# MadNLP/MadNLP.jl

Hardware: NVIDIA H100
Metric: ipm_iters_per_sec (higher is better)
Workload: dtype f64

## Files before the change

### include/b200kkt.h

```cpp
#ifndef B200KKT_H
#define B200KKT_H

#include <stdint.h>

#ifdef __cplusplus
extern "C" {
#endif

#define B2_OK                 0
#define B2_ERR_INVALID        1
#define B2_ERR_CUDA           2
#define B2_ERR_SYMBOLIC       3
#define B2_ERR_FACTORIZATION  4
#define B2_ERR_SOLVE          5
#define B2_ERR_NO_DEVICE      6
#define B2_ERR_UNSUPPORTED    7

#define B2_ORDER_METIS_ND 0
#define B2_ORDER_MINDEG   1
#define B2_ORDER_NATURAL  2
#define B2_ORDER_USER     3

const char* b2_last_error(void);
int b2_version(void);
int b2_device_count(int* count);

typedef struct b2_options {
    int32_t ordering;
    int32_t nemin;
    double  relax_zeros;
    double  pivot_eps;
    int32_t use_cuda_graph;
    int32_t small_front_max;
    int32_t n_parts;
    int32_t part_rank;
    int32_t kkt_n_primal;
    int32_t fuse_max_fronts;
    int32_t dep_schedule;
    int32_t chain_merge_f;
    int32_t kkt_n_dual;
    int32_t dense_pivoting;
    int32_t sparse_pivoting;
    int32_t reserved[1];
} b2_options;

#define B2_DENSE_PIVOT_STATIC        0
#define B2_DENSE_PIVOT_BUNCH_KAUFMAN 1
#define B2_SPARSE_PIVOT_STATIC       0
#define B2_SPARSE_PIVOT_PAIRS        1

#define B2_PIVOT_1X1            0
#define B2_PIVOT_1X1_PERTURBED  1
#define B2_PIVOT_2X2_FIRST      2
#define B2_PIVOT_2X2_SECOND     3

int b2_options_default(b2_options* opt);

typedef struct b2_solver b2_solver;

typedef struct b2_stats {
    int64_t n, nnz_a, nnz_l, flops;
    int64_t n_supernodes, n_levels;
    int64_t max_front, n_small_fronts, n_big_fronts;
    int64_t factor_bytes, workspace_bytes;
    int64_t sep_rows;
    int64_t n_factor_launches, n_solve_launches;
    int64_t n_perturbed;
} b2_stats;

int b2_create(int32_t n, int64_t nnz, const int32_t* colptr_h, const int32_t* rowval_h,
              const double* nzval_d, const b2_options* opt, const int32_t* user_perm_h,
              b2_solver** out);
int b2_create_symbolic_only(int32_t n, int64_t nnz, const int32_t* colptr_h, const int32_t* rowval_h,
                            const b2_options* opt, const int32_t* user_perm_h, b2_solver** out);
int b2_destroy(b2_solver* s);
int b2_set_values_ptr(b2_solver* s, const double* nzval_d);
int b2_factorize(b2_solver* s, void* stream);
int b2_inertia(b2_solver* s, int64_t* num_pos, int64_t* num_zero, int64_t* num_neg, void* stream);
int b2_inertia_enqueue(b2_solver* s, void* stream);
int b2_inertia_fetch(b2_solver* s, int64_t* num_pos, int64_t* num_zero, int64_t* num_neg);
int b2_solve(b2_solver* s, double* x_d, int32_t nrhs, void* stream);
int b2_improve(b2_solver* s, int32_t* changed);
int b2_get_stats(b2_solver* s, b2_stats* st);
int b2_get_perm(b2_solver* s, int32_t* perm_h);

int b2_exchange_buffer(b2_solver* s, double** buf_d, int64_t* n_factor_doubles, int64_t* n_solve_doubles);
int b2_exchange_vector(b2_solver* s, double** buf_d, int64_t* n_doubles);
int b2_inertia_parts(b2_solver* s, int64_t* local_neg, int64_t* local_zero, int64_t* top_neg, int64_t* top_zero, void* stream);
int b2_factorize_local(b2_solver* s, void* stream);
int b2_factorize_top(b2_solver* s, void* stream);
int b2_solve_fwd_local(b2_solver* s, double* x_d, void* stream);
int b2_solve_top(b2_solver* s, double* x_d, void* stream);
int b2_solve_bwd_local(b2_solver* s, double* x_d, void* stream);
int b2_owned_mask(b2_solver* s, uint8_t* owned_h);

typedef struct b2_symbolic_sizes {
    int64_t n, n_supernodes, n_rows, n_children, n_rel, n_amap, n_levels, lval_size, cb_size;
} b2_symbolic_sizes;
int b2_symbolic_query(b2_solver* s, b2_symbolic_sizes* sz);
int b2_symbolic_export(b2_solver* s, int32_t* perm, int32_t* sn_first, int32_t* sn_parent, int32_t* sn_level,
                       int64_t* rows_ptr, int32_t* rows, int64_t* lp_off, int64_t* cb_off,
                       int64_t* rel_ptr, int32_t* rel, int64_t* amap_ptr, int64_t* amap_src, int64_t* amap_dst);
int b2_symbolic_owner(b2_solver* s, int32_t* owner);
int b2_symbolic_exchange(b2_solver* s, int64_t* cbv_off, int64_t* exch_cb, int64_t* exch_cbv);
int b2_debug_get_factor(b2_solver* s, double* lval_h, double* dvec_h);
int b2_symbolic_pairs(b2_solver* s, uint8_t* pair_start_h);
int b2_get_pivot_blocks(b2_solver* s, int8_t* kind_h, double* d_h, double* d_off_h);
int b2_debug_profile_front(b2_solver* s, int32_t sn, int32_t reps, int64_t* stamps_h);
int b2_debug_trace(b2_solver* s, uint64_t* stamps_h, int32_t* parent_h, int32_t* w_h, int32_t* f_h, int64_t capacity, int64_t* count);
int b2_debug_trace_solve(b2_solver* s, uint64_t* stamps_h, int64_t capacity, int64_t* count);
int b2_debug_dep_order(b2_solver* s, int32_t* order_h, int64_t capacity, int64_t* count);

typedef struct b2d_solver b2d_solver;
int b2d_create(int32_t N, int32_t lda, const double* A_d, const b2_options* opt, b2d_solver** out);
int b2d_destroy(b2d_solver* s);
int b2d_debug_trace(b2d_solver* s, uint64_t* stamps_h, int64_t capacity, int64_t* count);
int b2d_factorize(b2d_solver* s, void* stream);
int b2d_inertia(b2d_solver* s, int64_t* num_pos, int64_t* num_zero, int64_t* num_neg, void* stream);
int b2d_inertia_enqueue(b2d_solver* s, void* stream);
int b2d_inertia_fetch(b2d_solver* s, int64_t* num_pos, int64_t* num_zero, int64_t* num_neg);
int b2d_solve(b2d_solver* s, double* x_d, int32_t nrhs, void* stream);
int b2d_get_pivots(b2d_solver* s, int32_t* ipiv_h, double* d_h, double* e_h);

int b2_coo_to_csc(int32_t m, int32_t n, int64_t nnz_coo, const int32_t* I_h, const int32_t* J_h,
                  int32_t* colptr_h, int32_t* rowval_h, int64_t* map_h, int64_t* nnz_csc);

int b2_coo_to_csc_device(int32_t m, int32_t n, int64_t nnz_coo, const int32_t* I_d, const int32_t* J_d,
                         int32_t* colptr_d, int32_t* rowval_d, int64_t* map_d, int64_t* nnz_csc, void* stream);

typedef struct b2_transfer_plan b2_transfer_plan;
int b2_transfer_plan_create(int64_t nnz_coo, int64_t nnz_csc, const int64_t* map_h, b2_transfer_plan** out);
int b2_transfer_plan_destroy(b2_transfer_plan* p);
int b2_transfer(b2_transfer_plan* p, double* dst_nz_d, const double* V_d, void* stream);

typedef struct b2_condensed_plan b2_condensed_plan;
int b2_condensed_symbolic(int32_t n, int32_t m,
                          const int32_t* H_colptr_h, const int32_t* H_rowval_h,
                          const int32_t* Jt_colptr_h, const int32_t* Jt_rowval_h,
                          b2_condensed_plan** out, int64_t* nnz_aug);
int b2_condensed_symbolic_device(int32_t n, int32_t m,
                                 const int32_t* H_colptr_d, const int32_t* H_rowval_d,
                                 const int32_t* Jt_colptr_d, const int32_t* Jt_rowval_d,
                                 b2_condensed_plan** out, int64_t* nnz_aug, void* stream);
int b2_condensed_pattern(b2_condensed_plan* p, int32_t* colptr_h, int32_t* rowval_h);
int b2_condensed_plan_sizes(b2_condensed_plan* p, int64_t* n_dptr, int64_t* n_hptr, int64_t* n_jptr);
int b2_condensed_plan_destroy(b2_condensed_plan* p);
int b2_condensed_assemble(b2_condensed_plan* p, double* aug_nz_d, const double* pr_diag_d,
                          const double* du_diag_d, const double* H_nz_d, const double* Jt_nz_d,
                          double* diag_buffer_d, void* stream);

int b2d_condensed_assemble(int32_t n, int32_t m, int32_t ns, int32_t n_eq,
                           const int64_t* ind_ineq_d, const int64_t* ind_eq_d,
                           const double* hess_d, const double* jac_d,
                           const double* pr_diag_d, const double* du_diag_d,
                           double* diag_buffer_d, double* aug_d, void* stream);

int b2d_aug_assemble(int32_t n, int32_t m, int32_t ns, const int64_t* ind_ineq_d,
                     const double* hess_d, const double* jac_d, const double* pr_diag_d,
                     const double* du_diag_d, const double* diag_hess_d, double* aug_d, void* stream);
int b2d_copy_diag(int32_t n, int32_t lda, const double* A_d, double* d_d, void* stream);

typedef struct b2d_ozaki_plan b2d_ozaki_plan;
int b2d_ozaki_plan_create(int32_t n, int32_t ns, b2d_ozaki_plan** out);
int b2d_ozaki_plan_destroy(b2d_ozaki_plan* p);
int b2d_condensed_assemble_ozaki(b2d_ozaki_plan* p, int32_t n, int32_t m, int32_t ns, int32_t n_eq,
                                 const int64_t* ind_ineq_d, const int64_t* ind_eq_d,
                                 const double* hess_d, const double* jac_d,
                                 const double* pr_diag_d, const double* du_diag_d,
                                 double* diag_buffer_d, double* aug_d, void* stream);
int b2d_ozaki_plan_status(b2d_ozaki_plan* p, int32_t* timed_out, void* stream);

int b2d_gemv_n(int32_t rows, int32_t cols, int32_t lda, const double* A_d, const double* x_d, double* y_d, double alpha, double beta, void* stream);
int b2d_gemv_t(int32_t rows, int32_t cols, int32_t lda, const double* A_d, const double* x_d, double* y_d, double alpha, double beta, void* stream);
int b2d_symv_lower(int32_t n, int32_t lda, const double* A_d, const double* x_d, double* y_d, double alpha, double beta, void* stream);

typedef struct b2_bounds b2_bounds;
typedef struct b2d_kkt b2d_kkt;
int b2d_kkt_create(int32_t n, int32_t m, int32_t ns, const int64_t* ind_ineq_h, b2d_kkt** out);
int b2d_kkt_destroy(b2d_kkt* k);
int b2d_kkt_solve_pre(b2d_kkt* k, b2_bounds* b, const double* jac_d, const double* pr_diag_d, const double* diag_buffer_d,
                      const double* l_diag_d, const double* u_diag_d, double* buffer_d, double* pd_buffer_d, double* w_d, void* stream);
int b2d_kkt_solve_post(b2d_kkt* k, b2_bounds* b, const double* jac_d, const double* pr_diag_d, const double* diag_buffer_d,
                       const double* l_lower_d, const double* u_lower_d, const double* l_diag_d, const double* u_diag_d,
                       const double* buffer_d, const double* pd_buffer_d, double* w_d, void* stream);
int b2d_kkt_mul(b2d_kkt* k, b2_bounds* b, const double* hess_d, const double* jac_d, const double* reg_d, const double* du_diag_d,
                const double* l_lower_d, const double* u_lower_d, const double* l_diag_d, const double* u_diag_d,
                double alpha, double beta, const double* x_d, double* w_d, void* stream);

typedef struct b2_bounds b2_bounds;
int b2_bounds_create(int64_t n_tot, int64_t nlb, int64_t nub, const int64_t* ind_lb_h, const int64_t* ind_ub_h,
                     b2_bounds** out);
int b2_bounds_destroy(b2_bounds* b);

int b2_set_aug_diagonal(b2_bounds* b, const double* reg_d, const double* l_lower_d, const double* l_diag_d,
                        const double* u_lower_d, const double* u_diag_d, double* pr_diag_d, void* stream);
int b2_set_aug_diagonal_unreduced(int64_t n_tot, int64_t nlb, int64_t nub, const double* reg_d, const double* l_lower_d,
                                  const double* u_lower_d, double* pr_diag_d, double* l_lower_aug_d, double* u_lower_aug_d,
                                  void* stream);
int b2_unreduced_solve_pre(int64_t n_tot, int64_t m, int64_t nlb, int64_t nub, const double* l_lower_aug_d,
                           const double* u_lower_aug_d, double* w_d, void* stream);
int b2_unreduced_solve_post(int64_t n_tot, int64_t m, int64_t nlb, int64_t nub, const double* l_lower_aug_d,
                            const double* u_lower_aug_d, double* w_d, void* stream);
int b2_scaled_set_aug_diagonal(b2_bounds* b, const double* reg_d, const double* l_lower_d, const double* l_diag_d,
                               const double* u_lower_d, const double* u_diag_d, double* pr_diag_d, double* scaling_d, void* stream);
int b2_scaled_transfer(b2_transfer_plan* p, int64_t n, int64_t n_tot, const int32_t* colptr_d, const int32_t* rowval_d,
                       const double* scaling_d, double* dst_nz_d, const double* V_d, void* stream);
int b2_scaled_solve_pre(b2_bounds* b, int64_t m, const double* l_diag_d, const double* u_diag_d, const double* scaling_d, double* w_d,
                        void* stream);
int b2_scaled_solve_post(b2_bounds* b, int64_t m, const double* l_lower_d, const double* u_lower_d, const double* l_diag_d,
                         const double* u_diag_d, const double* scaling_d, double* w_d, void* stream);
int b2_scaled_kktmul(b2_bounds* b, int64_t m, const double* reg_d, const double* du_diag_d, const double* l_lower_d,
                     const double* u_lower_d, const double* l_diag_d, const double* u_diag_d, double alpha, double beta,
                     const double* x_d, double* w_d, void* stream);
int b2_scaled_regularize_diagonal(int64_t n_tot, int64_t m, double dw, double dc, const double* scaling_d, double* reg_d,
                                  double* pr_diag_d, double* du_diag_d, void* stream);
int b2_regularize_diagonal(int64_t n_tot, int64_t m, double dw, double dc, double* reg_d, double* pr_diag_d,
                           double* du_diag_d, void* stream);
int b2_reduce_rhs(b2_bounds* b, int64_t m, const double* l_diag_d, const double* u_diag_d, double* w_d, void* stream);
int b2_finish_aug_solve(b2_bounds* b, int64_t m, const double* l_lower_d, const double* u_lower_d,
                        const double* l_diag_d, const double* u_diag_d, double* w_d, void* stream);

typedef struct b2_spmv_plan b2_spmv_plan;
int b2_spmv_plan_create(int32_t nrow, int32_t ncol, const int32_t* colptr_h, const int32_t* rowval_h, b2_spmv_plan** out);
int b2_spmv_plan_destroy(b2_spmv_plan* p);
int b2_spmv_n(b2_spmv_plan* p, const double* nz_d, const double* x_d, double* y_d, double alpha, double beta, void* stream);
int b2_spmv_t(b2_spmv_plan* p, const double* nz_d, const double* x_d, double* y_d, double alpha, double beta, void* stream);
int b2_spmv_symlower(b2_spmv_plan* p, const double* nz_d, const double* x_d, double* y_d, double alpha, double beta, void* stream);

int b2_kktmul(b2_bounds* b, int64_t m, const double* reg_d, const double* du_diag_d,
              const double* l_lower_d, const double* u_lower_d, const double* l_diag_d, const double* u_diag_d,
              double alpha, double beta, const double* x_d, double* w_d, void* stream);

int b2_condensed_solve_pre(b2_bounds* b, b2_spmv_plan* jt, int64_t n, int64_t m,
                           const double* jt_nz_d, const double* pr_diag_d, const double* diag_buffer_d,
                           const double* l_diag_d, const double* u_diag_d, double* buffer_d, double* w_d, void* stream);
int b2_condensed_solve_post(b2_bounds* b, b2_spmv_plan* jt, int64_t n, int64_t m,
                            const double* jt_nz_d, const double* pr_diag_d, const double* diag_buffer_d,
                            const double* l_lower_d, const double* u_lower_d, const double* l_diag_d, const double* u_diag_d,
                            const double* buffer_d, double* w_d, void* stream);
int b2_condensed_refine_pre(b2_bounds* b, b2_spmv_plan* jt, int64_t n, int64_t m,
                            const double* jt_nz_d, const double* pr_diag_d, const double* diag_buffer_d,
                            const double* l_diag_d, const double* u_diag_d, double* buffer_d, double* w_d, double* norms_d, void* stream);
int b2_condensed_solve_post_update(b2_bounds* b, b2_spmv_plan* jt, int64_t n, int64_t m,
                                   const double* jt_nz_d, const double* pr_diag_d, const double* diag_buffer_d,
                                   const double* l_lower_d, const double* u_lower_d, const double* l_diag_d, const double* u_diag_d,
                                   const double* buffer_d, double* w_d, double* x_d, double* norms_d, void* stream);
int b2_condensed_kkt_mul(b2_bounds* b, b2_spmv_plan* hess, b2_spmv_plan* jt, int64_t n, int64_t m,
                         const double* hess_nz_d, const double* jt_nz_d,
                         const double* reg_d, const double* du_diag_d, const double* l_lower_d, const double* u_lower_d,
                         const double* l_diag_d, const double* u_diag_d, double alpha, double beta,
                         const double* x_d, double* w_d, void* stream);
int b2_condensed_kkt_mul_norm(b2_bounds* b, b2_spmv_plan* hess, b2_spmv_plan* jt, int64_t n, int64_t m,
                         const double* hess_nz_d, const double* jt_nz_d,
                         const double* reg_d, const double* du_diag_d, const double* l_lower_d, const double* u_lower_d,
                         const double* l_diag_d, const double* u_diag_d, double alpha, double beta,
                         const double* x_d, double* w_d, double* norm_inf_d, void* stream);
int b2_condensed_kkt_mul_norm_y(b2_bounds* b, b2_spmv_plan* hess, b2_spmv_plan* jt, int64_t n, int64_t m,
                           const double* hess_nz_d, const double* jt_nz_d,
                           const double* reg_d, const double* du_diag_d, const double* l_lower_d, const double* u_lower_d,
                           const double* l_diag_d, const double* u_diag_d, double alpha, double beta,
                           const double* x_d, const double* y_d, double* w_d, double* norm_inf_d, void* stream);

int b2_richardson_begin(int64_t n, const double* b_d, double* w_d, double* x_d, double* norm_b_d, void* stream);
int b2_richardson_update(int64_t n, const double* b_d, double* w_d, double* x_d, double* norms_d, void* stream);
int b2_norm_inf(int64_t n, const double* x_d, double* out_d, void* stream);
int b2_axpy(int64_t n, double a, const double* x_d, double* y_d, void* stream);
int b2_copy(int64_t n, const double* x_d, double* y_d, void* stream);
int b2_copy_many(int32_t count, const double* const* src_d, double* const* dst_d, const int64_t* n, void* stream);
int b2_fill(int64_t n, double v, double* x_d, void* stream);

int b2_get_alpha_max(b2_bounds* b, const double* x_d, const double* xl_d, const double* xu_d, const double* dx_d, double tau,
                     double* out_d, void* stream);
int b2_get_alpha_z(b2_bounds* b, const double* zl_d, const double* zu_d, const double* dzl_d, const double* dzu_d, double tau,
                   double* out_d, void* stream);
int b2_get_varphi(b2_bounds* b, double obj_val, const double* x_d, const double* xl_d, const double* xu_d, double mu, double* out_d,
                  void* stream);
int b2_get_varphi_d(b2_bounds* b, const double* f_d, const double* x_d, const double* xl_d, const double* xu_d, const double* dx_d,
                    double mu, double* out_d, void* stream);
int b2_get_inf_du(b2_bounds* b, const double* f_d, const double* zl_d, const double* zu_d, const double* jacl_d, double sd,
                  double* out_d, void* stream);
int b2_get_inf_compl(b2_bounds* b, const double* x_d, const double* xl_d, const double* xu_d, const double* zl_d, const double* zu_d,
                     double mu, double sc, double* out_d, void* stream);
int b2_get_average_complementarity(b2_bounds* b, const double* x_d, const double* xl_d, const double* xu_d, const double* zl_d,
                                   const double* zu_d, double* out_d, void* stream);
int b2_get_min_complementarity(b2_bounds* b, const double* x_d, const double* xl_d, const double* xu_d, const double* zl_d,
                               const double* zu_d, double* out_d, void* stream);
int b2_get_rel_search_norm(b2_bounds* b, int64_t n, const double* x_d, const double* dx_d, double* out_d, void* stream);
int b2_get_sd(b2_bounds* b, int64_t m, const double* l_d, const double* zl_d, const double* zu_d, double s_max, double* out_d,
              void* stream);
int b2_get_sc(b2_bounds* b, const double* zl_d, const double* zu_d, double s_max, double* out_d, void* stream);
int b2_set_aug_rhs(b2_bounds* b, int64_t m, const double* x_d, const double* xl_d, const double* xu_d, const double* f_d,
                   const double* zl_d, const double* zu_d, const double* jacl_d, const double* c_d, double mu, double* p_d, void* stream);

int b2_set_g_ifr(int64_t n, const double* f_d, const double* x_d, const double* xl_d, const double* xu_d, const double* jacl_d, double mu,
                 double* g_d, void* stream);
int b2_set_aug_rhs_ifr(int64_t n_tot, int64_t m, int64_t nlb, int64_t nub, const double* c_d, double* p0_d, void* stream);
#define B2_CURV_WXT  0
#define B2_CURV_WXN  1
#define B2_CURV_GN   2
#define B2_CURV_TT   3
#define B2_CURV_LHS  4
#define B2_CURV_PASS 5
#define B2_CURV_RESULT_LEN 6
int b2_mul_hess_blk_tail(b2_bounds* b, int64_t n_h, int32_t unreduced, const double* pr_diag_d, const double* l_lower_d,
                         const double* l_diag_d, const double* u_lower_d, const double* u_diag_d, const double* t_d, double* wx_d,
                         const double* n_d, const double* g_d, double tol, double* result_d, void* stream);

int b2_rr_init(b2_bounds* b, int64_t m, const double* x_d, const double* c_d, double mu_R, double rho, double* x_ref_d, double* D_R_d,
               double* f_R_d, double* pp_d, double* nn_d, double* zp_d, double* zn_d, double* y_d, double* zl_d, double* zu_d, void* stream);
int b2_set_aug_rr(b2_bounds* b, int64_t m, double del_w, double del_c, double zeta, const double* D_R_d, const double* pp_d,
                  const double* nn_d, const double* zp_d, const double* zn_d, const double* x_d, const double* xl_d, const double* xu_d,
                  const double* zl_d, const double* zu_d, double* reg_d, double* du_diag_d, double* l_lower_d, double* u_lower_d,
                  double* l_diag_d, double* u_diag_d, void* stream);
int b2_set_aug_rr_scaled(b2_bounds* b, int64_t m, double del_w, double del_c, double zeta, const double* D_R_d, const double* pp_d,
                         const double* nn_d, const double* zp_d, const double* zn_d, const double* x_d, const double* xl_d, const double* xu_d,
                         const double* zl_d, const double* zu_d, double* reg_d, double* du_diag_d, double* l_lower_d, double* u_lower_d,
                         double* l_diag_d, double* u_diag_d, void* stream);
int b2_set_aug_rhs_rr(b2_bounds* b, int64_t m, const double* x_d, const double* xl_d, const double* xu_d, const double* zl_d,
                      const double* zu_d, const double* jacl_d, const double* f_R_d, const double* c_d, const double* y_d, const double* pp_d,
                      const double* nn_d, const double* zp_d, const double* zn_d, double mu_R, double rho, double* p_d, void* stream);
int b2_finish_aug_solve_rr(int64_t m, const double* l_d, const double* dl_d, const double* pp_d, const double* nn_d, const double* zp_d,
                           const double* zn_d, double mu_R, double rho, double* dpp_d, double* dnn_d, double* dzp_d, double* dzn_d,
                           void* stream);
int b2_set_f_rr(int64_t n, double zeta, const double* D_R_d, const double* x_d, const double* x_ref_d, double* f_R_d, void* stream);
int b2_reset_bound_dual(int64_t n, double* z_d, const double* x_d, double mu, double kappa_sigma, void* stream);
int b2_reset_bound_dual_lu(b2_bounds* b, double* zl_d, double* zu_d, const double* x_d, const double* xl_d, const double* xu_d, double mu,
                           double kappa_sigma, void* stream);
int b2_adjust_boundary(b2_bounds* b, const double* x_d, double* xl_d, double* xu_d, double mu, void* stream);
int b2_get_theta(b2_bounds* b, int64_t m, const double* c_d, double* out_d, void* stream);
int b2_get_theta_r(b2_bounds* b, int64_t m, const double* c_d, const double* pp_d, const double* nn_d, double* out_d, void* stream);
int b2_get_inf_pr_r(b2_bounds* b, int64_t m, const double* c_d, const double* pp_d, const double* nn_d, double* out_d, void* stream);
int b2_get_obj_val_r(b2_bounds* b, int64_t m, const double* pp_d, const double* nn_d, const double* D_R_d, const double* x_d,
                     const double* x_ref_d, double rho, double zeta, double* out_d, void* stream);
int b2_get_inf_du_r(b2_bounds* b, int64_t m, const double* f_R_d, const double* l_d, const double* zl_d, const double* zu_d,
                    const double* jacl_d, const double* zp_d, const double* zn_d, double rho, double sd, double* out_d, void* stream);
int b2_get_inf_compl_r(b2_bounds* b, int64_t m, const double* x_d, const double* xl_d, const double* xu_d, const double* zl_d,
                       const double* zu_d, const double* pp_d, const double* zp_d, const double* nn_d, const double* zn_d, double mu_R,
                       double sc, double* out_d, void* stream);
int b2_get_alpha_max_r(b2_bounds* b, int64_t m, const double* x_d, const double* xl_d, const double* xu_d, const double* dx_d,
                       const double* pp_d, const double* dpp_d, const double* nn_d, const double* dnn_d, double tau_R, double* out_d,
                       void* stream);
int b2_get_alpha_z_r(b2_bounds* b, int64_t m, const double* zl_d, const double* zu_d, const double* dzl_d, const double* dzu_d,
                     const double* zp_d, const double* dzp_d, const double* zn_d, const double* dzn_d, double tau_R, double* out_d,
                     void* stream);
int b2_get_varphi_r(b2_bounds* b, int64_t m, double obj_val, const double* x_d, const double* xl_d, const double* xu_d, const double* pp_d,
                    const double* nn_d, double mu_R, double* out_d, void* stream);
int b2_get_varphi_d_r(b2_bounds* b, int64_t m, const double* f_R_d, const double* x_d, const double* xl_d, const double* xu_d,
                      const double* dx_d, const double* pp_d, const double* nn_d, const double* dpp_d, const double* dnn_d, double mu_R,
                      double rho, double* out_d, void* stream);

int b2_set_aug_diagonal_iterate(b2_bounds* b, int64_t m, double del_w, double del_c, const double* x_d, const double* xl_d, const double* xu_d,
                                const double* zl_d, const double* zu_d, double* reg_d, double* du_diag_d, double* l_lower_d,
                                double* u_lower_d, double* l_diag_d, double* u_diag_d, void* stream);
int b2_set_aug_diagonal_iterate_scaled(b2_bounds* b, int64_t m, double del_w, double del_c, const double* x_d, const double* xl_d,
                                       const double* xu_d, const double* zl_d, const double* zu_d, double* reg_d, double* du_diag_d,
                                       double* l_lower_d, double* u_lower_d, double* l_diag_d, double* u_diag_d, void* stream);
int b2_set_aug_rhs_perturbed(b2_bounds* b, int64_t m, const double* x_d, const double* xl_d, const double* xu_d, const double* f_d,
                             const double* zl_d, const double* zu_d, const double* jacl_d, const double* c_d, const double* c_trial_d,
                             double alpha, double mu, double kappa_d, int64_t nllb, const int64_t* ind_llb_d, int64_t nuub,
                             const int64_t* ind_uub_d, double* p_d, void* stream);
int b2_set_initial_rhs(b2_bounds* b, int64_t m, const double* f_d, const double* zl_d, const double* zu_d, double* p_d, void* stream);
#define B2_DUAL_INIT_NORM       0
#define B2_DUAL_INIT_COPY       1
#define B2_DUAL_INIT_RESULT_LEN 2
int b2_dual_init_select(b2_bounds* b, int64_t m, const double* dy_d, int32_t solved, double constr_mult_init_max, double* y_d,
                        double* result_d, void* stream);
int b2_get_pd_error(b2_bounds* b, int64_t m, const double* c_d, const double* f_d, const double* zl_d, const double* zu_d,
                    const double* jacl_d, const double* x_d, const double* xl_d, const double* xu_d, double mu, double* out_d, void* stream);
int b2_restore_update(b2_bounds* b, int64_t m, const double* alpha_max_d, const double* alpha_z_d, double* alpha_d, const double* dx_d,
                      const double* dy_d, const double* dzl_d, const double* dzu_d, double* x_d, double* y_d, double* zl_d, double* zu_d,
                      void* stream);
int b2_soc_trial(int64_t n, const double* alpha_d, const double* x_d, const double* wx_d, double* x_trial_d, void* stream);

#define B2_QF_TAU         0
#define B2_QF_NRM_PRIMAL  1
#define B2_QF_NRM_DUAL    2
#define B2_QF_MU_AVG      3
#define B2_QF_SCAL_LEN    4
#define B2_QF_SIGMA       0
#define B2_QF_MU          1
#define B2_QF_N_EVAL      2
#define B2_QF_N_GS_ITER   3
#define B2_QF_TOL_EXIT    4
#define B2_QF_TRACE       8
#define B2_QF_MAX_GS_ITER 64
#define B2_QF_RESULT_LEN(max_gs_iter) (B2_QF_TRACE + 4 * (6 + (max_gs_iter)))
int b2_primal_dual_norm2(b2_bounds* b, int64_t m, const double* p_d, double* out_d, void* stream);
int b2_set_centering_aug_rhs(b2_bounds* b, int64_t m, int64_t nllb, const int64_t* ind_llb_d, int64_t nuub, const int64_t* ind_uub_d,
                             const double* mu_d, double kappa_d, double* p_d, void* stream);
int b2_qf_search(b2_bounds* b, int64_t m, const double* x_d, const double* xl_d, const double* xu_d, const double* zl_d, const double* zu_d,
                 const double* aff_d, const double* cen_d, const double* scal_d, double sigma_min, double sigma_max, double mu_min,
                 double mu_max, double sigma_tol, int32_t max_gs_iter, double* result_d, void* stream);

typedef struct b2_lbfgs b2_lbfgs;
int b2_lbfgs_create(int64_t n, int32_t max_history, int32_t init_strategy, double init_value, double sigma_min, double sigma_max,
                    b2_lbfgs** out);
int b2_lbfgs_destroy(b2_lbfgs* h);
int b2_lbfgs_state(b2_lbfgs* h, int64_t* p, int64_t* skipped, double* sigma, void* stream);
int b2_lbfgs_init(b2_lbfgs* h, double* Bk_d, const double* g0_d, double f0, void* stream);
int b2_lbfgs_update(b2_lbfgs* h, double* Bk_d, const double* sk_d, const double* yk_d, void* stream);
int b2_lbfgs_smw_prepare(b2_lbfgs* h, b2_solver* s, int64_t n_tot_plus_m, double* H_d, void* stream);
int b2_lbfgs_smw_apply(b2_lbfgs* h, int64_t n_tot_plus_m, const double* H_d, double* w_d, void* stream);
int b2_lbfgs_kkt_mul_lowrank(b2_lbfgs* h, double alpha, const double* x_d, double* w_d, void* stream);
#define B2_LBFGS_BUF_S  0
#define B2_LBFGS_BUF_Y  1
#define B2_LBFGS_BUF_U  2
#define B2_LBFGS_BUF_V  3
#define B2_LBFGS_BUF_SS 4
#define B2_LBFGS_BUF_L  5
#define B2_LBFGS_BUF_D  6
#define B2_LBFGS_BUF_J  7
#define B2_LBFGS_BUF_DL 8
#define B2_LBFGS_BUF_T  9
#define B2_LBFGS_BUF_TF 10
int b2_lbfgs_debug_get(b2_lbfgs* h, int32_t what, double* dst_h, int64_t* first, void* stream);
int b2_lbfgs_debug_ipiv(b2_lbfgs* h, int32_t* ipiv_h, void* stream);
int b2_debug_bk_factor(int32_t N, double* A_d, int32_t* ipiv_d, void* stream);
int b2_debug_bk_solve(int32_t N, const double* F_d, const int32_t* ipiv_d, double* b_d, void* stream);

#define B2_QN_BFGS        1
#define B2_QN_DAMPED_BFGS 2
typedef struct b2d_qn b2d_qn;
int b2d_qn_create(int64_t n, int32_t kind, b2d_qn** out);
int b2d_qn_destroy(b2d_qn* h);
int b2d_qn_init(b2d_qn* h, double* Bk_d, const double* g0_d, double f0, void* stream);
int b2d_qn_update(b2d_qn* h, double* Bk_d, const double* sk_d, const double* yk_d, void* stream);
int b2d_qn_rank2(b2d_qn* h, double* Bk_d, const double* yk_d, void* stream);
int b2d_qn_state(b2d_qn* h, int32_t* instantiated, int32_t* accepted, double* scalars, void* stream);
int b2d_qn_debug_vectors(b2d_qn* h, double* bsk_h, double* rk_h, void* stream);

#define B2_KRYLOV_MAX_RESTART 16
#define B2_KRYLOV_H           0
#define B2_KRYLOV_CS          272
#define B2_KRYLOV_SN          288
#define B2_KRYLOV_G           304
#define B2_KRYLOV_Y           321
#define B2_KRYLOV_SCALE       337
#define B2_KRYLOV_REC         344
#define B2_KRYLOV_REC_EST     0
#define B2_KRYLOV_REC_H       1
#define B2_KRYLOV_REC_NORM_W  2
#define B2_KRYLOV_REC_NORM_X  3
#define B2_KRYLOV_REC_NORM_B  4
#define B2_KRYLOV_REC_NORM_B2 5
#define B2_KRYLOV_REC_LEN     8
#define B2_KRYLOV_STATE_LEN   352
typedef struct b2_krylov b2_krylov;
int b2_krylov_create(int64_t n, int32_t restart, b2_krylov** out);
int b2_krylov_destroy(b2_krylov* h);
int b2_krylov_buffers(b2_krylov* h, double** V_d, double** Z_d, double** state_d);
int b2_krylov_begin(b2_krylov* h, int32_t first, const double* b_d, double* x_d, double* w_d, void* stream);
int b2_krylov_scale(b2_krylov* h, int32_t k, const double* w_d, void* stream);
int b2_krylov_orthogonalize(b2_krylov* h, int32_t k, double* w_d, void* stream);
int b2_krylov_close(b2_krylov* h, int32_t m, const double* b_d, double* x_d, double* w_d, void* stream);

typedef struct b2_inertia_source {
    const int32_t* counters_d;
    int64_t n;
    int32_t neg[2], zero[2];
    int32_t fail;
    int32_t reserved;
} b2_inertia_source;
int b2_inertia_source_get(b2_solver* s, b2_inertia_source* out);
typedef struct b2_refine_record {
    double ratio;
    double norm_w, norm_x, norm_b;
    int64_t ir;
    int64_t steps;
    int64_t num_pos, num_zero, num_neg;
    int32_t inertia_ok;
    int32_t fail;
    int64_t seq;
} b2_refine_record;
typedef struct b2_refine_loop b2_refine_loop;
int b2_refine_loop_create(b2_refine_loop** out);
int b2_refine_loop_destroy(b2_refine_loop* h);
int b2_refine_loop_begin(b2_refine_loop* h, int64_t n, const double* b_d, double* w_d, double* x_d, double* norms_d, void* stream);
int b2_refine_loop_end(b2_refine_loop* h, const b2_inertia_source* src, int64_t expect_pos, int64_t expect_neg, int32_t max_iter,
                       double tol, void* stream);
int b2_refine_loop_launch(b2_refine_loop* h, void* stream);
int b2_refine_loop_wait(b2_refine_loop* h);
int b2_refine_loop_record(b2_refine_loop* h, b2_refine_record* out);

typedef struct b2_inertia_options {
    double first_hessian_perturbation, min_hessian_perturbation, max_hessian_perturbation;
    double perturb_inc_fact_first, perturb_inc_fact, perturb_dec_fact;
} b2_inertia_options;
#define B2_TRIALS_ACCEPTED 1
#define B2_TRIALS_FAILED   2
#define B2_TRIALS_HANDOVER 3
#define B2_TRIALS_FAULT    4
typedef struct b2_inertia_record {
    int32_t status;
    int32_t inertia_ok;
    int64_t trials;
    double del_w, del_w_prev, del_c_prev;
    int64_t num_pos, num_zero, num_neg;
    int64_t ir;
    double ratio;
    int64_t ir_total;
    int64_t seq;
} b2_inertia_record;
int b2_inertia_trial_bound(const b2_inertia_options* opt, int64_t* out);
typedef struct b2_inertia_loop b2_inertia_loop;
int b2_inertia_loop_create(const b2_inertia_options* opt, b2_inertia_loop** out);
int b2_inertia_loop_destroy(b2_inertia_loop* h);
int b2_inertia_loop_begin(b2_inertia_loop* h, int64_t n_tot, int64_t m, double* reg_d, double* pr_diag_d, double* du_diag_d,
                          int32_t dual_always, void* stream);
int b2_inertia_loop_begin_scaled(b2_inertia_loop* h, int64_t n_tot, int64_t m, double* reg_d, double* pr_diag_d, double* du_diag_d,
                                 const double* scaling_d, int32_t dual_always, void* stream);
int b2_inertia_loop_refine(b2_inertia_loop* h, const b2_inertia_source* src, int64_t expect_pos, int64_t expect_neg, int64_t n,
                           const double* b_d, double* w_d, double* x_d, double* norms_d, void* stream);
int b2_inertia_loop_end(b2_inertia_loop* h, int32_t max_iter, double tol, double acceptable_tol, void* stream);
int b2_inertia_loop_launch(b2_inertia_loop* h, double del_w_last, double del_c, int64_t num_zero, void* stream);
int b2_inertia_loop_wait(b2_inertia_loop* h);
int b2_inertia_loop_record(b2_inertia_loop* h, b2_inertia_record* out, double* del_w_out, int64_t cap);


#ifdef __cplusplus
}
#endif
#endif
```

### madnlp.jl_b200/capi.py

```python
from __future__ import annotations

import ctypes as C
import os

_HERE = os.path.dirname(os.path.abspath(__file__))
LIB_PATH = os.path.join(_HERE, "csrc", "libb200kkt.so")

B2_OK = 0
B2_ERR_INVALID, B2_ERR_CUDA, B2_ERR_SYMBOLIC, B2_ERR_FACTORIZATION, B2_ERR_SOLVE, B2_ERR_NO_DEVICE, B2_ERR_UNSUPPORTED = 1, 2, 3, 4, 5, 6, 7
ORDER_METIS_ND, ORDER_MINDEG, ORDER_NATURAL, ORDER_USER = 0, 1, 2, 3
QN_BFGS, QN_DAMPED_BFGS = 1, 2
B2_DENSE_PIVOT_STATIC, B2_DENSE_PIVOT_BUNCH_KAUFMAN = 0, 1
B2_SPARSE_PIVOT_STATIC, B2_SPARSE_PIVOT_PAIRS = 0, 1
B2_PIVOT_1X1, B2_PIVOT_1X1_PERTURBED, B2_PIVOT_2X2_FIRST, B2_PIVOT_2X2_SECOND = 0, 1, 2, 3
CURV_WXT, CURV_WXN, CURV_GN, CURV_TT, CURV_LHS, CURV_PASS, CURV_RESULT_LEN = 0, 1, 2, 3, 4, 5, 6
DUAL_INIT_NORM, DUAL_INIT_COPY, DUAL_INIT_RESULT_LEN = 0, 1, 2
QF_TAU, QF_NRM_PRIMAL, QF_NRM_DUAL, QF_MU_AVG, QF_SCAL_LEN = 0, 1, 2, 3, 4
QF_SIGMA, QF_MU, QF_N_EVAL, QF_N_GS_ITER, QF_TOL_EXIT, QF_TRACE, QF_MAX_GS_ITER = 0, 1, 2, 3, 4, 8, 64
KRYLOV_MAX_RESTART, KRYLOV_Y, KRYLOV_REC, KRYLOV_REC_LEN, KRYLOV_STATE_LEN = 16, 321, 344, 8, 352
KREC_EST, KREC_H, KREC_NORM_W, KREC_NORM_X, KREC_NORM_B, KREC_NORM_B2 = 0, 1, 2, 3, 4, 5


def qf_result_len(max_gs_iter):
    return QF_TRACE + 4 * (6 + max_gs_iter)


class B2Error(RuntimeError):
    def __init__(self, code, msg):
        super().__init__(f"b200kkt error {code}: {msg}")
        self.code = code


class SymbolicException(B2Error):
    pass


class FactorizationException(B2Error):
    pass


class SolveException(B2Error):
    pass


class InertiaException(RuntimeError):
    pass


class _Pivoting(C.Structure):
    _fields_ = [("dense_pivoting", C.c_int32), ("sparse_pivoting", C.c_int32)]


class _OptionsTail(C.Union):
    _anonymous_ = ("_pivoting",)
    _fields_ = [("_pivoting", _Pivoting), ("reserved", C.c_int32 * 3)]


class Options(C.Structure):
    _anonymous_ = ("_tail",)
    _fields_ = [
        ("ordering", C.c_int32), ("nemin", C.c_int32), ("relax_zeros", C.c_double), ("pivot_eps", C.c_double),
        ("use_cuda_graph", C.c_int32), ("small_front_max", C.c_int32), ("n_parts", C.c_int32), ("part_rank", C.c_int32),
        ("kkt_n_primal", C.c_int32), ("fuse_max_fronts", C.c_int32), ("dep_schedule", C.c_int32), ("chain_merge_f", C.c_int32), ("kkt_n_dual", C.c_int32),
        ("_tail", _OptionsTail),
    ]


class Stats(C.Structure):
    _fields_ = [(k, C.c_int64) for k in (
        "n", "nnz_a", "nnz_l", "flops", "n_supernodes", "n_levels", "max_front", "n_small_fronts", "n_big_fronts",
        "factor_bytes", "workspace_bytes", "sep_rows", "n_factor_launches", "n_solve_launches", "n_perturbed")]

    def as_dict(self):
        return {k: int(getattr(self, k)) for k, _ in self._fields_}


class InertiaSource(C.Structure):
    _fields_ = [("counters_d", C.c_void_p), ("n", C.c_int64), ("neg", C.c_int32 * 2), ("zero", C.c_int32 * 2), ("fail", C.c_int32),
                ("reserved", C.c_int32)]


class RefineRecord(C.Structure):
    _fields_ = [("ratio", C.c_double), ("norm_w", C.c_double), ("norm_x", C.c_double), ("norm_b", C.c_double), ("ir", C.c_int64),
                ("steps", C.c_int64), ("num_pos", C.c_int64), ("num_zero", C.c_int64), ("num_neg", C.c_int64), ("inertia_ok", C.c_int32),
                ("fail", C.c_int32), ("seq", C.c_int64)]


class InertiaSchedule(C.Structure):
    _fields_ = [(k, C.c_double) for k in ("first_hessian_perturbation", "min_hessian_perturbation", "max_hessian_perturbation",
                                          "perturb_inc_fact_first", "perturb_inc_fact", "perturb_dec_fact")]


TRIALS_ACCEPTED, TRIALS_FAILED, TRIALS_HANDOVER, TRIALS_FAULT = 1, 2, 3, 4


class InertiaRecord(C.Structure):
    _fields_ = [("status", C.c_int32), ("inertia_ok", C.c_int32), ("trials", C.c_int64), ("del_w", C.c_double),
                ("del_w_prev", C.c_double), ("del_c_prev", C.c_double), ("num_pos", C.c_int64), ("num_zero", C.c_int64),
                ("num_neg", C.c_int64), ("ir", C.c_int64), ("ratio", C.c_double), ("ir_total", C.c_int64), ("seq", C.c_int64)]


class SymbolicSizes(C.Structure):
    _fields_ = [(k, C.c_int64) for k in (
        "n", "n_supernodes", "n_rows", "n_children", "n_rel", "n_amap", "n_levels", "lval_size", "cb_size")]


def _load():
    if not os.path.exists(LIB_PATH):
        raise ImportError(
            f"{LIB_PATH} not found: build it with `python -c 'import __graft_entry__ as g; g.build()'` "
            f"(or `make -C madnlp.jl_b200/csrc`). The GPU KKT path has no CPU fallback.")
    return C.CDLL(LIB_PATH)


lib = _load()

_p = C.c_void_p
_i32, _i64, _f64 = C.c_int32, C.c_int64, C.c_double
_PP = C.POINTER(C.c_void_p)

PROTOTYPES = {
    "b2_last_error": (C.c_char_p, []),
    "b2_version": (C.c_int, []),
    "b2_device_count": (C.c_int, [C.POINTER(C.c_int)]),
    "b2_options_default": (C.c_int, [C.POINTER(Options)]),
    "b2_create": (C.c_int, [_i32, _i64, _p, _p, _p, C.POINTER(Options), _p, _PP]),
    "b2_create_symbolic_only": (C.c_int, [_i32, _i64, _p, _p, C.POINTER(Options), _p, _PP]),
    "b2_destroy": (C.c_int, [_p]),
    "b2_set_values_ptr": (C.c_int, [_p, _p]),
    "b2_factorize": (C.c_int, [_p, _p]),
    "b2_inertia": (C.c_int, [_p, C.POINTER(_i64), C.POINTER(_i64), C.POINTER(_i64), _p]),
    "b2_inertia_enqueue": (C.c_int, [_p, _p]),
    "b2_inertia_fetch": (C.c_int, [_p, C.POINTER(_i64), C.POINTER(_i64), C.POINTER(_i64)]),
    "b2_solve": (C.c_int, [_p, _p, _i32, _p]),
    "b2_improve": (C.c_int, [_p, C.POINTER(_i32)]),
    "b2_get_stats": (C.c_int, [_p, C.POINTER(Stats)]),
    "b2_get_perm": (C.c_int, [_p, _p]),
    "b2_exchange_buffer": (C.c_int, [_p, _PP, C.POINTER(_i64), C.POINTER(_i64)]),
    "b2_exchange_vector": (C.c_int, [_p, _PP, C.POINTER(_i64)]),
    "b2_inertia_parts": (C.c_int, [_p, C.POINTER(_i64), C.POINTER(_i64), C.POINTER(_i64), C.POINTER(_i64), _p]),
    "b2_factorize_local": (C.c_int, [_p, _p]),
    "b2_factorize_top": (C.c_int, [_p, _p]),
    "b2_solve_fwd_local": (C.c_int, [_p, _p, _p]),
    "b2_solve_top": (C.c_int, [_p, _p, _p]),
    "b2_solve_bwd_local": (C.c_int, [_p, _p, _p]),
    "b2_owned_mask": (C.c_int, [_p, _p]),
    "b2_symbolic_query": (C.c_int, [_p, C.POINTER(SymbolicSizes)]),
    "b2_symbolic_export": (C.c_int, [_p] + [_p] * 13),
    "b2_symbolic_owner": (C.c_int, [_p, _p]),
    "b2_symbolic_exchange": (C.c_int, [_p, _p, C.POINTER(_i64), C.POINTER(_i64)]),
    "b2_debug_get_factor": (C.c_int, [_p, _p, _p]),
    "b2_symbolic_pairs": (C.c_int, [_p, _p]),
    "b2_get_pivot_blocks": (C.c_int, [_p, _p, _p, _p]),
    "b2_debug_profile_front": (C.c_int, [_p, _i32, _i32, _p]),
    "b2d_debug_trace": (C.c_int, [_p, _p, _i64, C.POINTER(_i64)]),
    "b2_debug_trace": (C.c_int, [_p, _p, _p, _p, _p, _i64, C.POINTER(_i64)]),
    "b2_debug_trace_solve": (C.c_int, [_p, _p, _i64, C.POINTER(_i64)]),
    "b2_debug_dep_order": (C.c_int, [_p, _p, _i64, C.POINTER(_i64)]),
    "b2d_create": (C.c_int, [_i32, _i32, _p, C.POINTER(Options), _PP]),
    "b2d_destroy": (C.c_int, [_p]),
    "b2d_factorize": (C.c_int, [_p, _p]),
    "b2d_inertia": (C.c_int, [_p, C.POINTER(_i64), C.POINTER(_i64), C.POINTER(_i64), _p]),
    "b2d_inertia_enqueue": (C.c_int, [_p, _p]),
    "b2d_inertia_fetch": (C.c_int, [_p, C.POINTER(_i64), C.POINTER(_i64), C.POINTER(_i64)]),
    "b2d_solve": (C.c_int, [_p, _p, _i32, _p]),
    "b2d_get_pivots": (C.c_int, [_p, _p, _p, _p]),
    "b2_condensed_symbolic_device": (C.c_int, [_i32, _i32, _p, _p, _p, _p, _PP, C.POINTER(_i64), _p]),
    "b2_coo_to_csc_device": (C.c_int, [_i32, _i32, _i64, _p, _p, _p, _p, _p, C.POINTER(_i64), _p]),
    "b2d_ozaki_plan_create": (C.c_int, [_i32, _i32, _PP]),
    "b2d_ozaki_plan_destroy": (C.c_int, [_p]),
    "b2d_condensed_assemble_ozaki": (C.c_int, [_p, _i32, _i32, _i32, _i32] + [_p] * 9),
    "b2d_ozaki_plan_status": (C.c_int, [_p, C.POINTER(_i32), _p]),
    "b2d_kkt_create": (C.c_int, [_i32, _i32, _i32, _p, _PP]),
    "b2d_kkt_destroy": (C.c_int, [_p]),
    "b2d_kkt_solve_pre": (C.c_int, [_p] * 10 + [_p]),
    "b2d_kkt_solve_post": (C.c_int, [_p] * 12 + [_p]),
    "b2d_kkt_mul": (C.c_int, [_p] * 10 + [_f64, _f64, _p, _p, _p]),
    "b2d_gemv_n": (C.c_int, [_i32, _i32, _i32, _p, _p, _p, _f64, _f64, _p]),
    "b2d_gemv_t": (C.c_int, [_i32, _i32, _i32, _p, _p, _p, _f64, _f64, _p]),
    "b2d_symv_lower": (C.c_int, [_i32, _i32, _p, _p, _p, _f64, _f64, _p]),
    "b2_coo_to_csc": (C.c_int, [_i32, _i32, _i64, _p, _p, _p, _p, _p, C.POINTER(_i64)]),
    "b2_transfer_plan_create": (C.c_int, [_i64, _i64, _p, _PP]),
    "b2_transfer_plan_destroy": (C.c_int, [_p]),
    "b2_transfer": (C.c_int, [_p, _p, _p, _p]),
    "b2_condensed_symbolic": (C.c_int, [_i32, _i32, _p, _p, _p, _p, _PP, C.POINTER(_i64)]),
    "b2_condensed_pattern": (C.c_int, [_p, _p, _p]),
    "b2_condensed_plan_sizes": (C.c_int, [_p, C.POINTER(_i64), C.POINTER(_i64), C.POINTER(_i64)]),
    "b2_condensed_plan_destroy": (C.c_int, [_p]),
    "b2_condensed_assemble": (C.c_int, [_p, _p, _p, _p, _p, _p, _p, _p]),
    "b2d_condensed_assemble": (C.c_int, [_i32, _i32, _i32, _i32, _p, _p, _p, _p, _p, _p, _p, _p, _p]),
    "b2d_aug_assemble": (C.c_int, [_i32, _i32, _i32] + [_p] * 8),
    "b2d_copy_diag": (C.c_int, [_i32, _i32, _p, _p, _p]),
    "b2_bounds_create": (C.c_int, [_i64, _i64, _i64, _p, _p, _PP]),
    "b2_bounds_destroy": (C.c_int, [_p]),
    "b2_set_aug_diagonal": (C.c_int, [_p, _p, _p, _p, _p, _p, _p, _p]),
    "b2_set_aug_diagonal_unreduced": (C.c_int, [_i64, _i64, _i64] + [_p] * 7),
    "b2_unreduced_solve_pre": (C.c_int, [_i64, _i64, _i64, _i64, _p, _p, _p, _p]),
    "b2_unreduced_solve_post": (C.c_int, [_i64, _i64, _i64, _i64, _p, _p, _p, _p]),
    "b2_regularize_diagonal": (C.c_int, [_i64, _i64, _f64, _f64, _p, _p, _p, _p]),
    "b2_scaled_set_aug_diagonal": (C.c_int, [_p] + [_p] * 7 + [_p]),
    "b2_scaled_transfer": (C.c_int, [_p, _i64, _i64, _p, _p, _p, _p, _p, _p]),
    "b2_scaled_solve_pre": (C.c_int, [_p, _i64, _p, _p, _p, _p, _p]),
    "b2_scaled_solve_post": (C.c_int, [_p, _i64, _p, _p, _p, _p, _p, _p, _p]),
    "b2_scaled_kktmul": (C.c_int, [_p, _i64, _p, _p, _p, _p, _p, _p, _f64, _f64, _p, _p, _p]),
    "b2_scaled_regularize_diagonal": (C.c_int, [_i64, _i64, _f64, _f64, _p, _p, _p, _p, _p]),
    "b2_reduce_rhs": (C.c_int, [_p, _i64, _p, _p, _p, _p]),
    "b2_finish_aug_solve": (C.c_int, [_p, _i64, _p, _p, _p, _p, _p, _p]),
    "b2_spmv_plan_create": (C.c_int, [_i32, _i32, _p, _p, _PP]),
    "b2_spmv_plan_destroy": (C.c_int, [_p]),
    "b2_spmv_n": (C.c_int, [_p, _p, _p, _p, _f64, _f64, _p]),
    "b2_spmv_t": (C.c_int, [_p, _p, _p, _p, _f64, _f64, _p]),
    "b2_spmv_symlower": (C.c_int, [_p, _p, _p, _p, _f64, _f64, _p]),
    "b2_kktmul": (C.c_int, [_p, _i64, _p, _p, _p, _p, _p, _p, _f64, _f64, _p, _p, _p]),
    "b2_condensed_solve_pre": (C.c_int, [_p, _p, _i64, _i64, _p, _p, _p, _p, _p, _p, _p, _p]),
    "b2_condensed_solve_post": (C.c_int, [_p, _p, _i64, _i64, _p, _p, _p, _p, _p, _p, _p, _p, _p, _p]),
    "b2_condensed_kkt_mul": (C.c_int, [_p, _p, _p, _i64, _i64, _p, _p, _p, _p, _p, _p, _p, _p, _f64, _f64, _p, _p, _p]),
    "b2_condensed_kkt_mul_norm": (C.c_int, [_p, _p, _p, _i64, _i64, _p, _p, _p, _p, _p, _p, _p, _p, _f64, _f64, _p, _p, _p, _p]),
    "b2_condensed_refine_pre": (C.c_int, [_p, _p, _i64, _i64, _p, _p, _p, _p, _p, _p, _p, _p, _p]),
    "b2_condensed_solve_post_update": (C.c_int, [_p, _p, _i64, _i64, _p, _p, _p, _p, _p, _p, _p, _p, _p, _p, _p, _p]),
    "b2_condensed_kkt_mul_norm_y": (C.c_int, [_p, _p, _p, _i64, _i64, _p, _p, _p, _p, _p, _p, _p, _p, _f64, _f64, _p, _p, _p, _p, _p]),
    "b2_get_alpha_max": (C.c_int, [_p, _p, _p, _p, _p, _f64, _p, _p]),
    "b2_get_alpha_z": (C.c_int, [_p, _p, _p, _p, _p, _f64, _p, _p]),
    "b2_get_varphi": (C.c_int, [_p, _f64, _p, _p, _p, _f64, _p, _p]),
    "b2_get_varphi_d": (C.c_int, [_p, _p, _p, _p, _p, _p, _f64, _p, _p]),
    "b2_get_inf_du": (C.c_int, [_p, _p, _p, _p, _p, _f64, _p, _p]),
    "b2_get_inf_compl": (C.c_int, [_p, _p, _p, _p, _p, _p, _f64, _f64, _p, _p]),
    "b2_get_average_complementarity": (C.c_int, [_p, _p, _p, _p, _p, _p, _p, _p]),
    "b2_get_min_complementarity": (C.c_int, [_p, _p, _p, _p, _p, _p, _p, _p]),
    "b2_get_rel_search_norm": (C.c_int, [_p, _i64, _p, _p, _p, _p]),
    "b2_get_sd": (C.c_int, [_p, _i64, _p, _p, _p, _f64, _p, _p]),
    "b2_get_sc": (C.c_int, [_p, _p, _p, _f64, _p, _p]),
    "b2_set_aug_rhs": (C.c_int, [_p, _i64, _p, _p, _p, _p, _p, _p, _p, _p, _f64, _p, _p]),
    "b2_set_g_ifr": (C.c_int, [_i64, _p, _p, _p, _p, _p, _f64, _p, _p]),
    "b2_set_aug_rhs_ifr": (C.c_int, [_i64, _i64, _i64, _i64, _p, _p, _p]),
    "b2_mul_hess_blk_tail": (C.c_int, [_p, _i64, _i32] + [_p] * 9 + [_f64, _p, _p]),
    "b2_rr_init": (C.c_int, [_p, _i64, _p, _p, _f64, _f64] + [_p] * 10 + [_p]),
    "b2_set_aug_rr": (C.c_int, [_p, _i64, _f64, _f64, _f64] + [_p] * 16 + [_p]),
    "b2_set_aug_rr_scaled": (C.c_int, [_p, _i64, _f64, _f64, _f64] + [_p] * 16 + [_p]),
    "b2_set_aug_rhs_rr": (C.c_int, [_p, _i64] + [_p] * 13 + [_f64, _f64, _p, _p]),
    "b2_finish_aug_solve_rr": (C.c_int, [_i64] + [_p] * 6 + [_f64, _f64] + [_p] * 4 + [_p]),
    "b2_set_f_rr": (C.c_int, [_i64, _f64, _p, _p, _p, _p, _p]),
    "b2_reset_bound_dual": (C.c_int, [_i64, _p, _p, _f64, _f64, _p]),
    "b2_reset_bound_dual_lu": (C.c_int, [_p] + [_p] * 5 + [_f64, _f64, _p]),
    "b2_adjust_boundary": (C.c_int, [_p, _p, _p, _p, _f64, _p]),
    "b2_get_theta": (C.c_int, [_p, _i64, _p, _p, _p]),
    "b2_get_theta_r": (C.c_int, [_p, _i64, _p, _p, _p, _p, _p]),
    "b2_get_inf_pr_r": (C.c_int, [_p, _i64, _p, _p, _p, _p, _p]),
    "b2_get_obj_val_r": (C.c_int, [_p, _i64] + [_p] * 5 + [_f64, _f64, _p, _p]),
    "b2_get_inf_du_r": (C.c_int, [_p, _i64] + [_p] * 7 + [_f64, _f64, _p, _p]),
    "b2_get_inf_compl_r": (C.c_int, [_p, _i64] + [_p] * 9 + [_f64, _f64, _p, _p]),
    "b2_get_alpha_max_r": (C.c_int, [_p, _i64] + [_p] * 8 + [_f64, _p, _p]),
    "b2_get_alpha_z_r": (C.c_int, [_p, _i64] + [_p] * 8 + [_f64, _p, _p]),
    "b2_get_varphi_r": (C.c_int, [_p, _i64, _f64] + [_p] * 5 + [_f64, _p, _p]),
    "b2_get_varphi_d_r": (C.c_int, [_p, _i64] + [_p] * 9 + [_f64, _f64, _p, _p]),
    "b2_set_aug_diagonal_iterate": (C.c_int, [_p, _i64, _f64, _f64] + [_p] * 11 + [_p]),
    "b2_set_aug_diagonal_iterate_scaled": (C.c_int, [_p, _i64, _f64, _f64] + [_p] * 11 + [_p]),
    "b2_set_aug_rhs_perturbed": (C.c_int, [_p, _i64] + [_p] * 9 + [_f64, _f64, _f64, _i64, _p, _i64, _p, _p, _p]),
    "b2_set_initial_rhs": (C.c_int, [_p, _i64, _p, _p, _p, _p, _p]),
    "b2_dual_init_select": (C.c_int, [_p, _i64, _p, _i32, _f64, _p, _p, _p]),
    "b2_get_pd_error": (C.c_int, [_p, _i64] + [_p] * 8 + [_f64, _p, _p]),
    "b2_restore_update": (C.c_int, [_p, _i64] + [_p] * 11 + [_p]),
    "b2_soc_trial": (C.c_int, [_i64, _p, _p, _p, _p, _p]),
    "b2_primal_dual_norm2": (C.c_int, [_p, _i64, _p, _p, _p]),
    "b2_set_centering_aug_rhs": (C.c_int, [_p, _i64, _i64, _p, _i64, _p, _p, _f64, _p, _p]),
    "b2_qf_search": (C.c_int, [_p, _i64] + [_p] * 8 + [_f64] * 5 + [_i32, _p, _p]),
    "b2_richardson_begin": (C.c_int, [_i64, _p, _p, _p, _p, _p]),
    "b2_richardson_update": (C.c_int, [_i64, _p, _p, _p, _p, _p]),
    "b2_copy_many": (C.c_int, [_i32, C.POINTER(C.c_void_p), C.POINTER(C.c_void_p), C.POINTER(_i64), _p]),
    "b2_norm_inf": (C.c_int, [_i64, _p, _p, _p]),
    "b2_axpy": (C.c_int, [_i64, _f64, _p, _p, _p]),
    "b2_copy": (C.c_int, [_i64, _p, _p, _p]),
    "b2_fill": (C.c_int, [_i64, _f64, _p, _p]),
    "b2_lbfgs_create": (C.c_int, [_i64, _i32, _i32, _f64, _f64, _f64, _PP]),
    "b2_lbfgs_destroy": (C.c_int, [_p]),
    "b2_lbfgs_state": (C.c_int, [_p, C.POINTER(_i64), C.POINTER(_i64), C.POINTER(_f64), _p]),
    "b2_lbfgs_init": (C.c_int, [_p, _p, _p, _f64, _p]),
    "b2_lbfgs_update": (C.c_int, [_p, _p, _p, _p, _p]),
    "b2_lbfgs_smw_prepare": (C.c_int, [_p, _p, _i64, _p, _p]),
    "b2_lbfgs_smw_apply": (C.c_int, [_p, _i64, _p, _p, _p]),
    "b2_lbfgs_kkt_mul_lowrank": (C.c_int, [_p, _f64, _p, _p, _p]),
    "b2_lbfgs_debug_get": (C.c_int, [_p, _i32, _p, C.POINTER(_i64), _p]),
    "b2_lbfgs_debug_ipiv": (C.c_int, [_p, _p, _p]),
    "b2_debug_bk_factor": (C.c_int, [_i32, _p, _p, _p]),
    "b2_debug_bk_solve": (C.c_int, [_i32, _p, _p, _p, _p]),
    "b2d_qn_create": (C.c_int, [_i64, _i32, _PP]),
    "b2d_qn_destroy": (C.c_int, [_p]),
    "b2d_qn_init": (C.c_int, [_p, _p, _p, _f64, _p]),
    "b2d_qn_update": (C.c_int, [_p, _p, _p, _p, _p]),
    "b2d_qn_rank2": (C.c_int, [_p, _p, _p, _p]),
    "b2d_qn_state": (C.c_int, [_p, C.POINTER(_i32), C.POINTER(_i32), _p, _p]),
    "b2d_qn_debug_vectors": (C.c_int, [_p, _p, _p, _p]),
    "b2_krylov_create": (C.c_int, [_i64, _i32, _PP]),
    "b2_krylov_destroy": (C.c_int, [_p]),
    "b2_krylov_buffers": (C.c_int, [_p, _PP, _PP, _PP]),
    "b2_krylov_begin": (C.c_int, [_p, _i32, _p, _p, _p, _p]),
    "b2_krylov_scale": (C.c_int, [_p, _i32, _p, _p]),
    "b2_krylov_orthogonalize": (C.c_int, [_p, _i32, _p, _p]),
    "b2_krylov_close": (C.c_int, [_p, _i32, _p, _p, _p, _p]),
    "b2_inertia_source_get": (C.c_int, [_p, C.POINTER(InertiaSource)]),
    "b2_refine_loop_create": (C.c_int, [_PP]),
    "b2_refine_loop_destroy": (C.c_int, [_p]),
    "b2_refine_loop_begin": (C.c_int, [_p, _i64, _p, _p, _p, _p, _p]),
    "b2_refine_loop_end": (C.c_int, [_p, C.POINTER(InertiaSource), _i64, _i64, _i32, _f64, _p]),
    "b2_refine_loop_launch": (C.c_int, [_p, _p]),
    "b2_refine_loop_wait": (C.c_int, [_p]),
    "b2_refine_loop_record": (C.c_int, [_p, C.POINTER(RefineRecord)]),
    "b2_inertia_trial_bound": (C.c_int, [C.POINTER(InertiaSchedule), C.POINTER(_i64)]),
    "b2_inertia_loop_create": (C.c_int, [C.POINTER(InertiaSchedule), _PP]),
    "b2_inertia_loop_destroy": (C.c_int, [_p]),
    "b2_inertia_loop_begin": (C.c_int, [_p, _i64, _i64, _p, _p, _p, _i32, _p]),
    "b2_inertia_loop_begin_scaled": (C.c_int, [_p, _i64, _i64, _p, _p, _p, _p, _i32, _p]),
    "b2_inertia_loop_refine": (C.c_int, [_p, C.POINTER(InertiaSource), _i64, _i64, _i64, _p, _p, _p, _p, _p]),
    "b2_inertia_loop_end": (C.c_int, [_p, _i32, _f64, _f64, _p]),
    "b2_inertia_loop_launch": (C.c_int, [_p, _f64, _f64, _i64, _p]),
    "b2_inertia_loop_wait": (C.c_int, [_p]),
    "b2_inertia_loop_record": (C.c_int, [_p, C.POINTER(InertiaRecord), _p, _i64]),
}

for _name, (_res, _args) in PROTOTYPES.items():
    _fn = getattr(lib, _name)
    _fn.restype = _res
    _fn.argtypes = _args


def last_error() -> str:
    return (lib.b2_last_error() or b"").decode()


_EXC = {B2_ERR_SYMBOLIC: SymbolicException, B2_ERR_FACTORIZATION: FactorizationException, B2_ERR_SOLVE: SolveException}


def check(rc: int):
    if rc != B2_OK:
        raise _EXC.get(rc, B2Error)(rc, last_error())


def device_count() -> int:
    n = C.c_int(0)
    rc = lib.b2_device_count(C.byref(n))
    return n.value if rc == B2_OK else 0


def require_device():
    if device_count() == 0:
        raise B2Error(B2_ERR_NO_DEVICE, "no CUDA device visible; the GPU KKT path has no CPU fallback")


def default_options(**kw) -> Options:
    o = Options()
    check(lib.b2_options_default(C.byref(o)))
    for k, v in kw.items():
        if not hasattr(o, k):
            raise TypeError(f"unknown b2 option {k!r}")
        setattr(o, k, v)
    return o


def ptr(t):
    if t is None:
        return None
    if hasattr(t, "data_ptr"):
        return t.data_ptr()
    return t.ctypes.data


def copy_many(pairs, stream=None):
    n = len(pairs)
    src = (C.c_void_p * n)(*[s.data_ptr() for s, _ in pairs])
    dst = (C.c_void_p * n)(*[d.data_ptr() for _, d in pairs])
    ns = (C.c_int64 * n)(*[d.numel() for _, d in pairs])
    check(lib.b2_copy_many(n, src, dst, ns, stream_ptr(stream)))


def stream_ptr(stream=None):
    if stream is None:
        import torch
        return torch.cuda.current_stream().cuda_stream
    return getattr(stream, "cuda_stream", stream)
```

### madnlp.jl_b200/csrc/assembly.cu

```cuda
#include <algorithm>
#include <cstring>
#include <numeric>
#include <stdexcept>
#include <vector>

#include "common.cuh"
#include "condensed_plan.cuh"

using namespace b2;

extern "C" int b2_coo_to_csc(int32_t m, int32_t n, int64_t nnz_coo, const int32_t* I_h, const int32_t* J_h,
                             int32_t* colptr_h, int32_t* rowval_h, int64_t* map_h, int64_t* nnz_csc) {
    if (m < 0 || n < 0 || nnz_coo < 0 || (nnz_coo && (!I_h || !J_h)) || !colptr_h || !rowval_h || !map_h) {
        set_error("b2_coo_to_csc: invalid argument");
        return B2_ERR_INVALID;
    }
    std::vector<int64_t> order(nnz_coo);
    std::iota(order.begin(), order.end(), (int64_t)0);
    for (int64_t k = 0; k < nnz_coo; ++k)
        if (I_h[k] < 0 || I_h[k] >= m || J_h[k] < 0 || J_h[k] >= n) { set_error("b2_coo_to_csc: index out of range"); return B2_ERR_INVALID; }
    std::stable_sort(order.begin(), order.end(), [&](int64_t a, int64_t b) {
        if (J_h[a] != J_h[b]) return J_h[a] < J_h[b];
        return I_h[a] < I_h[b];
    });
    std::fill(colptr_h, colptr_h + n + 1, 0);
    int64_t slot = -1;
    int32_t li = -1, lj = -1;
    for (int64_t q = 0; q < nnz_coo; ++q) {
        const int64_t k = order[q];
        if (I_h[k] != li || J_h[k] != lj) {
            ++slot;
            li = I_h[k]; lj = J_h[k];
            rowval_h[slot] = li;
            colptr_h[lj + 1]++;
        }
        map_h[k] = slot;
    }
    for (int32_t j = 0; j < n; ++j) colptr_h[j + 1] += colptr_h[j];
    if (nnz_csc) *nnz_csc = slot + 1;
    return B2_OK;
}

struct b2_transfer_plan {
    int64_t nnz_coo = 0, nnz_csc = 0;
    DevBuf<int32_t> ptr;
    DevBuf<int32_t> src;
};

__global__ void k_transfer(int64_t nslot, const int32_t* __restrict__ ptr, const int32_t* __restrict__ src,
                           const double* __restrict__ V, double* __restrict__ dst) {
    pdl_sync();
    for (int64_t i = (int64_t)blockIdx.x * blockDim.x + threadIdx.x; i < nslot; i += (int64_t)gridDim.x * blockDim.x) {
        const int a = ptr[i], b = ptr[i + 1];
        double acc = 0.0;
        for (int q = a; q < b; ++q) acc = __dadd_rn(acc, V[src[q]]);
        dst[i] = acc;
    }
}

extern "C" int b2_transfer_plan_create(int64_t nnz_coo, int64_t nnz_csc, const int64_t* map_h, b2_transfer_plan** out) {
    if (!out || nnz_coo < 0 || nnz_csc < 0 || (nnz_coo && !map_h) || nnz_coo >= (int64_t)1 << 31) {
        set_error("b2_transfer_plan_create: invalid argument");
        return B2_ERR_INVALID;
    }
    std::vector<int32_t> ptr(nnz_csc + 1, 0), src(nnz_coo);
    for (int64_t k = 0; k < nnz_coo; ++k) {
        if (map_h[k] < 0 || map_h[k] >= nnz_csc) { set_error("b2_transfer_plan_create: map out of range"); return B2_ERR_INVALID; }
        ptr[map_h[k] + 1]++;
    }
    for (int64_t i = 0; i < nnz_csc; ++i) ptr[i + 1] += ptr[i];
    std::vector<int32_t> pos(ptr.begin(), ptr.end() - 1);
    for (int64_t k = 0; k < nnz_coo; ++k) src[pos[map_h[k]]++] = (int32_t)k;
    auto* p = new b2_transfer_plan();
    p->nnz_coo = nnz_coo; p->nnz_csc = nnz_csc;
    if (p->ptr.upload(ptr.data(), ptr.size()) != cudaSuccess || p->src.upload(src.data(), src.size()) != cudaSuccess) {
        delete p;
        return cuda_fail(cudaGetLastError(), "transfer plan upload", __FILE__, __LINE__);
    }
    *out = p;
    return B2_OK;
}

extern "C" int b2_transfer_plan_destroy(b2_transfer_plan* p) { delete p; return B2_OK; }

extern "C" int b2_transfer(b2_transfer_plan* p, double* dst_nz_d, const double* V_d, void* stream) {
    if (!p || !dst_nz_d || !V_d) { set_error("b2_transfer: invalid argument"); return B2_ERR_INVALID; }
    if (p->nnz_csc == 0) return B2_OK;
    const int grid = (int)std::min<int64_t>((p->nnz_csc + 255) / 256, 8 * sm_count());
    launch_pdl(k_transfer, dim3(grid), dim3(256), 0, as_stream(stream), p->nnz_csc, p->ptr.p, p->src.p, V_d, dst_nz_d);
    B2_CUDA(cudaGetLastError());
    return B2_OK;
}

__device__ __forceinline__ int64_t slot_column(const int32_t* __restrict__ colptr, int64_t lo, int64_t hi, int64_t slot) {
    while (lo < hi) {
        const int64_t mid = (lo + hi + 1) >> 1;
        if (colptr[mid] <= slot) lo = mid; else hi = mid - 1;
    }
    return lo;
}
__global__ void k_scaled_transfer(int64_t nslot, int64_t ncol, int64_t n_tot, const int32_t* __restrict__ ptr, const int32_t* __restrict__ src,
                                  const int32_t* __restrict__ colptr, const int32_t* __restrict__ rowval, const double* __restrict__ sf,
                                  const double* __restrict__ V, double* __restrict__ dst) {
    __shared__ int64_t cspan[2];
    pdl_sync();
    const int64_t s0 = (int64_t)blockIdx.x * blockDim.x;
    if (threadIdx.x < 2) cspan[threadIdx.x] = slot_column(colptr, 0, ncol - 1, threadIdx.x ? std::min<int64_t>(s0 + blockDim.x, nslot) - 1 : s0);
    __syncthreads();
    const int64_t i = s0 + threadIdx.x;
    if (i >= nslot) return;
    const int64_t c = slot_column(colptr, cspan[0], cspan[1], i);
    const int64_t r = rowval[i];
    const int a = ptr[i], b = ptr[i + 1];
    double acc = 0.0;
    if (c >= n_tot) {
        for (int q = a; q < b; ++q) acc = __dadd_rn(acc, V[src[q]]);
    } else if (r >= n_tot) {
        const double sc = sf[c];
        for (int q = a; q < b; ++q) acc = __dadd_rn(acc, __dmul_rn(V[src[q]], sc));
    } else {
        const double sr = sf[r], sc = sf[c];
        for (int q = a; q < b; ++q) {
            const int k = src[q];
            const double v = V[k];
            acc = __dadd_rn(acc, k < n_tot ? v : __dmul_rn(__dmul_rn(v, sr), sc));
        }
    }
    dst[i] = acc;
}

extern "C" int b2_scaled_transfer(b2_transfer_plan* p, int64_t n, int64_t n_tot, const int32_t* colptr_d, const int32_t* rowval_d,
                                  const double* scaling_d, double* dst_nz_d, const double* V_d, void* stream) {
    B2_NEED(p && n >= 0 && n_tot >= 0 && n_tot <= n && (p->nnz_csc == 0 || (n > 0 && colptr_d && rowval_d && dst_nz_d && V_d)),
            "b2_scaled_transfer");
    B2_NEED(n_tot == 0 || p->nnz_csc == 0 || scaling_d, "b2_scaled_transfer");
    if (p->nnz_csc == 0) return B2_OK;
    launch_pdl(k_scaled_transfer, dim3((unsigned)((p->nnz_csc + 255) / 256)), dim3(256), 0, as_stream(stream), p->nnz_csc, n, n_tot,
               p->ptr.p, p->src.p, colptr_d, rowval_d, scaling_d, V_d, dst_nz_d);
    B2_CUDA(cudaGetLastError());
    return B2_OK;
}

__global__ void k_diag_buffer(int64_t m, const double* __restrict__ Ss, const double* __restrict__ Sd, double* __restrict__ D) {
    pdl_sync();
    for (int64_t i = (int64_t)blockIdx.x * blockDim.x + threadIdx.x; i < m; i += (int64_t)gridDim.x * blockDim.x)
        D[i] = __ddiv_rn(Ss[i], __dsub_rn(1.0, __dmul_rn(Sd[i], Ss[i])));
}

__global__ void k_condensed(int64_t nslot, const int32_t* __restrict__ hsrc, const int32_t* __restrict__ dsrc,
                            const int32_t* __restrict__ tptr, const int4* __restrict__ trip,
                            const double* __restrict__ Hnz, const double* __restrict__ pr, const double* __restrict__ D,
                            const double* __restrict__ Jt, double* __restrict__ nz) {
    pdl_sync();
    for (int64_t i = (int64_t)blockIdx.x * blockDim.x + threadIdx.x; i < nslot; i += (int64_t)gridDim.x * blockDim.x) {
        double acc = 0.0;
        const int h = hsrc[i], dd = dsrc[i];
        if (h >= 0) acc = __dadd_rn(acc, Hnz[h]);
        if (dd >= 0) acc = __dadd_rn(acc, pr[dd]);
        const int a = tptr[i], b = tptr[i + 1];
        for (int q0 = a; q0 < b; q0 += 4) {
            int4 t[4]; double dv[4], j1[4], j2[4];
#pragma unroll
            for (int u = 0; u < 4; ++u) t[u] = (q0 + u < b) ? trip[q0 + u] : make_int4(-1, 0, 0, 0);
#pragma unroll
            for (int u = 0; u < 4; ++u) { const bool ok = t[u].x >= 0; dv[u] = ok ? D[t[u].x] : 0.0; j1[u] = ok ? Jt[t[u].y] : 0.0; j2[u] = ok ? Jt[t[u].z] : 0.0; }
#pragma unroll
            for (int u = 0; u < 4; ++u) if (t[u].x >= 0) acc = __dadd_rn(acc, __dmul_rn(__dmul_rn(dv[u], j1[u]), j2[u]));
        }
        nz[i] = acc;
    }
}

extern "C" int b2_condensed_symbolic(int32_t n, int32_t m, const int32_t* Hc, const int32_t* Hr,
                                     const int32_t* Jc, const int32_t* Jr, b2_condensed_plan** out, int64_t* nnz_aug) {
    if (!out || n <= 0 || m < 0 || !Hc || !Jc) { set_error("b2_condensed_symbolic: invalid argument"); return B2_ERR_INVALID; }
    struct Ent { int32_t col, row, kind, s1, s2; };
    const int64_t nnzH = Hc[n];
    int64_t nj = 0;
    for (int32_t i = 0; i < m; ++i) { const int64_t c = Jc[i + 1] - Jc[i]; nj += c * (c + 1) / 2; }
    std::vector<Ent> e;
    e.reserve((size_t)(n + nnzH + nj));
    for (int32_t i = 0; i < n; ++i) e.push_back({i, i, -1, i, 0});
    for (int32_t j = 0; j < n; ++j)
        for (int32_t p = Hc[j]; p < Hc[j + 1]; ++p) e.push_back({j, Hr[p], 0, p, 0});
    for (int32_t i = 0; i < m; ++i)
        for (int32_t j = Jc[i]; j < Jc[i + 1]; ++j)
            for (int32_t k = j; k < Jc[i + 1]; ++k) e.push_back({Jr[j], Jr[k], i + 1, j, k});
    std::stable_sort(e.begin(), e.end(), [](const Ent& a, const Ent& b) {
        if (a.col != b.col) return a.col < b.col;
        return a.row < b.row;
    });
    auto* p = new b2_condensed_plan();
    p->n = n; p->m = m;
    p->colptr.assign(n + 1, 0);
    std::vector<int32_t> hsrc, dsrc, tptr;
    std::vector<int4> trip;
    trip.reserve(nj);
    int32_t lc = -1, lr = -1;
    for (const Ent& x : e) {
        if (x.row < x.col) { delete p; set_error("b2_condensed_symbolic: entry above the diagonal (H must be lower, Jt rows sorted)"); return B2_ERR_INVALID; }
        if (x.col != lc || x.row != lr) {
            lc = x.col; lr = x.row;
            p->rowval.push_back(x.row);
            p->colptr[x.col + 1]++;
            hsrc.push_back(-1); dsrc.push_back(-1);
            tptr.push_back((int32_t)trip.size());
        }
        if (x.kind == -1) { dsrc.back() = x.s1; p->n_dptr++; }
        else if (x.kind == 0) {
            if (hsrc.back() >= 0) { delete p; set_error("b2_condensed_symbolic: duplicate entry in H"); return B2_ERR_INVALID; }
            hsrc.back() = x.s1; p->n_hptr++;
        } else { trip.push_back(make_int4(x.kind - 1, x.s1, x.s2, 0)); p->n_jptr++; }
    }
    tptr.push_back((int32_t)trip.size());
    for (int32_t j = 0; j < n; ++j) p->colptr[j + 1] += p->colptr[j];
    p->nnz_aug = (int64_t)p->rowval.size();
    if (trip.empty()) trip.push_back(make_int4(0, 0, 0, 0));
    int ndev = 0;
    if (cudaGetDeviceCount(&ndev) == cudaSuccess && ndev > 0) {
        if (p->hsrc.upload(hsrc.data(), hsrc.size()) != cudaSuccess || p->dsrc.upload(dsrc.data(), dsrc.size()) != cudaSuccess ||
            p->tptr.upload(tptr.data(), tptr.size()) != cudaSuccess || p->trip.upload(trip.data(), trip.size()) != cudaSuccess) {
            delete p;
            return cuda_fail(cudaGetLastError(), "condensed plan upload", __FILE__, __LINE__);
        }
    } else {
        cudaGetLastError();
    }
    *out = p;
    if (nnz_aug) *nnz_aug = p->nnz_aug;
    return B2_OK;
}

extern "C" int b2_condensed_pattern(b2_condensed_plan* p, int32_t* colptr_h, int32_t* rowval_h) {
    if (!p || !colptr_h || !rowval_h) return B2_ERR_INVALID;
    std::memcpy(colptr_h, p->colptr.data(), p->colptr.size() * sizeof(int32_t));
    std::memcpy(rowval_h, p->rowval.data(), p->rowval.size() * sizeof(int32_t));
    return B2_OK;
}

extern "C" int b2_condensed_plan_sizes(b2_condensed_plan* p, int64_t* n_dptr, int64_t* n_hptr, int64_t* n_jptr) {
    if (!p) return B2_ERR_INVALID;
    if (n_dptr) *n_dptr = p->n_dptr;
    if (n_hptr) *n_hptr = p->n_hptr;
    if (n_jptr) *n_jptr = p->n_jptr;
    return B2_OK;
}

extern "C" int b2_condensed_plan_destroy(b2_condensed_plan* p) { delete p; return B2_OK; }

extern "C" int b2_condensed_assemble(b2_condensed_plan* p, double* aug_nz_d, const double* pr_diag_d, const double* du_diag_d,
                                     const double* H_nz_d, const double* Jt_nz_d, double* diag_buffer_d, void* stream) {
    if (!p || !aug_nz_d || !pr_diag_d || !du_diag_d || !diag_buffer_d) { set_error("b2_condensed_assemble: invalid argument"); return B2_ERR_INVALID; }
    if (!p->hsrc.p) { set_error("b2_condensed_assemble: plan has no device state (no CUDA device at creation)"); return B2_ERR_NO_DEVICE; }
    cudaStream_t st = as_stream(stream);
    if (p->m > 0) {
        const int g = (int)std::min<int64_t>((p->m + 255) / 256, 8 * sm_count());
        launch_pdl(k_diag_buffer, dim3(g), dim3(256), 0, st, p->m, pr_diag_d + p->n, du_diag_d, diag_buffer_d);
    }
    const int grid = (int)std::min<int64_t>((p->nnz_aug + 255) / 256, 8 * sm_count());
    launch_pdl(k_condensed, dim3(grid), dim3(256), 0, st, p->nnz_aug, p->hsrc.p, p->dsrc.p, p->tptr.p, p->trip.p, H_nz_d, pr_diag_d, diag_buffer_d,
                                      Jt_nz_d, aug_nz_d);
    B2_CUDA(cudaGetLastError());
    return B2_OK;
}

constexpr int DT_M = 128, DT_N = 64, DT_K = 16;

__global__ void k_dense_diag_buffer(int64_t ns, const int64_t* __restrict__ ind_ineq, const double* __restrict__ Ss,
                                    const double* __restrict__ du, double* __restrict__ D) {
    for (int64_t i = (int64_t)blockIdx.x * blockDim.x + threadIdx.x; i < ns; i += (int64_t)gridDim.x * blockDim.x)
        D[i] = Ss[i] / (1.0 - du[ind_ineq[i]] * Ss[i]);
}

__global__ void __launch_bounds__(256) k_dense_syrk(int n, int m, int ns, int N, const int64_t* __restrict__ ind_ineq,
                                                    const double* __restrict__ hess, const double* __restrict__ jac,
                                                    const double* __restrict__ pr, const double* __restrict__ D,
                                                    double* __restrict__ aug) {
    const int ti = blockIdx.x, tj = blockIdx.y;
    const int i0 = ti * DT_M, j0 = tj * DT_N;
    if (j0 > i0 + DT_M - 1) return;
    extern __shared__ double dsm[];
    typedef double (*ATile)[DT_K][DT_M + 4];
    typedef double (*BTile)[DT_K][DT_N + 4];
    ATile As = (ATile)dsm;
    BTile Bs = (BTile)(dsm + 2 * DT_K * (DT_M + 4));
    const int tid = threadIdx.x, warp = tid >> 5, lane = tid & 31;
    const int g = lane >> 2, q = lane & 3;
    const int wi = (warp & 3) * 32, wj = (warp >> 2) * 32;
    double c[4][4][2];
#pragma unroll
    for (int x = 0; x < 4; ++x)
#pragma unroll
        for (int y = 0; y < 4; ++y) c[x][y][0] = c[x][y][1] = 0.0;
    const int nchunk = (ns + DT_K - 1) / DT_K;
    const int lk = tid % DT_K, lc = tid / DT_K;
    double ra[DT_M / 16], rb[DT_N / 16];
    auto gload = [&](int ch) {
        const int k = ch * DT_K + lk;
        const bool kv = k < ns;
        const int64_t row = kv ? ind_ineq[k] : 0;
        const double dk = kv ? D[k] : 0.0;
#pragma unroll
        for (int cc = 0; cc < DT_M / 16; ++cc) {
            const int col = i0 + lc + 16 * cc;
            ra[cc] = (kv && col < n) ? jac[(size_t)col * m + row] : 0.0;
        }
#pragma unroll
        for (int cc = 0; cc < DT_N / 16; ++cc) {
            const int col = j0 + lc + 16 * cc;
            rb[cc] = (kv && col < n) ? dk * jac[(size_t)col * m + row] : 0.0;
        }
    };
    auto sstore = [&](int buf) {
#pragma unroll
        for (int cc = 0; cc < DT_M / 16; ++cc) As[buf][lk][lc + 16 * cc] = ra[cc];
#pragma unroll
        for (int cc = 0; cc < DT_N / 16; ++cc) Bs[buf][lk][lc + 16 * cc] = rb[cc];
    };
    if (nchunk > 0) { gload(0); sstore(0); }
    __syncthreads();
    for (int ch = 0; ch < nchunk; ++ch) {
        const int buf = ch & 1;
        if (ch + 1 < nchunk) gload(ch + 1);
#pragma unroll
        for (int k0 = 0; k0 < DT_K; k0 += 4) {
            double af[4], bf[4];
#pragma unroll
            for (int x = 0; x < 4; ++x) af[x] = As[buf][k0 + q][wi + 8 * x + g];
#pragma unroll
            for (int y = 0; y < 4; ++y) bf[y] = Bs[buf][k0 + q][wj + 8 * y + g];
#pragma unroll
            for (int x = 0; x < 4; x += 2)
#pragma unroll
                for (int y = 0; y < 4; ++y)
                    asm volatile("mma.sync.aligned.m16n8k4.row.col.f64.f64.f64.f64 {%0,%1,%2,%3}, {%4,%5}, {%6}, {%0,%1,%2,%3};\n"
                                 : "+d"(c[x][y][0]), "+d"(c[x][y][1]), "+d"(c[x + 1][y][0]), "+d"(c[x + 1][y][1])
                                 : "d"(af[x]), "d"(af[x + 1]), "d"(bf[y]));
        }
        if (ch + 1 < nchunk) sstore(buf ^ 1);
        __syncthreads();
    }
#pragma unroll
    for (int x = 0; x < 4; ++x)
#pragma unroll
        for (int y = 0; y < 4; ++y)
#pragma unroll
            for (int e = 0; e < 2; ++e) {
                const int i = i0 + wi + 8 * x + g;
                const int j = j0 + wj + 8 * y + 2 * q + e;
                if (i < n && j < n && i >= j) {
                    double v = c[x][y][e] + hess[(size_t)j * n + i];
                    if (i == j) v += pr[i];
                    aug[(size_t)j * N + i] = v;
                }
            }
}

__global__ void k_dense_eq_rows(int n, int m, int n_eq, int N, const int64_t* __restrict__ ind_eq,
                                const double* __restrict__ jac, const double* __restrict__ du, double* __restrict__ aug) {
    const int64_t total = (int64_t)n_eq * N;
    for (int64_t t = (int64_t)blockIdx.x * blockDim.x + threadIdx.x; t < total; t += (int64_t)gridDim.x * blockDim.x) {
        const int i = (int)(t % n_eq), j = (int)(t / n_eq);
        double v;
        if (j < n) v = jac[(size_t)j * m + ind_eq[i]];
        else {
            const int jj = j - n;
            if (jj > i) continue;
            v = (jj == i) ? du[ind_eq[i]] : 0.0;
        }
        aug[(size_t)j * N + n + i] = v;
    }
}

int b2d_assemble_parts(int32_t n, int32_t m, int32_t ns, int32_t n_eq, const int64_t* ind_ineq_d, const int64_t* ind_eq_d,
                       const double* jac_d, const double* pr_diag_d, const double* du_diag_d, double* diag_buffer_d, double* aug_d,
                       bool before_syrk, cudaStream_t st) {
    const int N = n + n_eq;
    if (before_syrk) {
        if (ns > 0) {
            const int g = std::min((ns + 255) / 256, 8 * sm_count());
            k_dense_diag_buffer<<<g, 256, 0, st>>>(ns, ind_ineq_d, pr_diag_d + n, du_diag_d, diag_buffer_d);
        }
    } else if (n_eq > 0) {
        const int64_t total = (int64_t)n_eq * N;
        const int g = (int)std::min<int64_t>((total + 255) / 256, 8 * sm_count());
        k_dense_eq_rows<<<g, 256, 0, st>>>(n, m, n_eq, N, ind_eq_d, jac_d, du_diag_d, aug_d);
    }
    B2_CUDA(cudaGetLastError());
    return B2_OK;
}

extern "C" int b2d_condensed_assemble(int32_t n, int32_t m, int32_t ns, int32_t n_eq, const int64_t* ind_ineq_d,
// ... 73 lines not shown
```

### madnlp.jl_b200/csrc/kktvec.cu

```cuda
#include <algorithm>
#include <cstring>
#include <vector>

#include "bounds.cuh"
#include "common.cuh"

using namespace b2;

extern "C" int b2_bounds_create(int64_t n_tot, int64_t nlb, int64_t nub, const int64_t* ind_lb_h, const int64_t* ind_ub_h,
                                b2_bounds** out) {
    if (!out || n_tot < 0 || nlb < 0 || nub < 0 || (nlb && !ind_lb_h) || (nub && !ind_ub_h)) {
        set_error("b2_bounds_create: invalid argument");
        return B2_ERR_INVALID;
    }
    std::vector<int32_t> lp(n_tot, -1), up(n_tot, -1);
    for (int64_t k = 0; k < nlb; ++k) {
        if (ind_lb_h[k] < 0 || ind_lb_h[k] >= n_tot || lp[ind_lb_h[k]] != -1) { set_error("b2_bounds_create: bad ind_lb"); return B2_ERR_INVALID; }
        lp[ind_lb_h[k]] = (int32_t)k;
    }
    for (int64_t k = 0; k < nub; ++k) {
        if (ind_ub_h[k] < 0 || ind_ub_h[k] >= n_tot || up[ind_ub_h[k]] != -1) { set_error("b2_bounds_create: bad ind_ub"); return B2_ERR_INVALID; }
        up[ind_ub_h[k]] = (int32_t)k;
    }
    auto* b = new b2_bounds();
    b->n_tot = n_tot; b->nlb = nlb; b->nub = nub;
    if (b->ind_lb.upload(ind_lb_h, nlb) != cudaSuccess || b->ind_ub.upload(ind_ub_h, nub) != cudaSuccess ||
        b->lbpos.upload(lp.data(), lp.size()) != cudaSuccess || b->ubpos.upload(up.data(), up.size()) != cudaSuccess ||
        b->red_part.alloc(8 * B2_RED_BLOCKS) != cudaSuccess || b->red_ticket.alloc(1) != cudaSuccess ||
        cudaMemset(b->red_ticket.p, 0, sizeof(unsigned)) != cudaSuccess || b->qf_state.alloc(B2_QF_STATE_DOUBLES) != cudaSuccess ||
        cudaMemset(b->qf_state.p, 0, B2_QF_STATE_DOUBLES * sizeof(double)) != cudaSuccess) {
        delete b;
        return cuda_fail(cudaGetLastError(), "bounds upload", __FILE__, __LINE__);
    }
    *out = b;
    return B2_OK;
}
extern "C" int b2_bounds_destroy(b2_bounds* b) { delete b; return B2_OK; }

__global__ void k_set_aug_diagonal(int64_t n_tot, const int32_t* __restrict__ lbpos, const int32_t* __restrict__ ubpos,
                                   const double* __restrict__ reg, const double* __restrict__ ll, const double* __restrict__ ld,
                                   const double* __restrict__ ul, const double* __restrict__ ud, double* __restrict__ pr) {
    pdl_sync();
    GRID_STRIDE(i, n_tot) {
        double v = reg[i];
        const int p = lbpos[i], q = ubpos[i];
        if (p >= 0) v = __dsub_rn(v, __ddiv_rn(ll[p], ld[p]));
        if (q >= 0) v = __dsub_rn(v, __ddiv_rn(ul[q], ud[q]));
        pr[i] = v;
    }
}
extern "C" int b2_set_aug_diagonal(b2_bounds* b, const double* reg_d, const double* l_lower_d, const double* l_diag_d,
                                   const double* u_lower_d, const double* u_diag_d, double* pr_diag_d, void* stream) {
    if (!b || !reg_d || !pr_diag_d) { set_error("b2_set_aug_diagonal: invalid argument"); return B2_ERR_INVALID; }
    if (b->n_tot == 0) return B2_OK;
    launch_pdl(k_set_aug_diagonal, dim3(grid_elem(b->n_tot)), dim3(256), 0, as_stream(stream), b->n_tot, b->lbpos.p, b->ubpos.p, reg_d, l_lower_d, l_diag_d,
                                                                         u_lower_d, u_diag_d, pr_diag_d);
    B2_CUDA(cudaGetLastError());
    return B2_OK;
}

__global__ void k_set_aug_diagonal_unreduced(int64_t n_tot, int64_t nlb, int64_t nub, const double* __restrict__ reg,
                                             const double* __restrict__ ll, const double* __restrict__ ul, double* __restrict__ pr,
                                             double* __restrict__ lla, double* __restrict__ ula) {
    GRID_STRIDE(t, n_tot + nlb + nub) {
        if (t < n_tot) pr[t] = reg[t];
        else if (t < n_tot + nlb) lla[t - n_tot] = __dsqrt_rn(ll[t - n_tot]);
        else ula[t - n_tot - nlb] = __dsqrt_rn(ul[t - n_tot - nlb]);
    }
}
extern "C" int b2_set_aug_diagonal_unreduced(int64_t n_tot, int64_t nlb, int64_t nub, const double* reg_d, const double* l_lower_d,
                                             const double* u_lower_d, double* pr_diag_d, double* l_lower_aug_d, double* u_lower_aug_d,
                                             void* stream) {
    if (n_tot < 0 || nlb < 0 || nub < 0 || (n_tot && (!reg_d || !pr_diag_d)) || (nlb && (!l_lower_d || !l_lower_aug_d)) ||
        (nub && (!u_lower_d || !u_lower_aug_d))) {
        set_error("b2_set_aug_diagonal_unreduced: invalid argument");
        return B2_ERR_INVALID;
    }
    const int64_t tot = n_tot + nlb + nub;
    if (tot == 0) return B2_OK;
    k_set_aug_diagonal_unreduced<<<grid_elem(tot), 256, 0, as_stream(stream)>>>(n_tot, nlb, nub, reg_d, l_lower_d, u_lower_d, pr_diag_d,
                                                                               l_lower_aug_d, u_lower_aug_d);
    B2_CUDA(cudaGetLastError());
    return B2_OK;
}

template <bool POST>
__global__ void k_unreduced_scale(int64_t nlb, int64_t nub, const double* __restrict__ sl, const double* __restrict__ su,
                                  double* __restrict__ wz) {
    GRID_STRIDE(t, nlb + nub) {
        const bool lower = t < nlb;
        const double s = lower ? sl[t] : su[t - nlb];
        const double v = wz[t];
        if (POST) wz[t] = __dmul_rn(v, lower ? -s : s);
        else if (s != 0.0) wz[t] = __ddiv_rn(v, s);
    }
}
template <bool POST>
static int unreduced_scale(const char* name, int64_t n_tot, int64_t m, int64_t nlb, int64_t nub, const double* sl, const double* su,
                           double* w, void* stream) {
    if (n_tot < 0 || m < 0 || nlb < 0 || nub < 0 || !w || (nlb && !sl) || (nub && !su)) {
        set_error(std::string(name) + ": invalid argument");
        return B2_ERR_INVALID;
    }
    if (nlb + nub == 0) return B2_OK;
    k_unreduced_scale<POST><<<grid_elem(nlb + nub), 256, 0, as_stream(stream)>>>(nlb, nub, sl, su, w + n_tot + m);
    B2_CUDA(cudaGetLastError());
    return B2_OK;
}
extern "C" int b2_unreduced_solve_pre(int64_t n_tot, int64_t m, int64_t nlb, int64_t nub, const double* l_lower_aug_d,
                                      const double* u_lower_aug_d, double* w_d, void* stream) {
    return unreduced_scale<false>("b2_unreduced_solve_pre", n_tot, m, nlb, nub, l_lower_aug_d, u_lower_aug_d, w_d, stream);
}
extern "C" int b2_unreduced_solve_post(int64_t n_tot, int64_t m, int64_t nlb, int64_t nub, const double* l_lower_aug_d,
                                       const double* u_lower_aug_d, double* w_d, void* stream) {
    return unreduced_scale<true>("b2_unreduced_solve_post", n_tot, m, nlb, nub, l_lower_aug_d, u_lower_aug_d, w_d, stream);
}

__global__ void k_regularize(int64_t n_tot, int64_t m, double dw, double dc, double* __restrict__ reg, double* __restrict__ pr,
                             double* __restrict__ du) {
    GRID_STRIDE(i, n_tot + m) {
        if (i < n_tot) { reg[i] += dw; pr[i] += dw; }
        else du[i - n_tot] -= dc;
    }
}
extern "C" int b2_regularize_diagonal(int64_t n_tot, int64_t m, double dw, double dc, double* reg_d, double* pr_diag_d,
                                      double* du_diag_d, void* stream) {
    if (n_tot < 0 || m < 0 || !reg_d || !pr_diag_d || (m && !du_diag_d)) { set_error("b2_regularize_diagonal: invalid argument"); return B2_ERR_INVALID; }
    if (n_tot + m == 0) return B2_OK;
    k_regularize<<<grid_elem(n_tot + m), 256, 0, as_stream(stream)>>>(n_tot, m, dw, dc, reg_d, pr_diag_d, du_diag_d);
    B2_CUDA(cudaGetLastError());
    return B2_OK;
}

__global__ void k_reduce_rhs(int64_t n_tot, int64_t m, int64_t nlb, const int32_t* __restrict__ lbpos, const int32_t* __restrict__ ubpos,
                             const double* __restrict__ ld, const double* __restrict__ ud, double* __restrict__ w) {
    const double* wzl = w + n_tot + m;
    const double* wzu = wzl + nlb;
    GRID_STRIDE(i, n_tot) {
        const int p = lbpos[i], q = ubpos[i];
        if (p < 0 && q < 0) continue;
        double v = w[i];
        if (p >= 0) v = __dsub_rn(v, __ddiv_rn(wzl[p], ld[p]));
        if (q >= 0) v = __dsub_rn(v, __ddiv_rn(wzu[q], ud[q]));
        w[i] = v;
    }
}
extern "C" int b2_reduce_rhs(b2_bounds* b, int64_t m, const double* l_diag_d, const double* u_diag_d, double* w_d, void* stream) {
    if (!b || !w_d) { set_error("b2_reduce_rhs: invalid argument"); return B2_ERR_INVALID; }
    if (b->n_tot == 0) return B2_OK;
    k_reduce_rhs<<<grid_elem(b->n_tot), 256, 0, as_stream(stream)>>>(b->n_tot, m, b->nlb, b->lbpos.p, b->ubpos.p, l_diag_d, u_diag_d, w_d);
    B2_CUDA(cudaGetLastError());
    return B2_OK;
}

__global__ void k_finish_aug_solve(int64_t n_tot, int64_t m, int64_t nlb, int64_t nub, const int64_t* __restrict__ ind_lb,
                                   const int64_t* __restrict__ ind_ub, const double* __restrict__ ll, const double* __restrict__ ul,
                                   const double* __restrict__ ld, const double* __restrict__ ud, double* __restrict__ w) {
    pdl_sync();
    double* dlb = w + n_tot + m;
    double* dub = dlb + nlb;
    GRID_STRIDE(t, nlb + nub) {
        if (t < nlb) dlb[t] = __ddiv_rn(__dadd_rn(-dlb[t], __dmul_rn(ll[t], w[ind_lb[t]])), ld[t]);
        else {
            const int64_t k = t - nlb;
            dub[k] = __ddiv_rn(__dsub_rn(dub[k], __dmul_rn(ul[k], w[ind_ub[k]])), ud[k]);
        }
    }
}
extern "C" int b2_finish_aug_solve(b2_bounds* b, int64_t m, const double* l_lower_d, const double* u_lower_d,
                                   const double* l_diag_d, const double* u_diag_d, double* w_d, void* stream) {
    if (!b || !w_d) { set_error("b2_finish_aug_solve: invalid argument"); return B2_ERR_INVALID; }
    if (b->nlb + b->nub == 0) return B2_OK;
    launch_pdl(k_finish_aug_solve, dim3(grid_elem(b->nlb + b->nub)), dim3(256), 0, as_stream(stream), b->n_tot, m, b->nlb, b->nub, b->ind_lb.p, b->ind_ub.p,
                                                                               l_lower_d, u_lower_d, l_diag_d, u_diag_d, w_d);
    B2_CUDA(cudaGetLastError());
    return B2_OK;
}

struct b2_spmv_plan {
    int32_t nrow = 0, ncol = 0;
    int64_t nnz = 0;
    DevBuf<int32_t> colptr, rowval, rowptr, colidx, valmap;
};

extern "C" int b2_spmv_plan_create(int32_t nrow, int32_t ncol, const int32_t* colptr_h, const int32_t* rowval_h, b2_spmv_plan** out) {
    if (!out || nrow < 0 || ncol < 0 || !colptr_h) { set_error("b2_spmv_plan_create: invalid argument"); return B2_ERR_INVALID; }
    const int64_t nnz = colptr_h[ncol];
    std::vector<int32_t> rowptr(nrow + 1, 0), colidx(nnz), valmap(nnz);
    for (int64_t p = 0; p < nnz; ++p) {
        if (rowval_h[p] < 0 || rowval_h[p] >= nrow) { set_error("b2_spmv_plan_create: row index out of range"); return B2_ERR_INVALID; }
        rowptr[rowval_h[p] + 1]++;
    }
    for (int32_t i = 0; i < nrow; ++i) rowptr[i + 1] += rowptr[i];
    std::vector<int32_t> pos(rowptr.begin(), rowptr.end() - 1);
    for (int32_t j = 0; j < ncol; ++j)
        for (int32_t p = colptr_h[j]; p < colptr_h[j + 1]; ++p) {
            const int32_t q = pos[rowval_h[p]]++;
            colidx[q] = j;
            valmap[q] = p;
        }
    auto* pl = new b2_spmv_plan();
    pl->nrow = nrow; pl->ncol = ncol; pl->nnz = nnz;
    if (pl->colptr.upload(colptr_h, ncol + 1) != cudaSuccess || pl->rowval.upload(rowval_h, nnz) != cudaSuccess ||
        pl->rowptr.upload(rowptr.data(), rowptr.size()) != cudaSuccess || pl->colidx.upload(colidx.data(), nnz) != cudaSuccess ||
        pl->valmap.upload(valmap.data(), nnz) != cudaSuccess) {
        delete pl;
        return cuda_fail(cudaGetLastError(), "spmv plan upload", __FILE__, __LINE__);
    }
    *out = pl;
    return B2_OK;
}
extern "C" int b2_spmv_plan_destroy(b2_spmv_plan* p) { delete p; return B2_OK; }

constexpr int GB = 8;
__device__ __forceinline__ double col_dot(const int32_t* __restrict__ colptr, const int32_t* __restrict__ rowval,
                                          const double* __restrict__ nz, const double* __restrict__ x, int64_t j) {
    double s = 0.0;
    const int a = colptr[j], b = colptr[j + 1];
    for (int p0 = a; p0 < b; p0 += GB) {
        int ri[GB]; double nv[GB], xv[GB];
#pragma unroll
        for (int u = 0; u < GB; ++u) { ri[u] = (p0 + u < b) ? rowval[p0 + u] : -1; nv[u] = (p0 + u < b) ? nz[p0 + u] : 0.0; }
#pragma unroll
        for (int u = 0; u < GB; ++u) xv[u] = (ri[u] >= 0) ? x[ri[u]] : 0.0;
#pragma unroll
        for (int u = 0; u < GB; ++u) if (ri[u] >= 0) s = fma(nv[u], xv[u], s);
    }
    return s;
}
template <bool STRICT, int B = GB>
__device__ __forceinline__ double row_dot_t(const int32_t* __restrict__ rowptr, const int32_t* __restrict__ colidx,
                                            const int32_t* __restrict__ valmap, const double* __restrict__ nz,
                                            const double* __restrict__ x, int64_t i) {
    double s = 0.0;
    const int a = rowptr[i], b = rowptr[i + 1];
    for (int q0 = a; q0 < b; q0 += B) {
        int ci[B], vi[B]; double nv[B], xv[B];
#pragma unroll
        for (int u = 0; u < B; ++u) {
            const bool ok = q0 + u < b;
            ci[u] = ok ? colidx[q0 + u] : -1; vi[u] = ok ? valmap[q0 + u] : 0;
            if (STRICT && ci[u] == (int)i) ci[u] = -1;
        }
#pragma unroll
        for (int u = 0; u < B; ++u) { nv[u] = (ci[u] >= 0) ? nz[vi[u]] : 0.0; xv[u] = (ci[u] >= 0) ? x[ci[u]] : 0.0; }
#pragma unroll
        for (int u = 0; u < B; ++u) if (ci[u] >= 0) s = fma(nv[u], xv[u], s);
    }
    return s;
}
__device__ __forceinline__ double row_dot(const int32_t* __restrict__ rowptr, const int32_t* __restrict__ colidx,
                                          const int32_t* __restrict__ valmap, const double* __restrict__ nz,
                                          const double* __restrict__ x, int64_t i) {
    return row_dot_t<false>(rowptr, colidx, valmap, nz, x, i);
}
__device__ __forceinline__ double row_dot_strict(const int32_t* __restrict__ rowptr, const int32_t* __restrict__ colidx,
                                                 const int32_t* __restrict__ valmap, const double* __restrict__ nz,
                                                 const double* __restrict__ x, int64_t i) {
    return row_dot_t<true>(rowptr, colidx, valmap, nz, x, i);
}

__global__ void k_spmv_t(int64_t ncol, const int32_t* colptr, const int32_t* rowval, const double* nz, const double* x, double* y,
                         double alpha, double beta) {
    GRID_STRIDE(j, ncol) {
        const double s = col_dot(colptr, rowval, nz, x, j);
        y[j] = (beta == 0.0) ? alpha * s : alpha * s + beta * y[j];
    }
}
__global__ void k_spmv_n(int64_t nrow, const int32_t* rowptr, const int32_t* colidx, const int32_t* valmap, const double* nz,
                         const double* x, double* y, double alpha, double beta) {
    GRID_STRIDE(i, nrow) {
        const double s = row_dot(rowptr, colidx, valmap, nz, x, i);
        y[i] = (beta == 0.0) ? alpha * s : alpha * s + beta * y[i];
    }
}
__global__ void k_spmv_sym(int64_t n, const int32_t* colptr, const int32_t* rowval, const int32_t* rowptr, const int32_t* colidx,
                           const int32_t* valmap, const double* nz, const double* x, double* y, double alpha, double beta) {
    GRID_STRIDE(i, n) {
        const double s = col_dot(colptr, rowval, nz, x, i) + row_dot_strict(rowptr, colidx, valmap, nz, x, i);
        y[i] = (beta == 0.0) ? alpha * s : alpha * s + beta * y[i];
    }
}

extern "C" int b2_spmv_n(b2_spmv_plan* p, const double* nz_d, const double* x_d, double* y_d, double alpha, double beta, void* stream) {
    if (!p || !x_d || !y_d) { set_error("b2_spmv_n: invalid argument"); return B2_ERR_INVALID; }
    if (p->nrow == 0) return B2_OK;
    k_spmv_n<<<grid_elem(p->nrow), 256, 0, as_stream(stream)>>>(p->nrow, p->rowptr.p, p->colidx.p, p->valmap.p, nz_d, x_d, y_d, alpha, beta);
    B2_CUDA(cudaGetLastError());
    return B2_OK;
}
extern "C" int b2_spmv_t(b2_spmv_plan* p, const double* nz_d, const double* x_d, double* y_d, double alpha, double beta, void* stream) {
    if (!p || !x_d || !y_d) { set_error("b2_spmv_t: invalid argument"); return B2_ERR_INVALID; }
    if (p->ncol == 0) return B2_OK;
    k_spmv_t<<<grid_elem(p->ncol), 256, 0, as_stream(stream)>>>(p->ncol, p->colptr.p, p->rowval.p, nz_d, x_d, y_d, alpha, beta);
    B2_CUDA(cudaGetLastError());
    return B2_OK;
}
extern "C" int b2_spmv_symlower(b2_spmv_plan* p, const double* nz_d, const double* x_d, double* y_d, double alpha, double beta, void* stream) {
    if (!p || !x_d || !y_d || p->nrow != p->ncol) { set_error("b2_spmv_symlower: invalid argument"); return B2_ERR_INVALID; }
    if (p->nrow == 0) return B2_OK;
    k_spmv_sym<<<grid_elem(p->nrow), 256, 0, as_stream(stream)>>>(p->nrow, p->colptr.p, p->rowval.p, p->rowptr.p, p->colidx.p, p->valmap.p,
                                                                 nz_d, x_d, y_d, alpha, beta);
    B2_CUDA(cudaGetLastError());
    return B2_OK;
}

struct KktMulArgs {
    int64_t n_tot, m, nlb, nub;
    const int32_t *lbpos, *ubpos;
    const int64_t *ind_lb, *ind_ub;
    const double *reg, *du, *ll, *ul, *ld, *ud;
    double alpha, beta;
};
__device__ __forceinline__ double scl(double beta, double w) { return beta == 0.0 ? 0.0 : beta * w; }
__device__ __forceinline__ double kktmul_entry(const KktMulArgs& a, int64_t t, double wt, const double* __restrict__ x) {
    const double* xzl = x + a.n_tot + a.m;
    const double* xzu = xzl + a.nlb;
    if (t < a.n_tot) {
        double v = wt + a.alpha * a.reg[t] * x[t];
        const int p = a.lbpos[t], q = a.ubpos[t];
        if (p >= 0) v -= a.alpha * xzl[p];
        if (q >= 0) v += a.alpha * xzu[q];
        return v;
    }
    if (t < a.n_tot + a.m) return wt + a.alpha * a.du[t - a.n_tot] * x[t];
    if (t < a.n_tot + a.m + a.nlb) {
        const int64_t k = t - a.n_tot - a.m;
        return scl(a.beta, wt) + a.alpha * (x[a.ind_lb[k]] * a.ll[k] - xzl[k] * a.ld[k]);
    }
    const int64_t k = t - a.n_tot - a.m - a.nlb;
    return scl(a.beta, wt) + a.alpha * (x[a.ind_ub[k]] * a.ul[k] + xzu[k] * a.ud[k]);
}
__global__ void k_kktmul(KktMulArgs a, const double* __restrict__ x, double* __restrict__ w) {
    GRID_STRIDE(t, a.n_tot + a.m + a.nlb + a.nub) w[t] = kktmul_entry(a, t, w[t], x);
}
static KktMulArgs make_kktmul(b2_bounds* b, int64_t m, const double* reg, const double* du, const double* ll, const double* ul,
                              const double* ld, const double* ud, double alpha, double beta) {
    KktMulArgs a;
    a.n_tot = b->n_tot; a.m = m; a.nlb = b->nlb; a.nub = b->nub;
    a.lbpos = b->lbpos.p; a.ubpos = b->ubpos.p; a.ind_lb = b->ind_lb.p; a.ind_ub = b->ind_ub.p;
    a.reg = reg; a.du = du; a.ll = ll; a.ul = ul; a.ld = ld; a.ud = ud; a.alpha = alpha; a.beta = beta;
    return a;
}
extern "C" int b2_kktmul(b2_bounds* b, int64_t m, const double* reg_d, const double* du_diag_d, const double* l_lower_d,
                         const double* u_lower_d, const double* l_diag_d, const double* u_diag_d, double alpha, double beta,
                         const double* x_d, double* w_d, void* stream) {
    if (!b || !x_d || !w_d) { set_error("b2_kktmul: invalid argument"); return B2_ERR_INVALID; }
    KktMulArgs a = make_kktmul(b, m, reg_d, du_diag_d, l_lower_d, u_lower_d, l_diag_d, u_diag_d, alpha, beta);
    const int64_t tot = a.n_tot + a.m + a.nlb + a.nub;
    if (tot == 0) return B2_OK;
    k_kktmul<<<grid_elem(tot), 256, 0, as_stream(stream)>>>(a, x_d, w_d);
    B2_CUDA(cudaGetLastError());
    return B2_OK;
}

__global__ void k_scaled_set_aug_diagonal(int64_t n_tot, const int32_t* __restrict__ lbpos, const int32_t* __restrict__ ubpos,
                                          const double* __restrict__ reg, const double* __restrict__ ll, const double* __restrict__ ld,
                                          const double* __restrict__ ul, const double* __restrict__ ud, double* __restrict__ pr,
                                          double* __restrict__ sf) {
    pdl_sync();
    GRID_STRIDE(i, n_tot) {
        const int p = lbpos[i], q = ubpos[i];
        double xlzu = q >= 0 ? ul[q] : 0.0;
        double xuzl = p >= 0 ? ll[p] : 0.0;
        double s = 1.0;
        if (p >= 0) { xlzu = __dmul_rn(xlzu, ld[p]); s = __dmul_rn(s, __dsqrt_rn(ld[p])); }
        if (q >= 0) { xuzl = __dmul_rn(xuzl, ud[q]); s = __dmul_rn(s, __dsqrt_rn(ud[q])); }
        pr[i] = __dadd_rn(__dadd_rn(xlzu, xuzl), __dmul_rn(reg[i], __dmul_rn(s, s)));
        sf[i] = s;
    }
}
extern "C" int b2_scaled_set_aug_diagonal(b2_bounds* b, const double* reg_d, const double* l_lower_d, const double* l_diag_d,
                                          const double* u_lower_d, const double* u_diag_d, double* pr_diag_d, double* scaling_d,
                                          void* stream) {
    B2_NEED(b && (b->n_tot == 0 || (reg_d && pr_diag_d && scaling_d)), "b2_scaled_set_aug_diagonal");
    B2_NEED((b->nlb == 0 || (l_lower_d && l_diag_d)) && (b->nub == 0 || (u_lower_d && u_diag_d)), "b2_scaled_set_aug_diagonal");
    if (b->n_tot == 0) return B2_OK;
    launch_pdl(k_scaled_set_aug_diagonal, dim3(grid_elem(b->n_tot)), dim3(256), 0, as_stream(stream), b->n_tot, b->lbpos.p, b->ubpos.p,
               reg_d, l_lower_d, l_diag_d, u_lower_d, u_diag_d, pr_diag_d, scaling_d);
    B2_CUDA(cudaGetLastError());
    return B2_OK;
}

template <bool POST>
__global__ void k_scaled_solve(int64_t n_tot, int64_t m, int64_t nlb, const int32_t* __restrict__ lbpos, const int32_t* __restrict__ ubpos,
                               const double* __restrict__ ll, const double* __restrict__ ul, const double* __restrict__ ld,
                               const double* __restrict__ ud, const double* __restrict__ sf, double* __restrict__ w) {
    pdl_sync();
    double* wzl = w + n_tot + m;
    double* wzu = wzl + nlb;
    GRID_STRIDE(i, n_tot) {
        const int p = lbpos[i], q = ubpos[i];
        if (!POST) {
            double r3 = p >= 0 ? wzl[p] : 0.0;
            double r4 = q >= 0 ? wzu[q] : 0.0;
            if (q >= 0) r3 = __dmul_rn(r3, __dsqrt_rn(ud[q]));
            if (p >= 0) { r3 = __ddiv_rn(r3, __dsqrt_rn(ld[p])); r4 = __dmul_rn(r4, __dsqrt_rn(ld[p])); }
            if (q >= 0) r4 = __ddiv_rn(r4, __dsqrt_rn(ud[q]));
            w[i] = __dadd_rn(__dmul_rn(w[i], sf[i]), __dadd_rn(r3, r4));
        } else {
            const double x = __dmul_rn(w[i], sf[i]);
            w[i] = x;
            if (p >= 0) wzl[p] = __ddiv_rn(__dsub_rn(wzl[p], __dmul_rn(ll[p], x)), ld[p]);
            if (q >= 0) wzu[q] = __ddiv_rn(__dadd_rn(neg(wzu[q]), __dmul_rn(ul[q], x)), ud[q]);
        }
    }
}
template <bool POST>
static int scaled_solve(const char* name, b2_bounds* b, int64_t m, const double* ll, const double* ul, const double* ld, const double* ud,
                        const double* sf, double* w, void* stream) {
    if (!b || m < 0 || !w || (b->n_tot && !sf) || (b->nlb && (!ld || (POST && !ll))) || (b->nub && (!ud || (POST && !ul)))) {
        set_error(std::string(name) + ": invalid argument");
        return B2_ERR_INVALID;
    }
    if (b->n_tot == 0) return B2_OK;
    launch_pdl(k_scaled_solve<POST>, dim3(grid_elem(b->n_tot)), dim3(256), 0, as_stream(stream), b->n_tot, m, b->nlb, b->lbpos.p,
               b->ubpos.p, ll, ul, ld, ud, sf, w);
    B2_CUDA(cudaGetLastError());
    return B2_OK;
}
extern "C" int b2_scaled_solve_pre(b2_bounds* b, int64_t m, const double* l_diag_d, const double* u_diag_d, const double* scaling_d,
                                   double* w_d, void* stream) {
    return scaled_solve<false>("b2_scaled_solve_pre", b, m, nullptr, nullptr, l_diag_d, u_diag_d, scaling_d, w_d, stream);
}
extern "C" int b2_scaled_solve_post(b2_bounds* b, int64_t m, const double* l_lower_d, const double* u_lower_d, const double* l_diag_d,
                                    const double* u_diag_d, const double* scaling_d, double* w_d, void* stream) {
    return scaled_solve<true>("b2_scaled_solve_post", b, m, l_lower_d, u_lower_d, l_diag_d, u_diag_d, scaling_d, w_d, stream);
}

__global__ void k_scaled_kktmul(KktMulArgs a, const double* __restrict__ x, double* __restrict__ w) {
    const double* xzl = x + a.n_tot + a.m;
    const double* xzu = xzl + a.nlb;
    GRID_STRIDE(t, a.n_tot + a.m + a.nlb + a.nub) {
        const double wt = w[t];
        double v;
        if (t < a.n_tot) {
            v = __dadd_rn(wt, __dmul_rn(__dmul_rn(a.alpha, a.reg[t]), x[t]));
            const int p = a.lbpos[t], q = a.ubpos[t];
            if (p >= 0) v = __dsub_rn(v, __dmul_rn(a.alpha, xzl[p]));
            if (q >= 0) v = __dadd_rn(v, __dmul_rn(a.alpha, xzu[q]));
        } else if (t < a.n_tot + a.m) {
            v = __dadd_rn(wt, __dmul_rn(__dmul_rn(a.alpha, a.du[t - a.n_tot]), x[t]));
        } else if (t < a.n_tot + a.m + a.nlb) {
            const int64_t k = t - a.n_tot - a.m;
            v = __dadd_rn(scl(a.beta, wt), __dmul_rn(a.alpha, __dadd_rn(__dmul_rn(x[a.ind_lb[k]], a.ll[k]), __dmul_rn(xzl[k], a.ld[k]))));
        } else {
            const int64_t k = t - a.n_tot - a.m - a.nlb;
            v = __dadd_rn(scl(a.beta, wt), __dmul_rn(a.alpha, __dsub_rn(__dmul_rn(x[a.ind_ub[k]], a.ul[k]), __dmul_rn(xzu[k], a.ud[k]))));
        }
        w[t] = v;
    }
}
extern "C" int b2_scaled_kktmul(b2_bounds* b, int64_t m, const double* reg_d, const double* du_diag_d, const double* l_lower_d,
                                const double* u_lower_d, const double* l_diag_d, const double* u_diag_d, double alpha, double beta,
                                const double* x_d, double* w_d, void* stream) {
    B2_NEED(b && m >= 0 && x_d && w_d && (b->n_tot == 0 || reg_d) && (m == 0 || du_diag_d), "b2_scaled_kktmul");
    B2_NEED((b->nlb == 0 || (l_lower_d && l_diag_d)) && (b->nub == 0 || (u_lower_d && u_diag_d)), "b2_scaled_kktmul");
    KktMulArgs a = make_kktmul(b, m, reg_d, du_diag_d, l_lower_d, u_lower_d, l_diag_d, u_diag_d, alpha, beta);
    const int64_t tot = a.n_tot + a.m + a.nlb + a.nub;
    if (tot == 0) return B2_OK;
    k_scaled_kktmul<<<grid_elem(tot), 256, 0, as_stream(stream)>>>(a, x_d, w_d);
    B2_CUDA(cudaGetLastError());
    return B2_OK;
}

__global__ void k_scaled_regularize(int64_t n_tot, int64_t m, double dw, double dc, const double* __restrict__ sf, double* __restrict__ reg,
                                    double* __restrict__ pr, double* __restrict__ du) {
    GRID_STRIDE(i, n_tot + m) {
        if (i < n_tot) {
            const double s = sf[i];
            reg[i] = __dadd_rn(reg[i], dw);
            pr[i] = __dadd_rn(pr[i], __dmul_rn(dw, __dmul_rn(s, s)));
        } else {
            du[i - n_tot] = __dsub_rn(du[i - n_tot], dc);
        }
    }
}
extern "C" int b2_scaled_regularize_diagonal(int64_t n_tot, int64_t m, double dw, double dc, const double* scaling_d, double* reg_d,
                                             double* pr_diag_d, double* du_diag_d, void* stream) {
    B2_NEED(n_tot >= 0 && m >= 0 && (n_tot == 0 || (scaling_d && reg_d && pr_diag_d)) && (m == 0 || du_diag_d),
            "b2_scaled_regularize_diagonal");
    if (n_tot + m == 0) return B2_OK;
    k_scaled_regularize<<<grid_elem(n_tot + m), 256, 0, as_stream(stream)>>>(n_tot, m, dw, dc, scaling_d, reg_d, pr_diag_d, du_diag_d);
    B2_CUDA(cudaGetLastError());
    return B2_OK;
}

__device__ __forceinline__ void norm_inf_commit(double mx, unsigned long long* out) {
#pragma unroll
    for (int o = 16; o > 0; o >>= 1) { const double t = __shfl_xor_sync(0xffffffffu, mx, o); if (t > mx || t != t) mx = t; }
    if ((threadIdx.x & 31) == 0) atomicMax(out, (unsigned long long)__double_as_longlong(mx));
}

struct CondArgs {
    int64_t n, m, nlb;
    const int32_t *lbpos, *ubpos;
    const double *ld, *ud, *pr, *D;
};
__global__ void k_cond_pre1(CondArgs a, double* __restrict__ buffer, double* __restrict__ w, double* __restrict__ norms) {
    pdl_sync();
    if (norms && blockIdx.x == 0 && threadIdx.x == 0) { norms[0] = 0.0; norms[1] = 0.0; }
    const int64_t n_tot = a.n + a.m;
    const double* wzl = w + n_tot + a.m;
    const double* wzu = wzl + a.nlb;
    GRID_STRIDE(i, n_tot) {
        double v = w[i];
        const int p = a.lbpos[i], q = a.ubpos[i];
        if (p >= 0) v = __dsub_rn(v, __ddiv_rn(wzl[p], a.ld[p]));
        if (q >= 0) v = __dsub_rn(v, __ddiv_rn(wzu[q], a.ud[q]));
        if (p >= 0 || q >= 0) w[i] = v;
        if (i >= a.n) {
            const int64_t j = i - a.n;
            buffer[j] = a.D[j] * (w[n_tot + j] + v / a.pr[i]);
        }
    }
}
__global__ void k_cond_pre2(int64_t n, const int32_t* rowptr, const int32_t* colidx, const int32_t* valmap, const double* __restrict__ nz,
                            const double* __restrict__ buffer, double* w) {
    pdl_sync();
    GRID_STRIDE(i, n) w[i] += row_dot_t<false, 2 * GB>(rowptr, colidx, valmap, nz, buffer, i);
}

template <bool UPDATE>
__global__ void k_cond_post(CondArgs a, const int32_t* __restrict__ colptr, const int32_t* __restrict__ rowval, const double* __restrict__ nz,
                            const double* __restrict__ ll, const double* __restrict__ ul, const double* __restrict__ buffer, double* w,
                            double* __restrict__ x, unsigned long long* norm_x) {
    pdl_sync();
    const int64_t n = a.n, m = a.m, n_tot = n + m;
    double* dlb = w + n_tot + m;
    double* dub = dlb + a.nlb;
    double mx = 0.0;
    auto add_x = [&](int64_t t, double wt) {
        if (UPDATE) {
            const double xt = x[t] + wt;
            x[t] = xt;
            const double v = fabs(xt);
            if (v > mx || v != v) mx = v;
        }
    };
    GRID_STRIDE(t, m + n) {
        const int64_t i = t < m ? n + t : t - m;
        const int p = a.lbpos[i], q = a.ubpos[i];
        double wi;
        if (t < m) {
            const int64_t j = t;
            const double b2v = col_dot(colptr, rowval, nz, w, j);
            const double wz = fma(a.D[j], b2v, -buffer[j]);
            wi = __ddiv_rn(__dadd_rn(w[i], wz), a.pr[i]);
            w[n_tot + j] = wz;
            w[i] = wi;
            add_x(n_tot + j, wz);
        } else {
            wi = w[i];
        }
        add_x(i, wi);
        if (p >= 0) {
            const double d = __ddiv_rn(__dadd_rn(-dlb[p], __dmul_rn(ll[p], wi)), a.ld[p]);
            dlb[p] = d;
            add_x(n_tot + m + p, d);
        }
        if (q >= 0) {
            const double d = __ddiv_rn(__dsub_rn(dub[q], __dmul_rn(ul[q], wi)), a.ud[q]);
            dub[q] = d;
            add_x(n_tot + m + a.nlb + q, d);
        }
    }
    if (UPDATE) norm_inf_commit(mx, norm_x);
}

static CondArgs make_cond(b2_bounds* b, int64_t n, int64_t m, const double* l_diag, const double* u_diag, const double* pr,
                          const double* D) {
    CondArgs a;
    a.n = n; a.m = m; a.nlb = b->nlb; a.lbpos = b->lbpos.p; a.ubpos = b->ubpos.p;
    a.ld = l_diag; a.ud = u_diag; a.pr = pr; a.D = D;
    return a;
}
static int cond_pre(const char* name, b2_bounds* b, b2_spmv_plan* jt, int64_t n, int64_t m, const double* jt_nz_d, const double* pr_diag_d,
                    const double* diag_buffer_d, const double* l_diag_d, const double* u_diag_d, double* buffer_d, double* w_d,
                    double* norms_d, void* stream) {
    if (!b || !jt || !w_d || !buffer_d || b->n_tot != n + m || jt->nrow != n || jt->ncol != m) {
        set_error(std::string(name) + ": invalid argument");
        return B2_ERR_INVALID;
    }
    cudaStream_t st = as_stream(stream);
    launch_pdl(k_cond_pre1, dim3(grid_elem(n + m)), dim3(256), 0, st, make_cond(b, n, m, l_diag_d, u_diag_d, pr_diag_d, diag_buffer_d), buffer_d, w_d,
               norms_d);
    launch_pdl(k_cond_pre2, dim3(grid_elem(n)), dim3(256), 0, st, n, jt->rowptr.p, jt->colidx.p, jt->valmap.p, jt_nz_d, buffer_d, w_d);
    B2_CUDA(cudaGetLastError());
    return B2_OK;
}
template <bool UPDATE>
static int cond_post(const char* name, b2_bounds* b, b2_spmv_plan* jt, int64_t n, int64_t m, const double* jt_nz_d, const double* pr_diag_d,
                     const double* diag_buffer_d, const double* l_lower_d, const double* u_lower_d, const double* l_diag_d,
                     const double* u_diag_d, const double* buffer_d, double* w_d, double* x_d, double* norms_d, void* stream) {
    if (!b || !jt || !w_d || !buffer_d || b->n_tot != n + m || jt->nrow != n || jt->ncol != m || (UPDATE && (!x_d || !norms_d))) {
        set_error(std::string(name) + ": invalid argument");
        return B2_ERR_INVALID;
    }
    launch_pdl(k_cond_post<UPDATE>, dim3(grid_elem(n + m)), dim3(256), 0, as_stream(stream),
               make_cond(b, n, m, l_diag_d, u_diag_d, pr_diag_d, diag_buffer_d), jt->colptr.p, jt->rowval.p, jt_nz_d, l_lower_d, u_lower_d,
               buffer_d, w_d, x_d, (unsigned long long*)(UPDATE ? norms_d + 1 : nullptr));
    B2_CUDA(cudaGetLastError());
    return B2_OK;
}
extern "C" int b2_condensed_solve_pre(b2_bounds* b, b2_spmv_plan* jt, int64_t n, int64_t m, const double* jt_nz_d,
                                      const double* pr_diag_d, const double* diag_buffer_d, const double* l_diag_d,
                                      const double* u_diag_d, double* buffer_d, double* w_d, void* stream) {
    return cond_pre("b2_condensed_solve_pre", b, jt, n, m, jt_nz_d, pr_diag_d, diag_buffer_d, l_diag_d, u_diag_d, buffer_d, w_d, nullptr, stream);
}
extern "C" int b2_condensed_refine_pre(b2_bounds* b, b2_spmv_plan* jt, int64_t n, int64_t m, const double* jt_nz_d,
                                       const double* pr_diag_d, const double* diag_buffer_d, const double* l_diag_d,
                                       const double* u_diag_d, double* buffer_d, double* w_d, double* norms_d, void* stream) {
    if (!norms_d) { set_error("b2_condensed_refine_pre: invalid argument"); return B2_ERR_INVALID; }
    return cond_pre("b2_condensed_refine_pre", b, jt, n, m, jt_nz_d, pr_diag_d, diag_buffer_d, l_diag_d, u_diag_d, buffer_d, w_d, norms_d, stream);
}
extern "C" int b2_condensed_solve_post(b2_bounds* b, b2_spmv_plan* jt, int64_t n, int64_t m, const double* jt_nz_d,
                                       const double* pr_diag_d, const double* diag_buffer_d, const double* l_lower_d,
                                       const double* u_lower_d, const double* l_diag_d, const double* u_diag_d,
                                       const double* buffer_d, double* w_d, void* stream) {
    return cond_post<false>("b2_condensed_solve_post", b, jt, n, m, jt_nz_d, pr_diag_d, diag_buffer_d, l_lower_d, u_lower_d, l_diag_d, u_diag_d,
                            buffer_d, w_d, nullptr, nullptr, stream);
}
extern "C" int b2_condensed_solve_post_update(b2_bounds* b, b2_spmv_plan* jt, int64_t n, int64_t m, const double* jt_nz_d,
                                              const double* pr_diag_d, const double* diag_buffer_d, const double* l_lower_d,
                                              const double* u_lower_d, const double* l_diag_d, const double* u_diag_d,
                                              const double* buffer_d, double* w_d, double* x_d, double* norms_d, void* stream) {
    return cond_post<true>("b2_condensed_solve_post_update", b, jt, n, m, jt_nz_d, pr_diag_d, diag_buffer_d, l_lower_d, u_lower_d, l_diag_d,
                           u_diag_d, buffer_d, w_d, x_d, norms_d, stream);
}

struct CondMulArgs {
    int64_t n, m;
    const int32_t *h_colptr, *h_rowval, *h_rowptr, *h_colidx, *h_valmap;
    const int32_t *j_colptr, *j_rowval, *j_rowptr, *j_colidx, *j_valmap;
    const double *h_nz, *j_nz;
};
template <bool Y_IN>
__global__ void k_cond_mul(CondMulArgs c, KktMulArgs a, const double* __restrict__ x, const double* __restrict__ y, double* __restrict__ w,
                           unsigned long long* norm_out) {
    pdl_sync();
    const int64_t n = c.n, m = c.m;
    double mx = 0.0;
    const double* xs = x + n;
    const double* xz = x + n + m;
    GRID_STRIDE(t, a.n_tot + a.m + a.nlb + a.nub) {
        double wt = Y_IN ? y[t] : w[t];
        if (t < n) {
            const double hx = col_dot(c.h_colptr, c.h_rowval, c.h_nz, x, t) + row_dot_strict(c.h_rowptr, c.h_colidx, c.h_valmap, c.h_nz, x, t);
            const double jz = row_dot_t<false, 2 * GB>(c.j_rowptr, c.j_colidx, c.j_valmap, c.j_nz, xz, t);
            wt = a.alpha * hx + scl(a.beta, wt) + a.alpha * jz;
        } else if (t < n + m) {
            wt = scl(a.beta, wt) - a.alpha * xz[t - n];
        } else if (t < n + 2 * m) {
            const int64_t j = t - n - m;
            wt = a.alpha * col_dot(c.j_colptr, c.j_rowval, c.j_nz, x, j) + scl(a.beta, wt) - a.alpha * xs[j];
        }
        const double wv = kktmul_entry(a, t, wt, x);
        w[t] = wv;
        const double av = fabs(wv);
        if (av > mx || av != av) mx = av;
    }
    if (norm_out) norm_inf_commit(mx, norm_out);
}
static int cond_mul(b2_bounds* b, b2_spmv_plan* hess, b2_spmv_plan* jt, int64_t n, int64_t m, const double* hess_nz_d, const double* jt_nz_d,
                    const double* reg_d, const double* du_diag_d, const double* l_lower_d, const double* u_lower_d, const double* l_diag_d,
                    const double* u_diag_d, double alpha, double beta, const double* x_d, const double* y_d, double* w_d, double* norm_inf_d,
                    void* stream) {
    if (!b || !hess || !jt || !x_d || !w_d || b->n_tot != n + m || hess->nrow != n || jt->nrow != n || jt->ncol != m) {
        set_error("b2_condensed_kkt_mul: invalid argument");
        return B2_ERR_INVALID;
    }
    CondMulArgs c;
    c.n = n; c.m = m;
    c.h_colptr = hess->colptr.p; c.h_rowval = hess->rowval.p; c.h_rowptr = hess->rowptr.p; c.h_colidx = hess->colidx.p; c.h_valmap = hess->valmap.p;
    c.j_colptr = jt->colptr.p; c.j_rowval = jt->rowval.p; c.j_rowptr = jt->rowptr.p; c.j_colidx = jt->colidx.p; c.j_valmap = jt->valmap.p;
    c.h_nz = hess_nz_d; c.j_nz = jt_nz_d;
    KktMulArgs a = make_kktmul(b, m, reg_d, du_diag_d, l_lower_d, u_lower_d, l_diag_d, u_diag_d, alpha, beta);
    const int64_t tot = a.n_tot + a.m + a.nlb + a.nub;
    if (y_d) launch_pdl(k_cond_mul<true>, dim3(grid_elem(tot)), dim3(256), 0, as_stream(stream), c, a, x_d, y_d, w_d, (unsigned long long*)norm_inf_d);
    else launch_pdl(k_cond_mul<false>, dim3(grid_elem(tot)), dim3(256), 0, as_stream(stream), c, a, x_d, y_d, w_d, (unsigned long long*)norm_inf_d);
    B2_CUDA(cudaGetLastError());
    return B2_OK;
}
extern "C" int b2_condensed_kkt_mul_norm(b2_bounds* b, b2_spmv_plan* hess, b2_spmv_plan* jt, int64_t n, int64_t m,
                                    const double* hess_nz_d, const double* jt_nz_d, const double* reg_d, const double* du_diag_d,
                                    const double* l_lower_d, const double* u_lower_d, const double* l_diag_d, const double* u_diag_d,
                                    double alpha, double beta, const double* x_d, double* w_d, double* norm_inf_d, void* stream) {
    return cond_mul(b, hess, jt, n, m, hess_nz_d, jt_nz_d, reg_d, du_diag_d, l_lower_d, u_lower_d, l_diag_d, u_diag_d, alpha, beta, x_d,
                    nullptr, w_d, norm_inf_d, stream);
}
extern "C" int b2_condensed_kkt_mul_norm_y(b2_bounds* b, b2_spmv_plan* hess, b2_spmv_plan* jt, int64_t n, int64_t m,
                                      const double* hess_nz_d, const double* jt_nz_d, const double* reg_d, const double* du_diag_d,
                                      const double* l_lower_d, const double* u_lower_d, const double* l_diag_d, const double* u_diag_d,
                                      double alpha, double beta, const double* x_d, const double* y_d, double* w_d, double* norm_inf_d,
                                      void* stream) {
    if (!y_d || y_d == w_d) { set_error("b2_condensed_kkt_mul_norm_y: invalid argument (y must be a vector other than w)"); return B2_ERR_INVALID; }
    return cond_mul(b, hess, jt, n, m, hess_nz_d, jt_nz_d, reg_d, du_diag_d, l_lower_d, u_lower_d, l_diag_d, u_diag_d, alpha, beta, x_d,
                    y_d, w_d, norm_inf_d, stream);
}
extern "C" int b2_condensed_kkt_mul(b2_bounds* b, b2_spmv_plan* hess, b2_spmv_plan* jt, int64_t n, int64_t m,
                                    const double* hess_nz_d, const double* jt_nz_d, const double* reg_d, const double* du_diag_d,
                                    const double* l_lower_d, const double* u_lower_d, const double* l_diag_d, const double* u_diag_d,
                                    double alpha, double beta, const double* x_d, double* w_d, void* stream) {
    return b2_condensed_kkt_mul_norm(b, hess, jt, n, m, hess_nz_d, jt_nz_d, reg_d, du_diag_d, l_lower_d, u_lower_d, l_diag_d, u_diag_d, alpha,
                                     beta, x_d, w_d, nullptr, stream);
}

__global__ void k_norm_inf(int64_t n, const double* __restrict__ x, unsigned long long* out) {
    double mx = 0.0;
    GRID_STRIDE(i, n) { const double v = fabs(x[i]); if (v > mx || v != v) mx = v; }
    norm_inf_commit(mx, out);
}
__global__ void k_richardson_update(int64_t n, const double* __restrict__ b, double* __restrict__ w, double* __restrict__ x,
                                    unsigned long long* norm_x) {
    pdl_sync();
    double mx = 0.0;
    GRID_STRIDE(i, n) {
        const double xi = x[i] + w[i];
        x[i] = xi;
        w[i] = b[i];
        const double v = fabs(xi);
        if (v > mx || v != v) mx = v;
    }
    norm_inf_commit(mx, norm_x);
}
__global__ void k_richardson_begin(int64_t n, const double* __restrict__ b, double* __restrict__ w, double* __restrict__ x,
                                   unsigned long long* norm_b) {
    pdl_sync();
    double mx = 0.0;
    GRID_STRIDE(i, n) {
        const double bi = b[i];
        w[i] = bi;
        x[i] = 0.0;
        const double v = fabs(bi);
        if (v > mx || v != v) mx = v;
    }
    norm_inf_commit(mx, norm_b);
}
extern "C" int b2_richardson_begin(int64_t n, const double* b_d, double* w_d, double* x_d, double* norm_b_d, void* stream) {
    if (n < 0 || !norm_b_d || (n && (!b_d || !w_d || !x_d))) { set_error("b2_richardson_begin: invalid argument"); return B2_ERR_INVALID; }
    cudaStream_t st = as_stream(stream);
    B2_CUDA(cudaMemsetAsync(norm_b_d, 0, sizeof(double), st));
    if (n) k_richardson_begin<<<grid_elem(n), 256, 0, st>>>(n, b_d, w_d, x_d, (unsigned long long*)norm_b_d);
    B2_CUDA(cudaGetLastError());
    return B2_OK;
}
extern "C" int b2_richardson_update(int64_t n, const double* b_d, double* w_d, double* x_d, double* norms_d, void* stream) {
    if (n < 0 || !norms_d || (n && (!b_d || !w_d || !x_d))) { set_error("b2_richardson_update: invalid argument"); return B2_ERR_INVALID; }
    cudaStream_t st = as_stream(stream);
    B2_CUDA(cudaMemsetAsync(norms_d, 0, 2 * sizeof(double), st));
    if (n) launch_pdl(k_richardson_update, dim3(grid_elem(n)), dim3(256), 0, st, n, b_d, w_d, x_d, (unsigned long long*)(norms_d + 1));
    B2_CUDA(cudaGetLastError());
    return B2_OK;
}
extern "C" int b2_norm_inf(int64_t n, const double* x_d, double* out_d, void* stream) {
    if (n < 0 || !out_d || (n && !x_d)) { set_error("b2_norm_inf: invalid argument"); return B2_ERR_INVALID; }
    cudaStream_t st = as_stream(stream);
    B2_CUDA(cudaMemsetAsync(out_d, 0, sizeof(double), st));
    if (n) k_norm_inf<<<grid_elem(n), 256, 0, st>>>(n, x_d, (unsigned long long*)out_d);
    B2_CUDA(cudaGetLastError());
    return B2_OK;
}
__global__ void k_axpy(int64_t n, double a, const double* __restrict__ x, double* __restrict__ y) { GRID_STRIDE(i, n) y[i] += a * x[i]; }
__global__ void k_copy(int64_t n, const double* __restrict__ x, double* __restrict__ y) { GRID_STRIDE(i, n) y[i] = x[i]; }
__global__ void k_fill(int64_t n, double v, double* __restrict__ x) { GRID_STRIDE(i, n) x[i] = v; }
extern "C" int b2_axpy(int64_t n, double a, const double* x_d, double* y_d, void* stream) {
    if (n < 0 || (n && (!x_d || !y_d))) return B2_ERR_INVALID;
    if (n) k_axpy<<<grid_elem(n), 256, 0, as_stream(stream)>>>(n, a, x_d, y_d);
    B2_CUDA(cudaGetLastError());
    return B2_OK;
}
extern "C" int b2_copy(int64_t n, const double* x_d, double* y_d, void* stream) {
    if (n < 0 || (n && (!x_d || !y_d))) return B2_ERR_INVALID;
    if (n) k_copy<<<grid_elem(n), 256, 0, as_stream(stream)>>>(n, x_d, y_d);
    B2_CUDA(cudaGetLastError());
    return B2_OK;
}
struct CopyManyArgs { const double* src[16]; double* dst[16]; int64_t n[16]; };
__global__ void k_copy_many(CopyManyArgs c) {
    const double* __restrict__ x = c.src[blockIdx.y];
    double* __restrict__ y = c.dst[blockIdx.y];
    const int64_t n = c.n[blockIdx.y];
    GRID_STRIDE(i, n) y[i] = x[i];
}
extern "C" int b2_copy_many(int32_t count, const double* const* src_d, double* const* dst_d, const int64_t* n, void* stream) {
    if (count < 0 || count > 16 || (count && (!src_d || !dst_d || !n))) { set_error("b2_copy_many: invalid argument (at most 16 segments)"); return B2_ERR_INVALID; }
    if (count == 0) return B2_OK;
    CopyManyArgs c;
    int64_t nmax = 0;
    for (int k = 0; k < 16; ++k) {
        const bool on = k < count;
        if (on && (n[k] < 0 || (n[k] && (!src_d[k] || !dst_d[k])))) { set_error("b2_copy_many: invalid segment"); return B2_ERR_INVALID; }
        c.src[k] = on ? src_d[k] : nullptr; c.dst[k] = on ? dst_d[k] : nullptr; c.n[k] = on ? n[k] : 0;
        if (on) nmax = std::max(nmax, n[k]);
    }
    if (nmax == 0) return B2_OK;
    const int gx = (int)std::max<int64_t>(1, std::min<int64_t>((nmax + 255) / 256, 2 * sm_count()));
    k_copy_many<<<dim3(gx, count), 256, 0, as_stream(stream)>>>(c);
    B2_CUDA(cudaGetLastError());
    return B2_OK;
}
extern "C" int b2_fill(int64_t n, double v, double* x_d, void* stream) {
    if (n < 0 || (n && !x_d)) return B2_ERR_INVALID;
    if (n) k_fill<<<grid_elem(n), 256, 0, as_stream(stream)>>>(n, v, x_d);
    B2_CUDA(cudaGetLastError());
    return B2_OK;
}

__device__ __forceinline__ double scl2(double beta, double w) { return beta == 0.0 ? 0.0 : beta * w; }

constexpr int GEMV_ROWS = 32;
__global__ void __launch_bounds__(256) k_gemv_n(int rows, int cols, int lda, const double* __restrict__ A, const double* __restrict__ x,
                                                double* __restrict__ y, double alpha, double beta) {
    __shared__ double part[8][GEMV_ROWS];
    const int lane = threadIdx.x & 31, warp = threadIdx.x >> 5;
    const int i = blockIdx.x * GEMV_ROWS + lane;
    const bool ok = i < rows;
    const double* base = A + (ok ? i : 0);
    double acc = 0.0;
    int j = warp * 8;
    for (; j + 8 <= cols; j += 64) {
        double v[8], xv[8];
#pragma unroll
        for (int u = 0; u < 8; ++u) { v[u] = ok ? base[(size_t)(j + u) * lda] : 0.0; xv[u] = x[j + u]; }
#pragma unroll
        for (int u = 0; u < 8; ++u) acc = fma(v[u], xv[u], acc);
    }
    if (j < cols) {
        for (int u = 0; j + u < cols; ++u) acc = fma(ok ? base[(size_t)(j + u) * lda] : 0.0, x[j + u], acc);
    }
    part[warp][lane] = acc;
    __syncthreads();
    if (warp == 0 && ok) {
        double tot = 0.0;
#pragma unroll
        for (int q = 0; q < 8; ++q) tot += part[q][lane];
        y[i] = alpha * tot + scl2(beta, y[i]);
    }
}
__global__ void __launch_bounds__(256) k_gemv_t(int rows, int cols, int lda, const double* __restrict__ A, const double* __restrict__ x,
                                                double* __restrict__ y, double alpha, double beta) {
    const int lane = threadIdx.x & 31;
    const int j = blockIdx.x * 8 + (threadIdx.x >> 5);
    if (j >= cols) return;
    const double* col = A + (size_t)j * lda;
    double acc = 0.0;
    int i = lane;
    for (; i + 7 * 32 < rows; i += 8 * 32) {
        double v[8];
#pragma unroll
        for (int u = 0; u < 8; ++u) v[u] = col[i + 32 * u];
#pragma unroll
        for (int u = 0; u < 8; ++u) acc = fma(v[u], x[i + 32 * u], acc);
    }
    for (; i < rows; i += 32) acc = fma(col[i], x[i], acc);
#pragma unroll
    for (int o = 16; o > 0; o >>= 1) acc += __shfl_xor_sync(0xffffffffu, acc, o);
    if (lane == 0) y[j] = alpha * acc + scl2(beta, y[j]);
}
__global__ void __launch_bounds__(256) k_symv_lower_cols(int n, int lda, const double* __restrict__ A, const double* __restrict__ x,
                                                         double* __restrict__ y, double alpha, double beta) {
    const int lane = threadIdx.x & 31;
    const int j = blockIdx.x * 8 + (threadIdx.x >> 5);
    if (j >= n) return;
    const double* col = A + (size_t)j * lda;
    double acc = 0.0;
    int i = j + lane;
    for (; i + 7 * 32 < n; i += 8 * 32) {
        double v[8];
#pragma unroll
        for (int u = 0; u < 8; ++u) v[u] = col[i + 32 * u];
#pragma unroll
        for (int u = 0; u < 8; ++u) acc = fma(v[u], x[i + 32 * u], acc);
    }
    for (; i < n; i += 32) acc = fma(col[i], x[i], acc);
#pragma unroll
    for (int o = 16; o > 0; o >>= 1) acc += __shfl_xor_sync(0xffffffffu, acc, o);
    if (lane == 0) y[j] = alpha * acc + scl2(beta, y[j]);
}
__global__ void __launch_bounds__(256) k_symv_lower_rows(int n, int lda, const double* __restrict__ A, const double* __restrict__ x,
                                                         double* __restrict__ y, double alpha) {
    __shared__ double part[8][GEMV_ROWS];
    const int lane = threadIdx.x & 31, warp = threadIdx.x >> 5;
    const int r0 = blockIdx.x * GEMV_ROWS, i = r0 + lane;
    const bool ok = i < n;
    const double* base = A + (ok ? i : 0);
    const int jend = min(n, r0 + GEMV_ROWS);
    double acc = 0.0;
    for (int j = warp * 8; j < jend; j += 64) {
        double v[8], xv[8];
#pragma unroll
        for (int u = 0; u < 8; ++u) {
            const int jj = j + u;
            const bool use = ok && jj < i;
            v[u] = use ? base[(size_t)jj * lda] : 0.0;
            xv[u] = use ? x[jj] : 0.0;
        }
#pragma unroll
        for (int u = 0; u < 8; ++u) acc = fma(v[u], xv[u], acc);
    }
    part[warp][lane] = acc;
    __syncthreads();
    if (warp == 0 && ok) {
        double tot = 0.0;
#pragma unroll
        for (int q = 0; q < 8; ++q) tot += part[q][lane];
        y[i] += alpha * tot;
    }
}
static inline void launch_symv_lower(int n, int lda, const double* A, const double* x, double* y, double alpha, double beta, cudaStream_t st) {
    k_symv_lower_cols<<<(n + 7) / 8, 256, 0, st>>>(n, lda, A, x, y, alpha, beta);
    k_symv_lower_rows<<<(n + GEMV_ROWS - 1) / GEMV_ROWS, 256, 0, st>>>(n, lda, A, x, y, alpha);
}

extern "C" int b2d_gemv_n(int32_t rows, int32_t cols, int32_t lda, const double* A_d, const double* x_d, double* y_d, double alpha,
                          double beta, void* stream) {
    if (rows < 0 || cols < 0 || lda < rows || (rows && (!y_d || (cols && (!A_d || !x_d))))) { set_error("b2d_gemv_n: invalid argument"); return B2_ERR_INVALID; }
    if (rows == 0) return B2_OK;
    k_gemv_n<<<(rows + GEMV_ROWS - 1) / GEMV_ROWS, 256, 0, as_stream(stream)>>>(rows, cols, lda, A_d, x_d, y_d, alpha, beta);
    B2_CUDA(cudaGetLastError());
    return B2_OK;
}
extern "C" int b2d_gemv_t(int32_t rows, int32_t cols, int32_t lda, const double* A_d, const double* x_d, double* y_d, double alpha,
                          double beta, void* stream) {
    if (rows < 0 || cols < 0 || lda < rows || (cols && (!y_d || (rows && (!A_d || !x_d))))) { set_error("b2d_gemv_t: invalid argument"); return B2_ERR_INVALID; }
    if (cols == 0) return B2_OK;
    k_gemv_t<<<(cols + 7) / 8, 256, 0, as_stream(stream)>>>(rows, cols, lda, A_d, x_d, y_d, alpha, beta);
    B2_CUDA(cudaGetLastError());
    return B2_OK;
}
extern "C" int b2d_symv_lower(int32_t n, int32_t lda, const double* A_d, const double* x_d, double* y_d, double alpha, double beta,
                              void* stream) {
    if (n < 0 || lda < n || (n && (!A_d || !x_d || !y_d))) { set_error("b2d_symv_lower: invalid argument"); return B2_ERR_INVALID; }
    if (n == 0) return B2_OK;
    launch_symv_lower(n, lda, A_d, x_d, y_d, alpha, beta, as_stream(stream));
    B2_CUDA(cudaGetLastError());
    return B2_OK;
}

struct b2d_kkt {
    int32_t n = 0, m = 0, ns = 0, n_eq = 0;
    b2::DevBuf<int64_t> ind_ineq, ind_eq;
    b2::DevBuf<int32_t> ineq_pos;
};

extern "C" int b2d_kkt_create(int32_t n, int32_t m, int32_t ns, const int64_t* ind_ineq_h, b2d_kkt** out) {
    if (!out || n < 0 || m < 0 || ns < 0 || ns > m || (ns && !ind_ineq_h)) { set_error("b2d_kkt_create: invalid argument"); return B2_ERR_INVALID; }
    std::vector<int32_t> pos(std::max(m, 1), -1);
    for (int32_t k = 0; k < ns; ++k) {
        if (ind_ineq_h[k] < 0 || ind_ineq_h[k] >= m || pos[ind_ineq_h[k]] != -1) { set_error("b2d_kkt_create: bad ind_ineq"); return B2_ERR_INVALID; }
        pos[ind_ineq_h[k]] = k;
    }
    std::vector<int64_t> eq;
    for (int32_t j = 0; j < m; ++j) if (pos[j] < 0) eq.push_back(j);
    auto* k = new b2d_kkt();
    k->n = n; k->m = m; k->ns = ns; k->n_eq = m - ns;
    if (k->ind_ineq.upload(ind_ineq_h, ns) != cudaSuccess || k->ind_eq.upload(eq.data(), eq.size()) != cudaSuccess ||
        k->ineq_pos.upload(pos.data(), pos.size()) != cudaSuccess) {
        delete k;
        return cuda_fail(cudaGetLastError(), "b2d_kkt upload", __FILE__, __LINE__);
    }
    *out = k;
    return B2_OK;
}
extern "C" int b2d_kkt_destroy(b2d_kkt* k) { delete k; return B2_OK; }

__global__ void k_dcond_pre(int n, int m, int ns, int n_eq, int64_t nlb, const int32_t* __restrict__ lbpos, const int32_t* __restrict__ ubpos,
                            const int64_t* __restrict__ ind_ineq, const int64_t* __restrict__ ind_eq, const double* __restrict__ ld,
                            const double* __restrict__ ud, const double* __restrict__ pr, const double* __restrict__ D,
                            double* __restrict__ buffer, double* __restrict__ x, double* __restrict__ w) {
    const int64_t n_tot = (int64_t)n + ns;
    const double* wzl = w + n_tot + m;
    const double* wzu = wzl + nlb;
    GRID_STRIDE(t, n_tot + n_eq) {
        if (t < n_tot) {
            double v = w[t];
            const int p = lbpos[t], q = ubpos[t];
            if (p >= 0) v = __dsub_rn(v, __ddiv_rn(wzl[p], ld[p]));
            if (q >= 0) v = __dsub_rn(v, __ddiv_rn(wzu[q], ud[q]));
            if (p >= 0 || q >= 0) w[t] = v;
            if (t < n) x[t] = v;
            else {
                const int64_t k = t - n, j = ind_ineq[k];
                buffer[j] = __dmul_rn(D[k], __dadd_rn(w[n_tot + j], __ddiv_rn(v, pr[t])));
            }
        } else {
            const int64_t e = t - n_tot, j = ind_eq[e];
            buffer[j] = 0.0;
            x[n + e] = w[n_tot + j];
        }
    }
}

__global__ void k_dcond_post(int n, int m, int ns, int n_eq, const int64_t* __restrict__ ind_ineq, const int64_t* __restrict__ ind_eq,
                             const double* __restrict__ pr, const double* __restrict__ D, const double* __restrict__ buffer,
                             const double* __restrict__ x, double* __restrict__ w) {
    const int64_t n_tot = (int64_t)n + ns;
    GRID_STRIDE(t, n_tot + n_eq) {
        if (t < n) w[t] = x[t];
        else if (t < n_tot) {
            const int64_t k = t - n, j = ind_ineq[k];
            const double wz = __dsub_rn(__dmul_rn(w[n_tot + j], D[k]), buffer[j]);
            w[n_tot + j] = wz;
            w[t] = __ddiv_rn(__dadd_rn(w[t], wz), pr[t]);
        } else {
            const int64_t e = t - n_tot, j = ind_eq[e];
            w[n_tot + j] = x[n + e];
// ... 67 lines not shown
```

### madnlp.jl_b200/kkt.py

```python
from __future__ import annotations

import ctypes as C

import numpy as np
import torch

from . import capi
from .capi import lib, check, ptr
from .linear_solvers import B200DenseSolver, B200SparseSolver, DeviceCSC
from .quasi_newton import BFGS, CompactLBFGS, DampedBFGS, ExactHessian

_DEV = "cuda"


def _dz(n):
    return torch.zeros(int(n), dtype=torch.float64, device=_DEV)


def force_lower_triangular(I, J):
    sw = J > I
    tmp = J[sw].copy()
    J[sw] = I[sw]
    I[sw] = tmp

# ... 141 lines not shown
    def set_aug_diagonal_(self):
        check(lib.b2_set_aug_diagonal(self._bounds.h, ptr(self.reg), ptr(self.l_lower), ptr(self.l_diag),
                                      ptr(self.u_lower), ptr(self.u_diag), ptr(self.pr_diag), self.stream_ptr()))

    def regularize_diagonal(self, primal, dual):
        check(lib.b2_regularize_diagonal(self._n_tot, self._m, float(primal), float(dual), ptr(self.reg),
                                         ptr(self.pr_diag), ptr(self.du_diag), self.stream_ptr()))

    def reduce_rhs(self, w):
        check(lib.b2_reduce_rhs(self._bounds.h, self._m, ptr(self.l_diag), ptr(self.u_diag), ptr(w.values), self.stream_ptr()))

    def finish_aug_solve(self, w):
        check(lib.b2_finish_aug_solve(self._bounds.h, self._m, ptr(self.l_lower), ptr(self.u_lower), ptr(self.l_diag),
                                      ptr(self.u_diag), ptr(w.values), self.stream_ptr()))

    def _kktmul(self, w, x, alpha, beta):
        check(lib.b2_kktmul(self._bounds.h, self._m, ptr(self.reg), ptr(self.du_diag), ptr(self.l_lower), ptr(self.u_lower),
                            ptr(self.l_diag), ptr(self.u_diag), float(alpha), float(beta), ptr(x.values), ptr(w.values),
                            self.stream_ptr()))

    def factorize_kkt(self):
        return self.linear_solver.factorize()

    def get_kkt(self):
        return self.aug_com

    def is_inertia_correct(self, num_pos, num_zero, num_neg):
        return num_zero == 0 and num_pos == self.num_variables()

    def should_regularize_dual(self, num_pos, num_zero, num_neg):
        return num_zero != 0

    def _initialize_common(self):
        self.reg.fill_(1.0); self.pr_diag.fill_(1.0); self.du_diag.zero_(); self.hess.zero_()

    _unreduced = 0
    _curv = None

    def _hess_mul(self, wx, t):
        raise NotImplementedError

    def _hess_blk(self, wx, t, n=None, g=None, tol=0.0, result=None):
        for v in (wx, t) + ((n, g) if result is not None else ()):
            if v.numel() != self._n_tot:
                raise ValueError(f"mul_hess_blk: vectors must have n_tot = {self._n_tot} entries, got {v.numel()}")
        n_h = self._hess_mul(wx, t)
        check(lib.b2_mul_hess_blk_tail(self._bounds.h, n_h, self._unreduced, ptr(self.pr_diag), ptr(self.l_lower), ptr(self.l_diag),
                                       ptr(self.u_lower), ptr(self.u_diag), ptr(t), ptr(wx), ptr(n), ptr(g), float(tol), ptr(result),
                                       self.stream_ptr()))

    def mul_hess_blk(self, wx, t):
        self._hess_blk(wx, t)
        return wx

    def curv_test(self, t, n, g, wx, tol=0.0):
        if self._curv is None:
            self._curv = _dz(capi.CURV_RESULT_LEN)
        self._hess_blk(wx, t, n, g, tol, self._curv)
        return self._curv


class _SparseKKTBase(_KKTBase):

    def _build(self, cb, linear_solver, opt_linear_solver, unreduced, diagonal_hessian=False):
        n, m = cb.nvar, cb.ncon
        ns = len(cb.ind_ineq)
        if diagonal_hessian:
            hI = np.arange(n, dtype=np.int64); hJ = np.arange(n, dtype=np.int64)
        else:
            hI = np.array(cb.hess_I, dtype=np.int64); hJ = np.array(cb.hess_J, dtype=np.int64)
        force_lower_triangular(hI, hJ)
        jI = np.asarray(cb.jac_I, dtype=np.int64); jJ = np.asarray(cb.jac_J, dtype=np.int64)
        n_jac, n_hess = len(jI), len(hI)
        n_tot = n + ns
        nlb, nub = (len(cb.ind_lb), len(cb.ind_ub)) if unreduced else (0, 0)
        self.n, self.m, self.ns, self.n_tot = n, m, ns, n_tot
        L = n_tot + m + n_hess + n_jac + ns + 2 * nlb + 2 * nub
        o1 = n_tot; o2 = o1 + n_hess; o3 = o2 + n_jac; o4 = o3 + ns; o5 = o4 + m
        I = np.empty(L, dtype=np.int64); J = np.empty(L, dtype=np.int64)
        ineq = np.asarray(cb.ind_ineq, dtype=np.int64)
        I[:o1] = np.arange(n_tot); J[:o1] = np.arange(n_tot)
        I[o1:o2] = hI; J[o1:o2] = hJ
        I[o2:o3] = jI + n_tot; J[o2:o3] = jJ
        I[o3:o4] = ineq + n_tot; J[o3:o4] = np.arange(n, n + ns)
        I[o4:o5] = np.arange(n_tot, n_tot + m); J[o4:o5] = np.arange(n_tot, n_tot + m)
        self.V = _dz(L)
        self.pr_diag = self.V[:o1]
        self.hess = self.V[o1:o2]
        self.jac = self.V[o2:o4]
        self.jac_callback = self.V[o2:o3]
        self.du_diag = self.V[o4:o5]
        N = n_tot + m
        if unreduced:
            lb_rows = N + np.arange(nlb); ub_rows = N + nlb + np.arange(nub)
            o6 = o5 + nlb; o7 = o6 + nlb; o8 = o7 + nub
            I[o5:o6] = lb_rows; J[o5:o6] = lb_rows
            I[o6:o7] = lb_rows; J[o6:o7] = np.asarray(cb.ind_lb, dtype=np.int64)
            I[o7:o8] = ub_rows; J[o7:o8] = ub_rows
            I[o8:] = ub_rows; J[o8:] = np.asarray(cb.ind_ub, dtype=np.int64)
            N += nlb + nub
        self._init_common(cb, n_tot, m)
        if unreduced:
            self.l_diag, self.l_lower_aug = self.V[o5:o6], self.V[o6:o7]
            self.u_diag, self.u_lower_aug = self.V[o7:o8], self.V[o8:]
        self.N = N
        cp, rv, mp = coo_to_csc(I, J, N, N)
        self.aug_com = DeviceCSC(N, N, cp, rv, _dz(len(rv)))
        self._aug_plan = _transfer_plan(mp, len(rv))
        self.aug_csc_map = mp
        jI2 = np.concatenate([jI, ineq]); jJ2 = np.concatenate([jJ, np.arange(n, n + ns)])
        cp, rv, mp = coo_to_csc(jI2, jJ2, m, n_tot)
        self.jac_com = DeviceCSC(m, n_tot, cp, rv, _dz(len(rv)))
        self._jac_plan = _transfer_plan(mp, len(rv))
        self._jac_spmv = _spmv_plan(m, n_tot, cp, rv)
        cp, rv, mp = coo_to_csc(hI, hJ, n_tot, n_tot)
        self.hess_com = DeviceCSC(n_tot, n_tot, cp, rv, _dz(len(rv)))
        self._hess_plan = _transfer_plan(mp, len(rv))
        self._hess_spmv = _spmv_plan(n_tot, n_tot, cp, rv)
        if opt_linear_solver is None and hasattr(linear_solver, "default_options"):
            opt_linear_solver = linear_solver.default_options()
        if opt_linear_solver is not None and getattr(opt_linear_solver, "kkt_n_primal", None) == 0:
            opt_linear_solver.kkt_n_primal = n_tot
        if unreduced and opt_linear_solver is not None and getattr(opt_linear_solver, "kkt_n_dual", None) == 0:
            opt_linear_solver.kkt_n_dual = m
        self.linear_solver = linear_solver(self.aug_com, opt_linear_solver)

    def num_variables(self):
        return len(self.pr_diag)

    def inertia_rule(self):
        return self.num_variables(), None

    def dual_rule(self):
        return False

    def get_jacobian(self):
        return self.jac_callback

    def get_hessian(self):
        return self.hess

    def compress_jacobian(self):
        if self.ns:
            check(lib.b2_fill(self.ns, -1.0, ptr(self.jac[-self.ns:]), self.stream_ptr()))
        check(lib.b2_transfer(self._jac_plan.h, ptr(self.jac_com.nzval), ptr(self.jac), self.stream_ptr()))

    def compress_hessian(self):
        check(lib.b2_transfer(self._hess_plan.h, ptr(self.hess_com.nzval), ptr(self.hess), self.stream_ptr()))

    def build_kkt(self):
        check(lib.b2_transfer(self._aug_plan.h, ptr(self.aug_com.nzval), ptr(self.V), self.stream_ptr()))

    def mul(self, w, x, alpha=1.0, beta=0.0):
        sp = self.stream_ptr()
        check(lib.b2_spmv_symlower(self._hess_spmv.h, ptr(self.hess_com.nzval), ptr(x.values), ptr(w.values), alpha, beta, sp))
        check(lib.b2_spmv_t(self._jac_spmv.h, ptr(self.jac_com.nzval), ptr(x.dual()), ptr(w.values), alpha, 1.0, sp))
        check(lib.b2_spmv_n(self._jac_spmv.h, ptr(self.jac_com.nzval), ptr(x.values), ptr(w.dual()), alpha, beta, sp))
        self._mul_lowrank(w, x, alpha)
        self._kktmul(w, x, alpha, beta)
        return w

    def _mul_lowrank(self, w, x, alpha):
        pass

    def _hess_mul(self, wx, t):
        check(lib.b2_spmv_symlower(self._hess_spmv.h, ptr(self.hess_com.nzval), ptr(t), ptr(wx), 1.0, 0.0, self.stream_ptr()))
        return self.hess_com.n

    def jtprod(self, y, x):
        check(lib.b2_spmv_t(self._jac_spmv.h, ptr(self.jac_com.nzval), ptr(x), ptr(y), 1.0, 0.0, self.stream_ptr()))


class SparseKKTSystem(_SparseKKTBase):

    def __init__(self, cb, linear_solver=B200SparseSolver, opt_linear_solver=None, hessian_approximation=ExactHessian,
                 qn_options=None):
        lbfgs = hessian_approximation is CompactLBFGS
        if not lbfgs and hessian_approximation is not ExactHessian:
            raise ValueError(f"unsupported hessian_approximation {hessian_approximation!r}")
        if lbfgs and opt_linear_solver is not None and getattr(opt_linear_solver, "n_parts", 1) > 1:
            raise ValueError("CompactLBFGS is not supported with a sharded linear solver (n_parts > 1)")
        self._build(cb, linear_solver, opt_linear_solver, unreduced=False, diagonal_hessian=lbfgs)
        self.quasi_newton = CompactLBFGS(self.n, qn_options) if lbfgs else ExactHessian()
        self._lbfgs = lbfgs
        if lbfgs:
            self.quasi_newton.stream = self.stream
            self.smw_H = torch.zeros((2 * self.quasi_newton.max_mem, self.N), dtype=torch.float64, device=_DEV)

    def factorize_kkt(self):
        self.linear_solver.factorize()
        if self._lbfgs:
            self.quasi_newton.smw_prepare(self.linear_solver, self.smw_H)
        return self.linear_solver

    def _mul_lowrank(self, w, x, alpha):
        if self._lbfgs:
            self.quasi_newton.mul_lowrank(alpha, x.values, w.values)

    def initialize(self):
        self._initialize_common()
        self.l_lower.zero_(); self.u_lower.zero_(); self.l_diag.fill_(1.0); self.u_diag.fill_(1.0)
        self.hess_com.nzval.zero_()

    def solve_kkt(self, w: UnreducedKKTVector):
        self.reduce_rhs(w)
        self.linear_solver.solve_linear_system(w.primal_dual())
        if self._lbfgs:
            self.quasi_newton.smw_apply(self.smw_H, w.primal_dual())
        self.finish_aug_solve(w)
        return w


class SparseUnreducedKKTSystem(_SparseKKTBase):
    _unreduced = 1

    def __init__(self, cb, linear_solver=B200SparseSolver, opt_linear_solver=None):
        self._build(cb, linear_solver, opt_linear_solver, unreduced=True)

    def initialize(self):
        self._initialize_common()
        self.l_lower.zero_(); self.u_lower.zero_(); self.l_diag.fill_(-1.0); self.u_diag.fill_(-1.0)
        self.l_lower_aug.zero_(); self.u_lower_aug.zero_()
        self.hess_com.nzval.zero_()

    def set_aug_diagonal_(self):
        check(lib.b2_set_aug_diagonal_unreduced(self._n_tot, len(self.l_lower), len(self.u_lower), ptr(self.reg), ptr(self.l_lower),
                                                ptr(self.u_lower), ptr(self.pr_diag), ptr(self.l_lower_aug), ptr(self.u_lower_aug),
                                                self.stream_ptr()))

    def solve_kkt(self, w: UnreducedKKTVector):
        args = (self._n_tot, self._m, len(self.l_lower), len(self.u_lower), ptr(self.l_lower_aug), ptr(self.u_lower_aug), ptr(w.values),
                self.stream_ptr())
        check(lib.b2_unreduced_solve_pre(*args))
        self.linear_solver.solve_linear_system(w.full())
        check(lib.b2_unreduced_solve_post(*args))
        return w


class ScaledSparseKKTSystem(_SparseKKTBase):
    _scaled = True

    def __init__(self, cb, linear_solver=B200SparseSolver, opt_linear_solver=None):
        self._build(cb, linear_solver, opt_linear_solver, unreduced=False)
        self.quasi_newton = ExactHessian()
        self.scaling_factor = _dz(self.n_tot)
        self._aug_colptr_d = torch.from_numpy(np.ascontiguousarray(self.aug_com.colptr, dtype=np.int32)).to(_DEV)
        self._aug_rowval_d = torch.from_numpy(np.ascontiguousarray(self.aug_com.rowval, dtype=np.int32)).to(_DEV)

    def initialize(self):
        self._initialize_common()
        self.l_lower.zero_(); self.u_lower.zero_(); self.l_diag.fill_(1.0); self.u_diag.fill_(1.0)
        self.scaling_factor.fill_(1.0)
        self.hess_com.nzval.zero_()

    def set_aug_diagonal_(self):
        check(lib.b2_scaled_set_aug_diagonal(self._bounds.h, ptr(self.reg), ptr(self.l_lower), ptr(self.l_diag), ptr(self.u_lower),
                                             ptr(self.u_diag), ptr(self.pr_diag), ptr(self.scaling_factor), self.stream_ptr()))

    def build_kkt(self):
        check(lib.b2_scaled_transfer(self._aug_plan.h, self.N, self._n_tot, ptr(self._aug_colptr_d), ptr(self._aug_rowval_d),
                                     ptr(self.scaling_factor), ptr(self.aug_com.nzval), ptr(self.V), self.stream_ptr()))

    def regularize_diagonal(self, primal, dual):
        check(lib.b2_scaled_regularize_diagonal(self._n_tot, self._m, float(primal), float(dual), ptr(self.scaling_factor),
                                                ptr(self.reg), ptr(self.pr_diag), ptr(self.du_diag), self.stream_ptr()))

    def solve_kkt(self, w: UnreducedKKTVector):
        sp = self.stream_ptr()
        check(lib.b2_scaled_solve_pre(self._bounds.h, self._m, ptr(self.l_diag), ptr(self.u_diag), ptr(self.scaling_factor),
                                      ptr(w.values), sp))
        self.linear_solver.solve_linear_system(w.primal_dual())
        check(lib.b2_scaled_solve_post(self._bounds.h, self._m, ptr(self.l_lower), ptr(self.u_lower), ptr(self.l_diag),
                                       ptr(self.u_diag), ptr(self.scaling_factor), ptr(w.values), sp))
        return w

    def _kktmul(self, w, x, alpha, beta):
        check(lib.b2_scaled_kktmul(self._bounds.h, self._m, ptr(self.reg), ptr(self.du_diag), ptr(self.l_lower), ptr(self.u_lower),
                                   ptr(self.l_diag), ptr(self.u_diag), float(alpha), float(beta), ptr(x.values), ptr(w.values),
                                   self.stream_ptr()))

    def _hess_blk(self, *args, **kwargs):
        raise ValueError("mul_hess_blk!: not supported by the KKT formulation ScaledSparseKKTSystem (the inertia-free test needs it)")


class SparseCondensedKKTSystem(_KKTBase):

    def __init__(self, cb, linear_solver=B200SparseSolver, opt_linear_solver=None):
        n, m = cb.nvar, cb.ncon
        ns = len(cb.ind_ineq)
        if ns != m:
            raise ValueError("SparseCondensedKKTSystem does not support equality constrained NLPs.")
        hI = np.array(cb.hess_I, dtype=np.int64); hJ = np.array(cb.hess_J, dtype=np.int64)
        force_lower_triangular(hI, hJ)
        jI = np.asarray(cb.jac_I, dtype=np.int64); jJ = np.asarray(cb.jac_J, dtype=np.int64)
        self.n, self.m, self.ns, self.n_tot = n, m, ns, n + ns
        self.pr_diag = _dz(n + ns); self.du_diag = _dz(m)
        self._init_common(cb, n + ns, m)
        self.buffer = _dz(m); self.buffer2 = _dz(m); self.diag_buffer = _dz(m)
        self.hess = _dz(len(hI)); self.jac = _dz(len(jI))
        dev_sym = _symbolic_on_device()
        coo_to_csc = coo_to_csc_device if dev_sym else globals()["coo_to_csc"]
        cp, rv, mp = coo_to_csc(jJ, jI, n, m)
        self.jt_csc = DeviceCSC(n, m, cp, rv, _dz(len(rv)))
        self._jt_plan = _transfer_plan(mp, len(rv))
        self._jt_spmv = _spmv_plan(n, m, cp, rv)
        hcp, hrv, hmp = coo_to_csc(hI, hJ, n, n)
        self.hess_com = DeviceCSC(n, n, hcp, hrv, _dz(len(hrv)))
        self._hess_plan = _transfer_plan(hmp, len(hrv))
        self._hess_spmv = _spmv_plan(n, n, hcp, hrv)
        h = C.c_void_p(); nnz_aug = C.c_int64(0)
        if dev_sym:
            d32 = lambda a: torch.from_numpy(np.ascontiguousarray(a if len(a) else np.zeros(1), dtype=np.int32)).to(_DEV)
            pats = [d32(hcp), d32(hrv), d32(cp), d32(rv)]
            check(lib.b2_condensed_symbolic_device(n, m, ptr(pats[0]), ptr(pats[1]), ptr(pats[2]), ptr(pats[3]), C.byref(h),
                                                   C.byref(nnz_aug), capi.stream_ptr()))
        else:
            check(lib.b2_condensed_symbolic(n, m, hcp.ctypes.data, hrv.ctypes.data if len(hrv) else None, cp.ctypes.data,
                                            rv.ctypes.data if len(rv) else None, C.byref(h), C.byref(nnz_aug)))
        self._cond = _Plan(h, lib.b2_condensed_plan_destroy)
        acp = np.zeros(n + 1, dtype=np.int32); arv = np.zeros(nnz_aug.value, dtype=np.int32)
        check(lib.b2_condensed_pattern(h, acp.ctypes.data, arv.ctypes.data))
        self.aug_com = DeviceCSC(n, n, acp, arv, _dz(nnz_aug.value))
        self.N = n
        self.linear_solver = linear_solver(self.aug_com, opt_linear_solver)

    def plan_sizes(self):
        a, b, c = C.c_int64(), C.c_int64(), C.c_int64()
        check(lib.b2_condensed_plan_sizes(self._cond.h, C.byref(a), C.byref(b), C.byref(c)))
        return dict(dptr=a.value, hptr=b.value, jptr=c.value)

    def num_variables(self):
        return len(self.pr_diag)

    def initialize(self):
        self._initialize_common()
        self.l_lower.zero_(); self.u_lower.zero_(); self.l_diag.fill_(1.0); self.u_diag.fill_(1.0)
        self.hess_com.nzval.zero_()

    def get_jacobian(self):
        return self.jac

    def get_hessian(self):
        return self.hess

    def compress_jacobian(self):
        check(lib.b2_transfer(self._jt_plan.h, ptr(self.jt_csc.nzval), ptr(self.jac), self.stream_ptr()))

    def compress_hessian(self):
        check(lib.b2_transfer(self._hess_plan.h, ptr(self.hess_com.nzval), ptr(self.hess), self.stream_ptr()))

    def build_kkt(self):
        check(lib.b2_condensed_assemble(self._cond.h, ptr(self.aug_com.nzval), ptr(self.pr_diag), ptr(self.du_diag),
                                        ptr(self.hess_com.nzval), ptr(self.jt_csc.nzval), ptr(self.diag_buffer),
                                        self.stream_ptr()))

    def is_inertia_correct(self, num_pos, num_zero, num_neg):
        return num_zero == 0 and num_pos == self.n

    def inertia_rule(self):
        return self.n, None

    def should_regularize_dual(self, num_pos, num_zero, num_neg):
        return True

    def dual_rule(self):
        return True

    def _pre_args(self):
        return (self._bounds.h, self._jt_spmv.h, self.n, self.m, ptr(self.jt_csc.nzval), ptr(self.pr_diag), ptr(self.diag_buffer))

    def _post_args(self):
        return self._pre_args() + (ptr(self.l_lower), ptr(self.u_lower), ptr(self.l_diag), ptr(self.u_diag), ptr(self.buffer))

    def _mul_args(self):
        return (self._bounds.h, self._hess_spmv.h, self._jt_spmv.h, self.n, self.m, ptr(self.hess_com.nzval), ptr(self.jt_csc.nzval),
                ptr(self.reg), ptr(self.du_diag), ptr(self.l_lower), ptr(self.u_lower), ptr(self.l_diag), ptr(self.u_diag))

    def solve_kkt(self, w: UnreducedKKTVector):
        sp = self.stream_ptr()
        check(lib.b2_condensed_solve_pre(*self._pre_args(), ptr(self.l_diag), ptr(self.u_diag), ptr(self.buffer), ptr(w.values), sp))
        self.linear_solver.solve_linear_system(w.values[: self.n])
        check(lib.b2_condensed_solve_post(*self._post_args(), ptr(w.values), sp))
        return w

    def refine_step(self, x, b, w, norms):
        sp = self.stream_ptr()
        check(lib.b2_condensed_refine_pre(*self._pre_args(), ptr(self.l_diag), ptr(self.u_diag), ptr(self.buffer), ptr(w.values),
                                          ptr(norms), sp))
        self.linear_solver.solve_linear_system(w.values[: self.n])
        check(lib.b2_condensed_solve_post_update(*self._post_args(), ptr(w.values), ptr(x.values), ptr(norms), sp))
        check(lib.b2_condensed_kkt_mul_norm_y(*self._mul_args(), -1.0, 1.0, ptr(x.values), ptr(b.values), ptr(w.values), ptr(norms), sp))

    def mul(self, w, x, alpha=1.0, beta=0.0):
        check(lib.b2_condensed_kkt_mul(*self._mul_args(), float(alpha), float(beta), ptr(x.values), ptr(w.values), self.stream_ptr()))
        return w

    def mul_norm(self, w, x, alpha, beta, norm_out):
        check(lib.b2_condensed_kkt_mul_norm(*self._mul_args(), float(alpha), float(beta), ptr(x.values), ptr(w.values), ptr(norm_out),
                                            self.stream_ptr()))
        return w

    def _hess_mul(self, wx, t):
        check(lib.b2_spmv_symlower(self._hess_spmv.h, ptr(self.hess_com.nzval), ptr(t), ptr(wx), 1.0, 0.0, self.stream_ptr()))
        return self.n

    def jtprod(self, y, x):
        check(lib.b2_spmv_n(self._jt_spmv.h, ptr(self.jt_csc.nzval), ptr(x), ptr(y), 1.0, 0.0, self.stream_ptr()))
        y[self.n:] = -x


class _DenseKKTBase(_KKTBase):

    @staticmethod
    def _check_hessian_approximation(hessian_approximation):
        if hessian_approximation is not ExactHessian and hessian_approximation not in (BFGS, DampedBFGS):
            raise ValueError(f"unsupported hessian_approximation {hessian_approximation!r}")

    def _init_quasi_newton(self, hessian_approximation, qn_options):
        if hessian_approximation is ExactHessian:
            self.quasi_newton = ExactHessian()
        else:
            self.quasi_newton = hessian_approximation(self.n, qn_options, stream=self.stream)

    def get_jacobian(self):
        return self.jac

    def get_hessian(self):
        return self.hess

    def set_dense(self, hess_np=None, jac_np=None):
        if hess_np is not None:
            self.hess.copy_(torch.from_numpy(np.ascontiguousarray(hess_np.T)))
        if jac_np is not None:
            self.jac.copy_(torch.from_numpy(np.ascontiguousarray(jac_np.T)))

    def compress_jacobian(self):
        pass

    def _gemv(self, trans, x, y, alpha, beta):
        fn = lib.b2d_gemv_t if trans else lib.b2d_gemv_n
        check(fn(self.m, self.n, self.m, ptr(self.jac), ptr(x), ptr(y), float(alpha), float(beta), self.stream_ptr()))

    def mul(self, w, x, alpha=1.0, beta=0.0):
        check(lib.b2d_kkt_mul(self._dk.h, self._bounds.h, ptr(self.hess), ptr(self.jac), ptr(self.reg), ptr(self.du_diag),
                              ptr(self.l_lower), ptr(self.u_lower), ptr(self.l_diag), ptr(self.u_diag), float(alpha), float(beta),
                              ptr(x.values), ptr(w.values), self.stream_ptr()))
        return w

    def _hess_mul(self, wx, t):
        check(lib.b2d_symv_lower(self.n, self.n, ptr(self.hess), ptr(t), ptr(wx), 1.0, 0.0, self.stream_ptr()))
        return self.n

    def jtprod(self, y, x):
        self._gemv(True, x, y[: self.n], 1.0, 0.0)
        y[self.n:] = -x[self._ind_ineq_d]


class DenseCondensedKKTSystem(_DenseKKTBase):

    def __init__(self, cb, linear_solver=B200DenseSolver, opt_linear_solver=None, hessian_approximation=ExactHessian,
                 qn_options=None):
        self._check_hessian_approximation(hessian_approximation)
        n, m = cb.nvar, cb.ncon
        ind_ineq = np.asarray(cb.ind_ineq, dtype=np.int64)
        ind_eq = np.setdiff1d(np.arange(m), ind_ineq).astype(np.int64)
        ns = len(ind_ineq); n_eq = m - ns
        self.n, self.m, self.ns, self.n_eq = n, m, ns, n_eq
        N = n + n_eq
        self.N = N
        self.aug_com = torch.zeros((N, N), dtype=torch.float64, device=_DEV)
        self.hess = torch.zeros((n, n), dtype=torch.float64, device=_DEV)
        self.jac = torch.zeros((n, m), dtype=torch.float64, device=_DEV)
        self.pr_diag = _dz(n + ns); self.du_diag = _dz(m)
        self._init_common(cb, n + ns, m)
        self.l_diag.fill_(1.0); self.u_diag.fill_(1.0)
        self.pd_buffer = _dz(N); self.diag_buffer = _dz(ns); self.buffer = _dz(m)
        self.ind_eq = ind_eq
        self._ind_ineq_d = torch.from_numpy(ind_ineq).to(_DEV)
        self._ind_eq_d = torch.from_numpy(ind_eq).to(_DEV)
        h = C.c_void_p()
        ii = np.ascontiguousarray(ind_ineq, dtype=np.int64)
        check(lib.b2d_kkt_create(n, m, ns, ii.ctypes.data if ns else None, C.byref(h)))
        self._dk = _Plan(h, lib.b2d_kkt_destroy)
        import os
        want = os.environ.get("B2_OZAKI")
        use = (n >= 512 and 256 <= ns <= 16384) if want is None else (want != "0" and 0 < ns <= 16384)
        self._ozaki = None
        if use:
            hz = C.c_void_p()
            check(lib.b2d_ozaki_plan_create(n, ns, C.byref(hz)))
            self._ozaki = _Plan(hz, lib.b2d_ozaki_plan_destroy)
        self.linear_solver = linear_solver(self.aug_com, opt_linear_solver)
        self._init_quasi_newton(hessian_approximation, qn_options)

    def num_variables(self):
        return self.n

    def initialize(self):
        self._initialize_common()

    def compress_hessian(self):
        pass

    def build_kkt(self):
        if self._ozaki is not None:
            check(lib.b2d_condensed_assemble_ozaki(self._ozaki.h, self.n, self.m, self.ns, self.n_eq, ptr(self._ind_ineq_d), ptr(self._ind_eq_d),
                                                   ptr(self.hess), ptr(self.jac), ptr(self.pr_diag), ptr(self.du_diag),
                                                   ptr(self.diag_buffer), ptr(self.aug_com), self.stream_ptr()))
            return
        check(lib.b2d_condensed_assemble(self.n, self.m, self.ns, self.n_eq, ptr(self._ind_ineq_d), ptr(self._ind_eq_d),
                                         ptr(self.hess), ptr(self.jac), ptr(self.pr_diag), ptr(self.du_diag),
                                         ptr(self.diag_buffer), ptr(self.aug_com), self.stream_ptr()))

    def tensor_core_status(self):
        if self._ozaki is None:
            return None
        t = C.c_int32(0)
        check(lib.b2d_ozaki_plan_status(self._ozaki.h, C.byref(t), self.stream_ptr()))
        return t.value == 0

    def is_inertia_correct(self, num_pos, num_zero, num_neg):
        return num_zero == 0 and num_neg == self.n_eq

    def solve_kkt(self, w: UnreducedKKTVector):
        sp = self.stream_ptr()
        check(lib.b2d_kkt_solve_pre(self._dk.h, self._bounds.h, ptr(self.jac), ptr(self.pr_diag), ptr(self.diag_buffer),
                                    ptr(self.l_diag), ptr(self.u_diag), ptr(self.buffer), ptr(self.pd_buffer), ptr(w.values), sp))
        self.linear_solver.solve_linear_system(self.pd_buffer)
        check(lib.b2d_kkt_solve_post(self._dk.h, self._bounds.h, ptr(self.jac), ptr(self.pr_diag), ptr(self.diag_buffer),
                                     ptr(self.l_lower), ptr(self.u_lower), ptr(self.l_diag), ptr(self.u_diag), ptr(self.buffer),
                                     ptr(self.pd_buffer), ptr(w.values), sp))
        return w



class DenseKKTSystem(_DenseKKTBase):

    def __init__(self, cb, linear_solver=B200DenseSolver, opt_linear_solver=None, hessian_approximation=ExactHessian,
                 qn_options=None):
        self._check_hessian_approximation(hessian_approximation)
        n, m = cb.nvar, cb.ncon
        ind_ineq = np.asarray(cb.ind_ineq, dtype=np.int64)
        ns = len(ind_ineq)
        self.n, self.m, self.ns = n, m, ns
        N = n + ns + m
        self.N = N
        self.aug_com = torch.zeros((N, N), dtype=torch.float64, device=_DEV)
        self.hess = torch.zeros((n, n), dtype=torch.float64, device=_DEV)
        self.jac = torch.zeros((n, m), dtype=torch.float64, device=_DEV)
        self.pr_diag = _dz(n + ns); self.du_diag = _dz(m); self.diag_hess = _dz(n)
        self._init_common(cb, n + ns, m)
        self.l_diag.fill_(1.0); self.u_diag.fill_(1.0)
        self._ind_ineq_d = torch.from_numpy(ind_ineq).to(_DEV)
        h = C.c_void_p()
        check(lib.b2d_kkt_create(n, m, ns, ind_ineq.ctypes.data if ns else None, C.byref(h)))
        self._dk = _Plan(h, lib.b2d_kkt_destroy)
        self.linear_solver = linear_solver(self.aug_com, opt_linear_solver)
        self._init_quasi_newton(hessian_approximation, qn_options)

    def num_variables(self):
        return len(self.pr_diag)

    def initialize(self):
        self._initialize_common()

    def compress_hessian(self):
        check(lib.b2d_copy_diag(self.n, self.n, ptr(self.hess), ptr(self.diag_hess), self.stream_ptr()))

    def build_kkt(self):
        check(lib.b2d_aug_assemble(self.n, self.m, self.ns, ptr(self._ind_ineq_d), ptr(self.hess), ptr(self.jac),
                                   ptr(self.pr_diag), ptr(self.du_diag), ptr(self.diag_hess), ptr(self.aug_com), self.stream_ptr()))

    def solve_kkt(self, w: UnreducedKKTVector):
        self.reduce_rhs(w)
        self.linear_solver.solve_linear_system(w.primal_dual())
        self.finish_aug_solve(w)
        return w

    def mul_aug(self, y, x):
        check(lib.b2d_symv_lower(self.N, self.N, ptr(self.aug_com), ptr(x), ptr(y), 1.0, 0.0, self.stream_ptr()))
        return y


_QN_UNSUPPORTED = {SparseUnreducedKKTSystem: "SparseUnreducedKKTSystem", SparseCondensedKKTSystem: "SparseCondensedKKTSystem",
                   ScaledSparseKKTSystem: "ScaledSparseKKTSystem"}


def create_kkt_system(kkt_type, cb, linear_solver=None, opt_linear_solver=None, hessian_approximation=ExactHessian,
                      qn_options=None):
    dense = kkt_type in (DenseCondensedKKTSystem, DenseKKTSystem)
    if linear_solver is None:
        linear_solver = B200DenseSolver if dense else B200SparseSolver
    if hessian_approximation in (BFGS, DampedBFGS):
        if not dense:
            raise ValueError("[options] DENSE_BFGS and DENSE_DAMPED_BFGS quasi-Newton approximations\n"
                             "require a dense KKT system (DENSE_KKT_SYSTEM or DENSE_CONDENSED_KKT_SYSTEM).")
        return kkt_type(cb, linear_solver, opt_linear_solver, hessian_approximation=hessian_approximation, qn_options=qn_options)
    if hessian_approximation is not ExactHessian:
        if kkt_type is not SparseKKTSystem:
            name = _QN_UNSUPPORTED.get(kkt_type, kkt_type.__name__)
            raise ValueError(f"Quasi-Newton approximation of the Hessian is not supported by the KKT formulation {name}. "
                             "Please use SparseKKTSystem instead.")
        return kkt_type(cb, linear_solver, opt_linear_solver, hessian_approximation=hessian_approximation, qn_options=qn_options)
    return kkt_type(cb, linear_solver, opt_linear_solver)
```

Baseline: 1993.

## Keep row-major copies of Hessian and Jacobian values for row-wise SpMV

```diff
diff --git a/include/b200kkt.h b/include/b200kkt.h
--- a/include/b200kkt.h
+++ b/include/b200kkt.h
@@ -223,6 +223,7 @@
 typedef struct b2_spmv_plan b2_spmv_plan;
 int b2_spmv_plan_create(int32_t nrow, int32_t ncol, const int32_t* colptr_h, const int32_t* rowval_h, b2_spmv_plan** out);
 int b2_spmv_plan_destroy(b2_spmv_plan* p);
+int b2_transfer_rows(b2_transfer_plan* p, b2_spmv_plan* sp, double* dst_nz_d, double* dst_row_d, const double* V_d, void* stream);
 int b2_spmv_n(b2_spmv_plan* p, const double* nz_d, const double* x_d, double* y_d, double alpha, double beta, void* stream);
 int b2_spmv_t(b2_spmv_plan* p, const double* nz_d, const double* x_d, double* y_d, double alpha, double beta, void* stream);
 int b2_spmv_symlower(b2_spmv_plan* p, const double* nz_d, const double* x_d, double* y_d, double alpha, double beta, void* stream);
@@ -232,31 +233,31 @@
               double alpha, double beta, const double* x_d, double* w_d, void* stream);
 
 int b2_condensed_solve_pre(b2_bounds* b, b2_spmv_plan* jt, int64_t n, int64_t m,
-                           const double* jt_nz_d, const double* pr_diag_d, const double* diag_buffer_d,
+                           const double* jt_nz_row_d, const double* pr_diag_d, const double* diag_buffer_d,
                            const double* l_diag_d, const double* u_diag_d, double* buffer_d, double* w_d, void* stream);
 int b2_condensed_solve_post(b2_bounds* b, b2_spmv_plan* jt, int64_t n, int64_t m,
                             const double* jt_nz_d, const double* pr_diag_d, const double* diag_buffer_d,
                             const double* l_lower_d, const double* u_lower_d, const double* l_diag_d, const double* u_diag_d,
                             const double* buffer_d, double* w_d, void* stream);
 int b2_condensed_refine_pre(b2_bounds* b, b2_spmv_plan* jt, int64_t n, int64_t m,
-                            const double* jt_nz_d, const double* pr_diag_d, const double* diag_buffer_d,
+                            const double* jt_nz_row_d, const double* pr_diag_d, const double* diag_buffer_d,
                             const double* l_diag_d, const double* u_diag_d, double* buffer_d, double* w_d, double* norms_d, void* stream);
 int b2_condensed_solve_post_update(b2_bounds* b, b2_spmv_plan* jt, int64_t n, int64_t m,
                                    const double* jt_nz_d, const double* pr_diag_d, const double* diag_buffer_d,
                                    const double* l_lower_d, const double* u_lower_d, const double* l_diag_d, const double* u_diag_d,
                                    const double* buffer_d, double* w_d, double* x_d, double* norms_d, void* stream);
 int b2_condensed_kkt_mul(b2_bounds* b, b2_spmv_plan* hess, b2_spmv_plan* jt, int64_t n, int64_t m,
-                         const double* hess_nz_d, const double* jt_nz_d,
+                         const double* hess_nz_d, const double* jt_nz_d, const double* hess_nz_row_d, const double* jt_nz_row_d,
                          const double* reg_d, const double* du_diag_d, const double* l_lower_d, const double* u_lower_d,
                          const double* l_diag_d, const double* u_diag_d, double alpha, double beta,
                          const double* x_d, double* w_d, void* stream);
 int b2_condensed_kkt_mul_norm(b2_bounds* b, b2_spmv_plan* hess, b2_spmv_plan* jt, int64_t n, int64_t m,
-                         const double* hess_nz_d, const double* jt_nz_d,
+                         const double* hess_nz_d, const double* jt_nz_d, const double* hess_nz_row_d, const double* jt_nz_row_d,
                          const double* reg_d, const double* du_diag_d, const double* l_lower_d, const double* u_lower_d,
                          const double* l_diag_d, const double* u_diag_d, double alpha, double beta,
                          const double* x_d, double* w_d, double* norm_inf_d, void* stream);
 int b2_condensed_kkt_mul_norm_y(b2_bounds* b, b2_spmv_plan* hess, b2_spmv_plan* jt, int64_t n, int64_t m,
-                           const double* hess_nz_d, const double* jt_nz_d,
+                           const double* hess_nz_d, const double* jt_nz_d, const double* hess_nz_row_d, const double* jt_nz_row_d,
                            const double* reg_d, const double* du_diag_d, const double* l_lower_d, const double* u_lower_d,
                            const double* l_diag_d, const double* u_diag_d, double alpha, double beta,
                            const double* x_d, const double* y_d, double* w_d, double* norm_inf_d, void* stream);
diff --git a/madnlp.jl_b200/capi.py b/madnlp.jl_b200/capi.py
--- a/madnlp.jl_b200/capi.py
+++ b/madnlp.jl_b200/capi.py
@@ -183,6 +183,7 @@
     "b2_transfer_plan_create": (C.c_int, [_i64, _i64, _p, _PP]),
     "b2_transfer_plan_destroy": (C.c_int, [_p]),
     "b2_transfer": (C.c_int, [_p, _p, _p, _p]),
+    "b2_transfer_rows": (C.c_int, [_p, _p, _p, _p, _p, _p]),
     "b2_condensed_symbolic": (C.c_int, [_i32, _i32, _p, _p, _p, _p, _PP, C.POINTER(_i64)]),
     "b2_condensed_pattern": (C.c_int, [_p, _p, _p]),
     "b2_condensed_plan_sizes": (C.c_int, [_p, C.POINTER(_i64), C.POINTER(_i64), C.POINTER(_i64)]),
@@ -214,11 +215,11 @@
     "b2_kktmul": (C.c_int, [_p, _i64, _p, _p, _p, _p, _p, _p, _f64, _f64, _p, _p, _p]),
     "b2_condensed_solve_pre": (C.c_int, [_p, _p, _i64, _i64, _p, _p, _p, _p, _p, _p, _p, _p]),
     "b2_condensed_solve_post": (C.c_int, [_p, _p, _i64, _i64, _p, _p, _p, _p, _p, _p, _p, _p, _p, _p]),
-    "b2_condensed_kkt_mul": (C.c_int, [_p, _p, _p, _i64, _i64, _p, _p, _p, _p, _p, _p, _p, _p, _f64, _f64, _p, _p, _p]),
-    "b2_condensed_kkt_mul_norm": (C.c_int, [_p, _p, _p, _i64, _i64, _p, _p, _p, _p, _p, _p, _p, _p, _f64, _f64, _p, _p, _p, _p]),
+    "b2_condensed_kkt_mul": (C.c_int, [_p, _p, _p, _i64, _i64, _p, _p, _p, _p, _p, _p, _p, _p, _p, _p, _f64, _f64, _p, _p, _p]),
+    "b2_condensed_kkt_mul_norm": (C.c_int, [_p, _p, _p, _i64, _i64, _p, _p, _p, _p, _p, _p, _p, _p, _p, _p, _f64, _f64, _p, _p, _p, _p]),
     "b2_condensed_refine_pre": (C.c_int, [_p, _p, _i64, _i64, _p, _p, _p, _p, _p, _p, _p, _p, _p]),
     "b2_condensed_solve_post_update": (C.c_int, [_p, _p, _i64, _i64, _p, _p, _p, _p, _p, _p, _p, _p, _p, _p, _p, _p]),
-    "b2_condensed_kkt_mul_norm_y": (C.c_int, [_p, _p, _p, _i64, _i64, _p, _p, _p, _p, _p, _p, _p, _p, _f64, _f64, _p, _p, _p, _p, _p]),
+    "b2_condensed_kkt_mul_norm_y": (C.c_int, [_p, _p, _p, _i64, _i64, _p, _p, _p, _p, _p, _p, _p, _p, _p, _p, _f64, _f64, _p, _p, _p, _p, _p]),
     "b2_get_alpha_max": (C.c_int, [_p, _p, _p, _p, _p, _f64, _p, _p]),
     "b2_get_alpha_z": (C.c_int, [_p, _p, _p, _p, _p, _f64, _p, _p]),
     "b2_get_varphi": (C.c_int, [_p, _f64, _p, _p, _p, _f64, _p, _p]),
diff --git a/madnlp.jl_b200/csrc/assembly.cu b/madnlp.jl_b200/csrc/assembly.cu
--- a/madnlp.jl_b200/csrc/assembly.cu
+++ b/madnlp.jl_b200/csrc/assembly.cu
@@ -6,6 +6,7 @@
 
 #include "common.cuh"
 #include "condensed_plan.cuh"
+#include "spmv_plan.cuh"
 
 using namespace b2;
 
@@ -83,11 +84,35 @@
 
 extern "C" int b2_transfer_plan_destroy(b2_transfer_plan* p) { delete p; return B2_OK; }
 
+__global__ void k_transfer_rows(int64_t nslot, const int32_t* __restrict__ ptr, const int32_t* __restrict__ src,
+                                const int32_t* __restrict__ rowpos, const double* __restrict__ V, double* __restrict__ dst,
+                                double* __restrict__ dst_row) {
+    pdl_sync();
+    for (int64_t i = (int64_t)blockIdx.x * blockDim.x + threadIdx.x; i < nslot; i += (int64_t)gridDim.x * blockDim.x) {
+        const int a = ptr[i], b = ptr[i + 1];
+        double acc = 0.0;
+        for (int q = a; q < b; ++q) acc = __dadd_rn(acc, V[src[q]]);
+        dst[i] = acc;
+        dst_row[rowpos[i]] = acc;
+    }
+}
+
 extern "C" int b2_transfer(b2_transfer_plan* p, double* dst_nz_d, const double* V_d, void* stream) {
     if (!p || !dst_nz_d || !V_d) { set_error("b2_transfer: invalid argument"); return B2_ERR_INVALID; }
     if (p->nnz_csc == 0) return B2_OK;
     const int grid = (int)std::min<int64_t>((p->nnz_csc + 255) / 256, 8 * sm_count());
     launch_pdl(k_transfer, dim3(grid), dim3(256), 0, as_stream(stream), p->nnz_csc, p->ptr.p, p->src.p, V_d, dst_nz_d);
+    B2_CUDA(cudaGetLastError());
+    return B2_OK;
+}
+
+extern "C" int b2_transfer_rows(b2_transfer_plan* p, b2_spmv_plan* sp, double* dst_nz_d, double* dst_row_d, const double* V_d,
+                                void* stream) {
+    if (!p || !sp || !dst_nz_d || !dst_row_d || !V_d || sp->nnz != p->nnz_csc) { set_error("b2_transfer_rows: invalid argument"); return B2_ERR_INVALID; }
+    if (p->nnz_csc == 0) return B2_OK;
+    const int grid = (int)std::min<int64_t>((p->nnz_csc + 255) / 256, 8 * sm_count());
+    launch_pdl(k_transfer_rows, dim3(grid), dim3(256), 0, as_stream(stream), p->nnz_csc, p->ptr.p, p->src.p, sp->rowpos.p, V_d, dst_nz_d,
+               dst_row_d);
     B2_CUDA(cudaGetLastError());
     return B2_OK;
 }
diff --git a/madnlp.jl_b200/csrc/kktvec.cu b/madnlp.jl_b200/csrc/kktvec.cu
--- a/madnlp.jl_b200/csrc/kktvec.cu
+++ b/madnlp.jl_b200/csrc/kktvec.cu
@@ -4,6 +4,7 @@
 
 #include "bounds.cuh"
 #include "common.cuh"
+#include "spmv_plan.cuh"
 
 using namespace b2;
 
@@ -177,16 +178,10 @@
     return B2_OK;
 }
 
-struct b2_spmv_plan {
-    int32_t nrow = 0, ncol = 0;
-    int64_t nnz = 0;
-    DevBuf<int32_t> colptr, rowval, rowptr, colidx, valmap;
-};
-
 extern "C" int b2_spmv_plan_create(int32_t nrow, int32_t ncol, const int32_t* colptr_h, const int32_t* rowval_h, b2_spmv_plan** out) {
     if (!out || nrow < 0 || ncol < 0 || !colptr_h) { set_error("b2_spmv_plan_create: invalid argument"); return B2_ERR_INVALID; }
     const int64_t nnz = colptr_h[ncol];
-    std::vector<int32_t> rowptr(nrow + 1, 0), colidx(nnz), valmap(nnz);
+    std::vector<int32_t> rowptr(nrow + 1, 0), colidx(nnz), valmap(nnz), rowpos(nnz);
     for (int64_t p = 0; p < nnz; ++p) {
         if (rowval_h[p] < 0 || rowval_h[p] >= nrow) { set_error("b2_spmv_plan_create: row index out of range"); return B2_ERR_INVALID; }
         rowptr[rowval_h[p] + 1]++;
@@ -198,12 +193,13 @@
             const int32_t q = pos[rowval_h[p]]++;
             colidx[q] = j;
             valmap[q] = p;
+            rowpos[p] = q;
         }
     auto* pl = new b2_spmv_plan();
     pl->nrow = nrow; pl->ncol = ncol; pl->nnz = nnz;
     if (pl->colptr.upload(colptr_h, ncol + 1) != cudaSuccess || pl->rowval.upload(rowval_h, nnz) != cudaSuccess ||
         pl->rowptr.upload(rowptr.data(), rowptr.size()) != cudaSuccess || pl->colidx.upload(colidx.data(), nnz) != cudaSuccess ||
-        pl->valmap.upload(valmap.data(), nnz) != cudaSuccess) {
+        pl->valmap.upload(valmap.data(), nnz) != cudaSuccess || pl->rowpos.upload(rowpos.data(), nnz) != cudaSuccess) {
         delete pl;
         return cuda_fail(cudaGetLastError(), "spmv plan upload", __FILE__, __LINE__);
     }
@@ -244,6 +240,26 @@
         }
 #pragma unroll
         for (int u = 0; u < B; ++u) { nv[u] = (ci[u] >= 0) ? nz[vi[u]] : 0.0; xv[u] = (ci[u] >= 0) ? x[ci[u]] : 0.0; }
+#pragma unroll
+        for (int u = 0; u < B; ++u) if (ci[u] >= 0) s = fma(nv[u], xv[u], s);
+    }
+    return s;
+}
+template <bool STRICT, int B = GB>
+__device__ __forceinline__ double row_dot_rows(const int32_t* __restrict__ rowptr, const int32_t* __restrict__ colidx,
+                                               const double* __restrict__ nz_row, const double* __restrict__ x, int64_t i) {
+    double s = 0.0;
+    const int a = rowptr[i], b = rowptr[i + 1];
+    for (int q0 = a; q0 < b; q0 += B) {
+        int ci[B]; double nv[B], xv[B];
+#pragma unroll
+        for (int u = 0; u < B; ++u) {
+            const bool ok = q0 + u < b;
+            ci[u] = ok ? colidx[q0 + u] : -1; nv[u] = ok ? nz_row[q0 + u] : 0.0;
+            if (STRICT && ci[u] == (int)i) ci[u] = -1;
+        }
+#pragma unroll
+        for (int u = 0; u < B; ++u) xv[u] = (ci[u] >= 0) ? x[ci[u]] : 0.0;
 #pragma unroll
         for (int u = 0; u < B; ++u) if (ci[u] >= 0) s = fma(nv[u], xv[u], s);
     }
@@ -515,10 +531,10 @@
         }
     }
 }
-__global__ void k_cond_pre2(int64_t n, const int32_t* rowptr, const int32_t* colidx, const int32_t* valmap, const double* __restrict__ nz,
+__global__ void __launch_bounds__(256, 4) k_cond_pre2(int64_t n, const int32_t* rowptr, const int32_t* colidx, const double* __restrict__ nz_row,
                             const double* __restrict__ buffer, double* w) {
     pdl_sync();
-    GRID_STRIDE(i, n) w[i] += row_dot_t<false, 2 * GB>(rowptr, colidx, valmap, nz, buffer, i);
+    GRID_STRIDE(i, n) w[i] += row_dot_rows<false, 2 * GB>(rowptr, colidx, nz_row, buffer, i);
 }
 
 template <bool UPDATE>
@@ -575,17 +591,17 @@
     a.ld = l_diag; a.ud = u_diag; a.pr = pr; a.D = D;
     return a;
 }
-static int cond_pre(const char* name, b2_bounds* b, b2_spmv_plan* jt, int64_t n, int64_t m, const double* jt_nz_d, const double* pr_diag_d,
+static int cond_pre(const char* name, b2_bounds* b, b2_spmv_plan* jt, int64_t n, int64_t m, const double* jt_nz_row_d, const double* pr_diag_d,
                     const double* diag_buffer_d, const double* l_diag_d, const double* u_diag_d, double* buffer_d, double* w_d,
                     double* norms_d, void* stream) {
-    if (!b || !jt || !w_d || !buffer_d || b->n_tot != n + m || jt->nrow != n || jt->ncol != m) {
+    if (!b || !jt || !w_d || !buffer_d || (jt->nnz && !jt_nz_row_d) || b->n_tot != n + m || jt->nrow != n || jt->ncol != m) {
         set_error(std::string(name) + ": invalid argument");
         return B2_ERR_INVALID;
     }
     cudaStream_t st = as_stream(stream);
     launch_pdl(k_cond_pre1, dim3(grid_elem(n + m)), dim3(256), 0, st, make_cond(b, n, m, l_diag_d, u_diag_d, pr_diag_d, diag_buffer_d), buffer_d, w_d,
                norms_d);
-    launch_pdl(k_cond_pre2, dim3(grid_elem(n)), dim3(256), 0, st, n, jt->rowptr.p, jt->colidx.p, jt->valmap.p, jt_nz_d, buffer_d, w_d);
+    launch_pdl(k_cond_pre2, dim3(grid_elem(n)), dim3(256), 0, st, n, jt->rowptr.p, jt->colidx.p, jt_nz_row_d, buffer_d, w_d);
     B2_CUDA(cudaGetLastError());
     return B2_OK;
 }
@@ -603,16 +619,16 @@
     B2_CUDA(cudaGetLastError());
     return B2_OK;
 }
-extern "C" int b2_condensed_solve_pre(b2_bounds* b, b2_spmv_plan* jt, int64_t n, int64_t m, const double* jt_nz_d,
+extern "C" int b2_condensed_solve_pre(b2_bounds* b, b2_spmv_plan* jt, int64_t n, int64_t m, const double* jt_nz_row_d,
                                       const double* pr_diag_d, const double* diag_buffer_d, const double* l_diag_d,
                                       const double* u_diag_d, double* buffer_d, double* w_d, void* stream) {
-    return cond_pre("b2_condensed_solve_pre", b, jt, n, m, jt_nz_d, pr_diag_d, diag_buffer_d, l_diag_d, u_diag_d, buffer_d, w_d, nullptr, stream);
-}
-extern "C" int b2_condensed_refine_pre(b2_bounds* b, b2_spmv_plan* jt, int64_t n, int64_t m, const double* jt_nz_d,
+    return cond_pre("b2_condensed_solve_pre", b, jt, n, m, jt_nz_row_d, pr_diag_d, diag_buffer_d, l_diag_d, u_diag_d, buffer_d, w_d, nullptr, stream);
+}
+extern "C" int b2_condensed_refine_pre(b2_bounds* b, b2_spmv_plan* jt, int64_t n, int64_t m, const double* jt_nz_row_d,
                                        const double* pr_diag_d, const double* diag_buffer_d, const double* l_diag_d,
                                        const double* u_diag_d, double* buffer_d, double* w_d, double* norms_d, void* stream) {
     if (!norms_d) { set_error("b2_condensed_refine_pre: invalid argument"); return B2_ERR_INVALID; }
-    return cond_pre("b2_condensed_refine_pre", b, jt, n, m, jt_nz_d, pr_diag_d, diag_buffer_d, l_diag_d, u_diag_d, buffer_d, w_d, norms_d, stream);
+    return cond_pre("b2_condensed_refine_pre", b, jt, n, m, jt_nz_row_d, pr_diag_d, diag_buffer_d, l_diag_d, u_diag_d, buffer_d, w_d, norms_d, stream);
 }
 extern "C" int b2_condensed_solve_post(b2_bounds* b, b2_spmv_plan* jt, int64_t n, int64_t m, const double* jt_nz_d,
                                        const double* pr_diag_d, const double* diag_buffer_d, const double* l_lower_d,
@@ -631,9 +647,10 @@
 
 struct CondMulArgs {
     int64_t n, m;
-    const int32_t *h_colptr, *h_rowval, *h_rowptr, *h_colidx, *h_valmap;
-    const int32_t *j_colptr, *j_rowval, *j_rowptr, *j_colidx, *j_valmap;
+    const int32_t *h_colptr, *h_rowval, *h_rowptr, *h_colidx;
+    const int32_t *j_colptr, *j_rowval, *j_rowptr, *j_colidx;
     const double *h_nz, *j_nz;
+    const double *h_nz_row, *j_nz_row;
 };
 template <bool Y_IN>
 __global__ void k_cond_mul(CondMulArgs c, KktMulArgs a, const double* __restrict__ x, const double* __restrict__ y, double* __restrict__ w,
@@ -646,8 +663,8 @@
     GRID_STRIDE(t, a.n_tot + a.m + a.nlb + a.nub) {
         double wt = Y_IN ? y[t] : w[t];
         if (t < n) {
-            const double hx = col_dot(c.h_colptr, c.h_rowval, c.h_nz, x, t) + row_dot_strict(c.h_rowptr, c.h_colidx, c.h_valmap, c.h_nz, x, t);
-            const double jz = row_dot_t<false, 2 * GB>(c.j_rowptr, c.j_colidx, c.j_valmap, c.j_nz, xz, t);
+            const double hx = col_dot(c.h_colptr, c.h_rowval, c.h_nz, x, t) + row_dot_rows<true>(c.h_rowptr, c.h_colidx, c.h_nz_row, x, t);
+            const double jz = row_dot_rows<false>(c.j_rowptr, c.j_colidx, c.j_nz_row, xz, t);
             wt = a.alpha * hx + scl(a.beta, wt) + a.alpha * jz;
         } else if (t < n + m) {
             wt = scl(a.beta, wt) - a.alpha * xz[t - n];
@@ -663,18 +680,19 @@
     if (norm_out) norm_inf_commit(mx, norm_out);
 }
 static int cond_mul(b2_bounds* b, b2_spmv_plan* hess, b2_spmv_plan* jt, int64_t n, int64_t m, const double* hess_nz_d, const double* jt_nz_d,
+                    const double* hess_nz_row_d, const double* jt_nz_row_d,
                     const double* reg_d, const double* du_diag_d, const double* l_lower_d, const double* u_lower_d, const double* l_diag_d,
                     const double* u_diag_d, double alpha, double beta, const double* x_d, const double* y_d, double* w_d, double* norm_inf_d,
                     void* stream) {
-    if (!b || !hess || !jt || !x_d || !w_d || b->n_tot != n + m || hess->nrow != n || jt->nrow != n || jt->ncol != m) {
+    if (!b || !hess || !jt || !x_d || !w_d || (hess->nnz && !hess_nz_row_d) || (jt->nnz && !jt_nz_row_d) || b->n_tot != n + m || hess->nrow != n || jt->nrow != n || jt->ncol != m) {
         set_error("b2_condensed_kkt_mul: invalid argument");
         return B2_ERR_INVALID;
     }
     CondMulArgs c;
     c.n = n; c.m = m;
-    c.h_colptr = hess->colptr.p; c.h_rowval = hess->rowval.p; c.h_rowptr = hess->rowptr.p; c.h_colidx = hess->colidx.p; c.h_valmap = hess->valmap.p;
-    c.j_colptr = jt->colptr.p; c.j_rowval = jt->rowval.p; c.j_rowptr = jt->rowptr.p; c.j_colidx = jt->colidx.p; c.j_valmap = jt->valmap.p;
-    c.h_nz = hess_nz_d; c.j_nz = jt_nz_d;
+    c.h_colptr = hess->colptr.p; c.h_rowval = hess->rowval.p; c.h_rowptr = hess->rowptr.p; c.h_colidx = hess->colidx.p;
+    c.j_colptr = jt->colptr.p; c.j_rowval = jt->rowval.p; c.j_rowptr = jt->rowptr.p; c.j_colidx = jt->colidx.p;
+    c.h_nz = hess_nz_d; c.j_nz = jt_nz_d; c.h_nz_row = hess_nz_row_d; c.j_nz_row = jt_nz_row_d;
     KktMulArgs a = make_kktmul(b, m, reg_d, du_diag_d, l_lower_d, u_lower_d, l_diag_d, u_diag_d, alpha, beta);
     const int64_t tot = a.n_tot + a.m + a.nlb + a.nub;
     if (y_d) launch_pdl(k_cond_mul<true>, dim3(grid_elem(tot)), dim3(256), 0, as_stream(stream), c, a, x_d, y_d, w_d, (unsigned long long*)norm_inf_d);
@@ -683,26 +701,29 @@
     return B2_OK;
 }
 extern "C" int b2_condensed_kkt_mul_norm(b2_bounds* b, b2_spmv_plan* hess, b2_spmv_plan* jt, int64_t n, int64_t m,
-                                    const double* hess_nz_d, const double* jt_nz_d, const double* reg_d, const double* du_diag_d,
+                                    const double* hess_nz_d, const double* jt_nz_d, const double* hess_nz_row_d,
+                                    const double* jt_nz_row_d, const double* reg_d, const double* du_diag_d,
                                     const double* l_lower_d, const double* u_lower_d, const double* l_diag_d, const double* u_diag_d,
                                     double alpha, double beta, const double* x_d, double* w_d, double* norm_inf_d, void* stream) {
-    return cond_mul(b, hess, jt, n, m, hess_nz_d, jt_nz_d, reg_d, du_diag_d, l_lower_d, u_lower_d, l_diag_d, u_diag_d, alpha, beta, x_d,
+    return cond_mul(b, hess, jt, n, m, hess_nz_d, jt_nz_d, hess_nz_row_d, jt_nz_row_d, reg_d, du_diag_d, l_lower_d, u_lower_d, l_diag_d, u_diag_d, alpha, beta, x_d,
                     nullptr, w_d, norm_inf_d, stream);
 }
 extern "C" int b2_condensed_kkt_mul_norm_y(b2_bounds* b, b2_spmv_plan* hess, b2_spmv_plan* jt, int64_t n, int64_t m,
-                                      const double* hess_nz_d, const double* jt_nz_d, const double* reg_d, const double* du_diag_d,
+                                      const double* hess_nz_d, const double* jt_nz_d, const double* hess_nz_row_d,
+                                    const double* jt_nz_row_d, const double* reg_d, const double* du_diag_d,
                                       const double* l_lower_d, const double* u_lower_d, const double* l_diag_d, const double* u_diag_d,
                                       double alpha, double beta, const double* x_d, const double* y_d, double* w_d, double* norm_inf_d,
                                       void* stream) {
     if (!y_d || y_d == w_d) { set_error("b2_condensed_kkt_mul_norm_y: invalid argument (y must be a vector other than w)"); return B2_ERR_INVALID; }
-    return cond_mul(b, hess, jt, n, m, hess_nz_d, jt_nz_d, reg_d, du_diag_d, l_lower_d, u_lower_d, l_diag_d, u_diag_d, alpha, beta, x_d,
+    return cond_mul(b, hess, jt, n, m, hess_nz_d, jt_nz_d, hess_nz_row_d, jt_nz_row_d, reg_d, du_diag_d, l_lower_d, u_lower_d, l_diag_d, u_diag_d, alpha, beta, x_d,
                     y_d, w_d, norm_inf_d, stream);
 }
 extern "C" int b2_condensed_kkt_mul(b2_bounds* b, b2_spmv_plan* hess, b2_spmv_plan* jt, int64_t n, int64_t m,
-                                    const double* hess_nz_d, const double* jt_nz_d, const double* reg_d, const double* du_diag_d,
+                                    const double* hess_nz_d, const double* jt_nz_d, const double* hess_nz_row_d,
+                                    const double* jt_nz_row_d, const double* reg_d, const double* du_diag_d,
                                     const double* l_lower_d, const double* u_lower_d, const double* l_diag_d, const double* u_diag_d,
                                     double alpha, double beta, const double* x_d, double* w_d, void* stream) {
-    return b2_condensed_kkt_mul_norm(b, hess, jt, n, m, hess_nz_d, jt_nz_d, reg_d, du_diag_d, l_lower_d, u_lower_d, l_diag_d, u_diag_d, alpha,
+    return b2_condensed_kkt_mul_norm(b, hess, jt, n, m, hess_nz_d, jt_nz_d, hess_nz_row_d, jt_nz_row_d, reg_d, du_diag_d, l_lower_d, u_lower_d, l_diag_d, u_diag_d, alpha,
                                      beta, x_d, w_d, nullptr, stream);
 }
 
diff --git a/madnlp.jl_b200/csrc/spmv_plan.cuh b/madnlp.jl_b200/csrc/spmv_plan.cuh
--- /dev/null
+++ b/madnlp.jl_b200/csrc/spmv_plan.cuh
@@ -0,0 +1,8 @@
+#pragma once
+#include "common.cuh"
+
+struct b2_spmv_plan {
+    int32_t nrow = 0, ncol = 0;
+    int64_t nnz = 0;
+    b2::DevBuf<int32_t> colptr, rowval, rowptr, colidx, valmap, rowpos;
+};
diff --git a/madnlp.jl_b200/kkt.py b/madnlp.jl_b200/kkt.py
--- a/madnlp.jl_b200/kkt.py
+++ b/madnlp.jl_b200/kkt.py
@@ -467,10 +467,12 @@
         coo_to_csc = coo_to_csc_device if dev_sym else globals()["coo_to_csc"]
         cp, rv, mp = coo_to_csc(jJ, jI, n, m)
         self.jt_csc = DeviceCSC(n, m, cp, rv, _dz(len(rv)))
+        self.jt_nz_row = _dz(len(rv))
         self._jt_plan = _transfer_plan(mp, len(rv))
         self._jt_spmv = _spmv_plan(n, m, cp, rv)
         hcp, hrv, hmp = coo_to_csc(hI, hJ, n, n)
         self.hess_com = DeviceCSC(n, n, hcp, hrv, _dz(len(hrv)))
+        self.hess_nz_row = _dz(len(hrv))
         self._hess_plan = _transfer_plan(hmp, len(hrv))
         self._hess_spmv = _spmv_plan(n, n, hcp, hrv)
         h = C.c_void_p(); nnz_aug = C.c_int64(0)
@@ -500,7 +502,7 @@
     def initialize(self):
         self._initialize_common()
         self.l_lower.zero_(); self.u_lower.zero_(); self.l_diag.fill_(1.0); self.u_diag.fill_(1.0)
-        self.hess_com.nzval.zero_()
+        self.hess_com.nzval.zero_(); self.hess_nz_row.zero_()
 
     def get_jacobian(self):
         return self.jac
@@ -509,10 +511,12 @@
         return self.hess
 
     def compress_jacobian(self):
-        check(lib.b2_transfer(self._jt_plan.h, ptr(self.jt_csc.nzval), ptr(self.jac), self.stream_ptr()))
+        check(lib.b2_transfer_rows(self._jt_plan.h, self._jt_spmv.h, ptr(self.jt_csc.nzval), ptr(self.jt_nz_row), ptr(self.jac),
+                                   self.stream_ptr()))
 
     def compress_hessian(self):
-        check(lib.b2_transfer(self._hess_plan.h, ptr(self.hess_com.nzval), ptr(self.hess), self.stream_ptr()))
+        check(lib.b2_transfer_rows(self._hess_plan.h, self._hess_spmv.h, ptr(self.hess_com.nzval), ptr(self.hess_nz_row), ptr(self.hess),
+                                   self.stream_ptr()))
 
     def build_kkt(self):
         check(lib.b2_condensed_assemble(self._cond.h, ptr(self.aug_com.nzval), ptr(self.pr_diag), ptr(self.du_diag),
@@ -532,14 +536,16 @@
         return True
 
     def _pre_args(self):
-        return (self._bounds.h, self._jt_spmv.h, self.n, self.m, ptr(self.jt_csc.nzval), ptr(self.pr_diag), ptr(self.diag_buffer))
+        return (self._bounds.h, self._jt_spmv.h, self.n, self.m, ptr(self.jt_nz_row), ptr(self.pr_diag), ptr(self.diag_buffer))
 
     def _post_args(self):
-        return self._pre_args() + (ptr(self.l_lower), ptr(self.u_lower), ptr(self.l_diag), ptr(self.u_diag), ptr(self.buffer))
+        return (self._bounds.h, self._jt_spmv.h, self.n, self.m, ptr(self.jt_csc.nzval), ptr(self.pr_diag), ptr(self.diag_buffer),
+                ptr(self.l_lower), ptr(self.u_lower), ptr(self.l_diag), ptr(self.u_diag), ptr(self.buffer))
 
     def _mul_args(self):
         return (self._bounds.h, self._hess_spmv.h, self._jt_spmv.h, self.n, self.m, ptr(self.hess_com.nzval), ptr(self.jt_csc.nzval),
-                ptr(self.reg), ptr(self.du_diag), ptr(self.l_lower), ptr(self.u_lower), ptr(self.l_diag), ptr(self.u_diag))
+                ptr(self.hess_nz_row), ptr(self.jt_nz_row), ptr(self.reg), ptr(self.du_diag), ptr(self.l_lower), ptr(self.u_lower),
+                ptr(self.l_diag), ptr(self.u_diag))
 
     def solve_kkt(self, w: UnreducedKKTVector):
         sp = self.stream_ptr()
```

Measured after the change: 2029 (median of 6 runs). 1.8% higher.
